# eladhoffer/convNet.pytorch

Measured on NVIDIA H100. Metric: ResNet-50 images/sec (training step, synthetic 224x224), higher is better.
Workload: dtype bf16

## Files before the change

### convnet/pytorch_b200/csrc/bn_common.cuh

```cuda
#pragma once
#include "common.cuh"
#include "host.h"

namespace b200 {

constexpr int kBnThreads = 256;
constexpr int kBnMaxC = 2048;
constexpr int kBnMaxBlocks = 1184;
constexpr int kAccumFloats = kReplicas * 2 * kBnMaxC * 2 + 64;
constexpr int kMaxPartialBlocks = 6 * 148;
constexpr int kWsFloats = kAccumFloats + kMaxPartialBlocks * 2 * kBnMaxC;

struct RowMap {
  int cv, rows_per_iter;
};
static inline RowMap make_rowmap(int C) {
  RowMap m;
  m.cv = C / 8;
  m.rows_per_iter = kBnThreads / m.cv;
  return m;
}
static inline int partial_blocks(long long M, const RowMap& rm, int resident_per_sm) {
  long long iters = (M + rm.rows_per_iter - 1) / rm.rows_per_iter;
  long long want = (iters + 3) / 4;
  long long cap = (long long)resident_per_sm * sm_count();
  if (cap > kMaxPartialBlocks) cap = kMaxPartialBlocks;
  if (want > cap) want = cap;
  if (want < 1) want = 1;
  return (int)want;
}
static inline int stream_blocks(long long M, const RowMap& rm) {
  long long iters = (M + rm.rows_per_iter - 1) / rm.rows_per_iter;
  long long blocks = (iters + 15) / 16;
  if (blocks < 1) blocks = 1;
  if (blocks > 4 * kBnMaxBlocks) blocks = 4 * kBnMaxBlocks;
  return (int)blocks;
}

__device__ __forceinline__ void load8(const __nv_bfloat16* p, float (&f)[8]) {
  const uint4 u = *reinterpret_cast<const uint4*>(p);
  float2 a = unpack_bf16x2(u.x), b = unpack_bf16x2(u.y), c = unpack_bf16x2(u.z), d = unpack_bf16x2(u.w);
  f[0] = a.x; f[1] = a.y; f[2] = b.x; f[3] = b.y; f[4] = c.x; f[5] = c.y; f[6] = d.x; f[7] = d.y;
}
__device__ __forceinline__ uint4 ld_stream(const __nv_bfloat16* p) {
  uint4 u;
  asm volatile("ld.global.nc.L1::no_allocate.v4.u32 {%0,%1,%2,%3}, [%4];"
               : "=r"(u.x), "=r"(u.y), "=r"(u.z), "=r"(u.w) : "l"(p));
  return u;
}
__device__ __forceinline__ void unpack8(const uint4& u, float (&f)[8]) {
  float2 a = unpack_bf16x2(u.x), b = unpack_bf16x2(u.y), c = unpack_bf16x2(u.z), d = unpack_bf16x2(u.w);
  f[0] = a.x; f[1] = a.y; f[2] = b.x; f[3] = b.y; f[4] = c.x; f[5] = c.y; f[6] = d.x; f[7] = d.y;
}
__device__ __forceinline__ void store8(__nv_bfloat16* p, const float (&f)[8]) {
  uint4 u;
  u.x = pack_bf16x2(f[0], f[1]); u.y = pack_bf16x2(f[2], f[3]);
  u.z = pack_bf16x2(f[4], f[5]); u.w = pack_bf16x2(f[6], f[7]);
  *reinterpret_cast<uint4*>(p) = u;
}
__device__ __forceinline__ void loadf8(const float* p, float (&f)[8]) {
  const float4 a = __ldg(reinterpret_cast<const float4*>(p));
  const float4 b = __ldg(reinterpret_cast<const float4*>(p) + 1);
  f[0] = a.x; f[1] = a.y; f[2] = a.z; f[3] = a.w; f[4] = b.x; f[5] = b.y; f[6] = b.z; f[7] = b.w;
}
__device__ __forceinline__ int act_mask_value(float pre, int act) {
  if (act == B200_ACT_RELU) return pre > 0.f ? 1 : 0;
  if (act == B200_ACT_RELU6) return (pre > 0.f && pre < 6.f) ? 1 : 0;
  return 1;
}
__device__ __forceinline__ float act_mask(float v, int act) {
  if (act == B200_ACT_RELU) return v > 0.f ? 1.f : 0.f;
  if (act == B200_ACT_RELU6) return (v > 0.f && v < 6.f) ? 1.f : 0.f;
  return 1.f;
}

__device__ __forceinline__ long long mask_byte_index(long long row, int cv8, int v8) {
  return (((row >> 2) * cv8 + v8) << 2) + (row & 3);
}
template <int ROWS>
__device__ __forceinline__ unsigned long long mask_rows(const uint8_t* __restrict__ amask, long long row0, int cv8,
                                                        int v8) {
  const uint8_t* p = amask + mask_byte_index(row0, cv8, v8);
  if (ROWS == 2) return __ldg(reinterpret_cast<const unsigned short*>(p));
  if (ROWS == 4) return __ldg(reinterpret_cast<const unsigned int*>(p));
  const unsigned long long lo = __ldg(reinterpret_cast<const unsigned int*>(p));
  const unsigned long long hi = __ldg(reinterpret_cast<const unsigned int*>(p + 4LL * cv8));
  return lo | (hi << 32);
}

template <int VEC> struct RawVec;
template <> struct RawVec<4> { uint2 u; };
template <> struct RawVec<8> { uint4 u; };
__device__ __forceinline__ RawVec<4> ldv(const __nv_bfloat16* p, RawVec<4>*) {
  RawVec<4> r;
  asm volatile("ld.global.nc.L1::no_allocate.v2.u32 {%0,%1}, [%2];" : "=r"(r.u.x), "=r"(r.u.y) : "l"(p));
  return r;
}
__device__ __forceinline__ RawVec<8> ldv(const __nv_bfloat16* p, RawVec<8>*) {
  RawVec<8> r;
  r.u = ld_stream(p);
  return r;
}
__device__ __forceinline__ void unpackv(const RawVec<4>& r, float (&f)[4]) {
  const float2 a = unpack_bf16x2(r.u.x), b = unpack_bf16x2(r.u.y);
  f[0] = a.x; f[1] = a.y; f[2] = b.x; f[3] = b.y;
}
__device__ __forceinline__ void unpackv(const RawVec<8>& r, float (&f)[8]) { unpack8(r.u, f); }
__device__ __forceinline__ void storev(__nv_bfloat16* p, const float (&f)[4]) {
  uint2 u;
  u.x = pack_bf16x2(f[0], f[1]); u.y = pack_bf16x2(f[2], f[3]);
  *reinterpret_cast<uint2*>(p) = u;
}
__device__ __forceinline__ void storev(__nv_bfloat16* p, const float (&f)[8]) { store8(p, f); }
template <int VEC>
__device__ __forceinline__ void loadfv(const float* p, float (&f)[VEC]) {
#pragma unroll
  for (int i = 0; i < VEC; i += 4) {
    const float4 a = __ldg(reinterpret_cast<const float4*>(p + i));
    f[i] = a.x; f[i + 1] = a.y; f[i + 2] = a.z; f[i + 3] = a.w;
  }
}

template <int VEC>
static inline RowMap make_rowmap_v(int C) {
  RowMap m;
  m.cv = C / VEC;
  m.rows_per_iter = kBnThreads / m.cv;
  return m;
}

static int check_c(int C, const char* who) {
  B200_REQUIRE(C > 0 && C % 8 == 0 && C <= kBnMaxC, B200_ERR_UNSUPPORTED,
               "%s: C=%d must be a multiple of 8 and <= %d", who, C, kBnMaxC);
  return B200_OK;
}


template <int VEC, int ROWS, int SRC>
__device__ __forceinline__ void bn_bwd_reduce_body(
    const __nv_bfloat16* __restrict__ dy, const __nv_bfloat16* __restrict__ y, const uint8_t* __restrict__ amask,
    const __nv_bfloat16* __restrict__ z, long long M, int C, int cv, int rows_per_iter, int act,
    const float* __restrict__ mean, const float* __restrict__ invstd, const float* __restrict__ gamma,
    const float* __restrict__ beta, float* __restrict__ partial, float dscale) {
  constexpr bool kBits = SRC >= 2;
  const int t = threadIdx.x;
  const bool active = t < rows_per_iter * cv;
  const int r0 = t / cv, v = t - r0 * cv;
  const long long rows_per_block = kBits ? (((M + gridDim.x - 1) / gridDim.x + 7) & ~7LL) : (M + gridDim.x - 1) / gridDim.x;
  const long long row_begin = blockIdx.x * rows_per_block;
  const long long row_end = min(M, row_begin + rows_per_block);
  constexpr long long kRowStep = kBits ? 1 : 0;
  float acc[2 * VEC];
#pragma unroll
  for (int i = 0; i < 2 * VEC; ++i) acc[i] = 0.f;
  if (active) {
    float mu[VEC], sc[VEC], sh[VEC];
    loadfv<VEC>(mean + v * VEC, mu);
    if (SRC == 0 && act != B200_ACT_NONE) {
      float is[VEC];
      loadfv<VEC>(invstd + v * VEC, is);
      if (gamma) loadfv<VEC>(gamma + v * VEC, sc);
      if (beta) loadfv<VEC>(beta + v * VEC, sh);
#pragma unroll
      for (int i = 0; i < VEC; ++i) {
        sc[i] = (gamma ? sc[i] : 1.f) * is[i];
        sh[i] = (beta ? sh[i] : 0.f) - mu[i] * sc[i];
      }
    }
    const long long col = (long long)v * VEC;
    const long long rstep = kRowStep ? 1 : rows_per_iter;
    for (long long r = row_begin + (kRowStep ? (long long)r0 * ROWS : r0); r < row_end;
         r += (long long)ROWS * rows_per_iter) {
      RawVec<VEC> rd[ROWS], rz[ROWS], ry[ROWS];
      unsigned long long rm = 0;
      bool ok[ROWS];
      if (kBits) rm = mask_rows<ROWS>(amask, r, C >> 3, (int)(col >> 3)) >> (col & 7 & ~(VEC - 1));
#pragma unroll
      for (int u = 0; u < ROWS; ++u) {
        const long long rr = r + (long long)u * rstep;
        ok[u] = rr < row_end;
        if (ok[u]) {
          rd[u] = ldv(dy + rr * C + col, (RawVec<VEC>*)nullptr);
          rz[u] = ldv(z + rr * C + col, (RawVec<VEC>*)nullptr);
          if (SRC == 1) ry[u] = ldv(y + rr * C + col, (RawVec<VEC>*)nullptr);
        }
      }
#pragma unroll
      for (int u = 0; u < ROWS; ++u) {
        if (!ok[u]) continue;
        float da[VEC], za[VEC], ya[VEC];
        unpackv(rd[u], da);
        unpackv(rz[u], za);
        if (SRC == 1) unpackv(ry[u], ya);
#pragma unroll
        for (int i = 0; i < VEC; ++i) {
          float g = da[i];
          if (kBits) g = ((rm >> (8 * u + i)) & 1ull) ? (SRC == 3 ? g * dscale : g) : 0.f;
          else if (act != B200_ACT_NONE && act_mask(SRC == 1 ? ya[i] : fmaf(za[i], sc[i], sh[i]), act) == 0.f) g = 0.f;
          acc[i] = fmaf(g, za[i] - mu[i], acc[i]);
          acc[VEC + i] += g;
        }
      }
    }
    float is[VEC];
    loadfv<VEC>(invstd + v * VEC, is);
#pragma unroll
    for (int i = 0; i < VEC; ++i) acc[i] *= is[i];
  }
  __shared__ float red[kBnThreads][2 * VEC + 1];
#pragma unroll
  for (int i = 0; i < 2 * VEC; ++i) red[t][i] = acc[i];
  __syncthreads();
  float* dst = partial + (size_t)blockIdx.x * 2 * C;
  for (int o = t; o < 2 * C; o += kBnThreads) {
    const int stat = o / C;
    const int c = o - stat * C;
    const int vv = c / VEC, e = c - vv * VEC;
    float sacc = 0.f;
    for (int r = 0; r < rows_per_iter; ++r) sacc += red[r * cv + vv][stat * VEC + e];
    dst[o] = sacc;
  }
}

template <int VEC, int ROWS, int SRC>
__device__ __forceinline__ void bn_bwd_dx_body(
    const __nv_bfloat16* __restrict__ dy, const __nv_bfloat16* __restrict__ y, const uint8_t* __restrict__ amask,
    const __nv_bfloat16* __restrict__ z, long long M, int C, int cv, int rows_per_iter, int act,
    const float* __restrict__ mean, const float* __restrict__ invstd, const float* __restrict__ gamma,
    const float* __restrict__ beta, const float* __restrict__ sums, __nv_bfloat16* __restrict__ dz,
    __nv_bfloat16* __restrict__ g_out, float dscale) {
  constexpr bool kBits = SRC >= 2;
  const int t = threadIdx.x;
  if (t >= rows_per_iter * cv) return;
  const int r0 = t / cv, v = t - r0 * cv;
  const long long rows_per_block = kBits ? (((M + gridDim.x - 1) / gridDim.x + 7) & ~7LL) : (M + gridDim.x - 1) / gridDim.x;
  const long long row_begin = blockIdx.x * rows_per_block;
  const long long row_end = min(M, row_begin + rows_per_block);
  constexpr long long kRowStep = kBits ? 1 : 0;
  float A[VEC], B[VEC], Cc[VEC], sh[VEC];
  {
    float mu[VEC], is[VEC], dg[VEC], dbt[VEC];
    loadfv<VEC>(mean + v * VEC, mu);
    loadfv<VEC>(invstd + v * VEC, is);
    if (gamma) loadfv<VEC>(gamma + v * VEC, A);
    if (beta) loadfv<VEC>(beta + v * VEC, sh);
    loadfv<VEC>(sums + v * VEC, dg);
    loadfv<VEC>(sums + C + v * VEC, dbt);
    const float invM = 1.f / (float)M;
#pragma unroll
    for (int i = 0; i < VEC; ++i) {
      const float gm = gamma ? A[i] : 1.f;
      A[i] = gm * is[i];
      B[i] = -gm * is[i] * is[i] * dg[i] * invM;
      Cc[i] = -A[i] * dbt[i] * invM - B[i] * mu[i];
      sh[i] = (beta ? sh[i] : 0.f) - mu[i] * A[i];
    }
  }
  const long long col = (long long)v * VEC;
  const long long rstep = kRowStep ? 1 : rows_per_iter;
  for (long long r = row_begin + (kRowStep ? (long long)r0 * ROWS : r0); r < row_end;
       r += (long long)ROWS * rows_per_iter) {
    RawVec<VEC> rd[ROWS], rz[ROWS], ry[ROWS];
    unsigned long long rm = 0;
    bool ok[ROWS];
    if (kBits) rm = mask_rows<ROWS>(amask, r, C >> 3, (int)(col >> 3)) >> (col & 7 & ~(VEC - 1));
#pragma unroll
    for (int u = 0; u < ROWS; ++u) {
      const long long rr = r + (long long)u * rstep;
      ok[u] = rr < row_end;
      if (ok[u]) {
        rd[u] = ldv(dy + rr * C + col, (RawVec<VEC>*)nullptr);
        rz[u] = ldv(z + rr * C + col, (RawVec<VEC>*)nullptr);
        if (SRC == 1) ry[u] = ldv(y + rr * C + col, (RawVec<VEC>*)nullptr);
      }
    }
#pragma unroll
    for (int u = 0; u < ROWS; ++u) {
      if (!ok[u]) continue;
      const long long rr = r + (long long)u * rstep;
      float da[VEC], za[VEC], ya[VEC];
      unpackv(rd[u], da);
      unpackv(rz[u], za);
      if (SRC == 1) unpackv(ry[u], ya);
#pragma unroll
      for (int i = 0; i < VEC; ++i) {
        float g = da[i];
        if (kBits) g = ((rm >> (8 * u + i)) & 1ull) ? (SRC == 3 ? g * dscale : g) : 0.f;
        else if (act != B200_ACT_NONE && act_mask(SRC == 1 ? ya[i] : fmaf(za[i], A[i], sh[i]), act) == 0.f) g = 0.f;
        da[i] = g;
        za[i] = A[i] * g + B[i] * za[i] + Cc[i];
      }
      storev(dz + rr * C + col, za);
      if (g_out) storev(g_out + rr * C + col, da);
    }
  }
}

void launch_bwd_reduce_final(const float* partial, int nblocks, int C, float* sums, float* dgamma_acc,
                             float* dbeta_acc, cudaStream_t stream);

}
```

### convnet/pytorch_b200/csrc/conv.cu

```cuda
#include "common.cuh"
#include "host.h"
#include <stdlib.h>
#include <utility>

namespace b200 {

constexpr int kMaxStages = 8;
constexpr int kMaxTaps = 32;
constexpr int kConsumers = 256;
constexpr int kProducerWarp = 8;

struct TapEntry {
  uint16_t off_w, off_h;
  uint16_t b_tap;
  uint16_t pad_;
};

struct IgemmParams {
  int M_total;
  int I, J;
  int trav;
  int lower_w, lower_h;
  int N_total;
  int block_n, n_tiles, m_tiles;
  int ck, c_chunks;
  int ntaps;
  int num_stages;
  uint32_t a_bytes, b_bytes, tx_bytes;
  int OH, OW, os, oh0, ow0;
  int ldo;
  int act, out_fp32;
  int tma_store;
  int plain_a;
  int b_stationary;
  int own_ntile;
  int window;
  uint32_t epi_bytes;
  double* stats;
  void* out;
  const void* res;
  const float* bias;
  TapEntry taps[kMaxTaps];
};

__device__ __forceinline__ void store_pair(const IgemmParams& p, float v0, float v1, long long off, int n) {
  if (n >= p.N_total) return;
  const bool two = n + 1 < p.N_total;
  const bool vec = two && (p.ldo & 1) == 0;
  if (p.bias != nullptr) {
    v0 += __ldg(p.bias + n);
    if (two) v1 += __ldg(p.bias + n + 1);
  }
  if (p.res != nullptr) {
    const __nv_bfloat16* r = reinterpret_cast<const __nv_bfloat16*>(p.res) + off + n;
    if (vec) {
      const float2 t = unpack_bf16x2(*reinterpret_cast<const uint32_t*>(r));
      v0 += t.x;
      v1 += t.y;
    } else {
      v0 += __bfloat162float(r[0]);
      if (two) v1 += __bfloat162float(r[1]);
    }
  }
  v0 = apply_act(v0, p.act);
  v1 = apply_act(v1, p.act);
  if (p.out_fp32) {
    float* o = reinterpret_cast<float*>(p.out) + off + n;
    if (vec) {
      *reinterpret_cast<float2*>(o) = make_float2(v0, v1);
    } else {
      o[0] = v0;
      if (two) o[1] = v1;
    }
  } else {
    __nv_bfloat16* o = reinterpret_cast<__nv_bfloat16*>(p.out) + off + n;
    if (vec) {
      *reinterpret_cast<uint32_t*>(o) = pack_bf16x2(v0, v1);
    } else {
      o[0] = __float2bfloat16(v0);
      if (two) o[1] = __float2bfloat16(v1);
    }
  }
}

template <int KS, int SZ>
__device__ __forceinline__ void igemm_stage_mma(float (&acc)[2][SZ], uint64_t da, uint64_t db, uint32_t a_half,
                                                uint32_t scale0) {
  wgmma_fence();
#pragma unroll
  for (int k = 0; k < KS; ++k) {
    wgmma_bf16<0, 0>(acc[0], da + 2 * k, db + 2 * k, k != 0 ? 1u : scale0);
    wgmma_bf16<0, 0>(acc[1], da + a_half + 2 * k, db + 2 * k, k != 0 ? 1u : scale0);
  }
  wgmma_commit();
}

template <int BN>
__global__ void __launch_bounds__(kThreads, 1)
conv_igemm_kernel(const __grid_constant__ CUtensorMap tmA, const __grid_constant__ CUtensorMap tmB,
                  const __grid_constant__ CUtensorMap tmC, const __grid_constant__ CUtensorMap tmR,
                  const __grid_constant__ IgemmParams p) {
  extern __shared__ uint8_t smem_raw[];
  __shared__ __align__(8) uint64_t full_bar[kMaxStages];
  __shared__ __align__(8) uint64_t empty_bar[kMaxStages];
  __shared__ __align__(8) uint64_t turn_bar[2], res_bar[2], bstat_bar;

  const int warp = threadIdx.x >> 5;
  const int lane = threadIdx.x & 31;
  const uint32_t raw_addr = smem_u32(smem_raw);
  uint8_t* smem = smem_raw + (((raw_addr + 1023u) & ~1023u) - raw_addr);
  const uint32_t stage_bytes = p.b_stationary ? p.a_bytes : p.a_bytes + p.b_bytes;
  uint8_t* sBstat = smem + p.num_stages * stage_bytes;
  uint8_t* epi = sBstat + (p.b_stationary ? static_cast<uint32_t>(p.ntaps * p.c_chunks) * p.b_bytes : 0u);

  if (threadIdx.x == 0) {
    for (int s = 0; s < p.num_stages; ++s) {
      mbar_init(&full_bar[s], 1);
      mbar_init(&empty_bar[s], 4);
    }
    mbar_init(&bstat_bar, 1);
    for (int i = 0; i < 2; ++i) {
      mbar_init(&res_bar[i], 1);
      mbar_init(&turn_bar[i], 4);
    }
    fence_mbar_init();
    prefetch_tmap(&tmA);
    prefetch_tmap(&tmB);
    if (p.tma_store) {
      prefetch_tmap(&tmC);
      if (p.res != nullptr) prefetch_tmap(&tmR);
    }
  }
  __syncthreads();

  const int k_iters = p.ntaps * p.c_chunks;
  const int walk_first = p.own_ntile ? static_cast<int>(blockIdx.x) / p.n_tiles : static_cast<int>(blockIdx.x);
  const int walk_step = p.own_ntile ? static_cast<int>(gridDim.x) / p.n_tiles : static_cast<int>(gridDim.x);
  const int walk_end = p.own_ntile ? p.m_tiles : p.m_tiles * p.n_tiles;
  const int own_n = static_cast<int>(blockIdx.x) % p.n_tiles;

  if (warp >= kProducerWarp) {
    producer_setmaxnreg();
    if (warp == kProducerWarp && lane == 0) {
      int stage = 0;
      uint32_t phase = 0;
      const int IJ = p.I * p.J;
      if (p.b_stationary && walk_first < walk_end) {
        mbar_arrive_expect_tx(&bstat_bar, static_cast<uint32_t>(k_iters) * (p.tx_bytes - p.a_bytes));
        for (int t = 0; t < p.ntaps; ++t)
          for (int cc = 0; cc < p.c_chunks; ++cc)
            tma_load_3d(&tmB, &bstat_bar, sBstat + (t * p.c_chunks + cc) * p.b_bytes, cc * p.ck, p.taps[t].b_tap,
                        p.own_ntile ? own_n * BN : 0);
      }
      for (int tile = walk_first; tile < walk_end; tile += walk_step) {
        const int m_tile = p.own_ntile ? tile : tile / p.n_tiles;
        const int n_tile = p.own_ntile ? own_n : tile - m_tile * p.n_tiles;
        const int m0 = m_tile * kTileM;
        const int img = m0 / IJ;
        const int rem = m0 - img * IJ;
        const int bi = rem / p.J;
        const int bj = rem - bi * p.J;
        const int base_w = bj * p.trav + p.lower_w;
        const int base_h = bi * p.trav + p.lower_h;
        const int a_c0 = p.window ? (n_tile * BN / p.window) * p.window : 0;
        for (int t = 0; t < p.ntaps; ++t) {
          const TapEntry te = p.taps[t];
          for (int cc = 0; cc < p.c_chunks; ++cc) {
            mbar_wait(&empty_bar[stage], phase ^ 1u);
            uint8_t* sa = smem + stage * stage_bytes;
            uint8_t* sb = sa + p.a_bytes;
            mbar_arrive_expect_tx(&full_bar[stage], p.b_stationary ? p.a_bytes : p.tx_bytes);
            const int a_c = a_c0 + cc * p.ck;
            if (p.plain_a)
              tma_load_2d(&tmA, &full_bar[stage], sa, a_c, m0);
            else
              tma_load_im2col_4d(&tmA, &full_bar[stage], sa, a_c, base_w, base_h, img, te.off_w, te.off_h);
            if (!p.b_stationary) tma_load_3d(&tmB, &full_bar[stage], sb, cc * p.ck, te.b_tap, n_tile * BN);
            if (++stage == p.num_stages) { stage = 0; phase ^= 1u; }
          }
        }
      }
    }
    return;
  }
  consumer_setmaxnreg();

  const int wg = warp >> 2;
  const int wt = threadIdx.x & 127;
  const int r_lo = (warp & 3) * 16 + (lane >> 2);
  const int c_lo = 2 * (lane & 3);
  const bool leader = wt == 0;
  const uint32_t row_bytes = p.ck * 2;
  const uint64_t proto = make_smem_desc(0, 16, 8 * row_bytes, layout_type_for_row_bytes(row_bytes));
  const uint32_t a_half = (64u * row_bytes) >> 4;
  const int ksteps = p.ck / 16;
  const uint32_t bstat_addr = smem_u32(sBstat);
  constexpr int nbox = BN / 64;
  uint8_t* epi_w = epi + wg * p.epi_bytes;
  const int st_col = wt % BN;
  constexpr int st_rows = BN;
  const int st_row0 = (wt / BN) * st_rows;
  int st_ntile = -1;
  float st_s1 = 0.f, st_s2 = 0.f;
  const int IJ = p.I * p.J;
  if (p.b_stationary && walk_first < walk_end) mbar_wait(&bstat_bar, 0);

  float acc[2][BN / 2];
  int local = 0;
  for (int tile = walk_first; tile < walk_end; tile += walk_step, ++local) {
    if ((local & 1) != wg) continue;
    const int m_tile = p.own_ntile ? tile : tile / p.n_tiles;
    const int n_tile = p.own_ntile ? own_n : tile - m_tile * p.n_tiles;
    const int nbase = n_tile * BN;
    const int mine = local >> 1;
    if (p.tma_store) {
      if (leader && mine > 0) bulk_wait_group_read0();
      named_bar_sync(1 + wg, 128);
      if (leader && p.res != nullptr) {
        fence_proxy_async();
        mbar_arrive_expect_tx(&res_bar[wg], static_cast<uint32_t>(nbox) * kTileM * 128u);
        for (int b = 0; b < nbox; ++b)
          tma_load_2d(&tmR, &res_bar[wg], epi_w + b * (kTileM * 128), nbase + b * 64, m_tile * kTileM);
      }
    }

    const int pos = local * k_iters;
    int stage = pos % p.num_stages;
    uint32_t phase = static_cast<uint32_t>(pos / p.num_stages) & 1u;
    if (local > 0) mbar_wait(&turn_bar[wg], static_cast<uint32_t>((local - 1) >> 1) & 1u);
    wgmma_fence_acc(acc[0]);
    wgmma_fence_acc(acc[1]);
    int prev = 0;
    for (int it = 0; it < k_iters; ++it) {
      mbar_wait(&full_bar[stage], phase);
      const uint32_t a_addr = smem_u32(smem + stage * stage_bytes);
      const uint64_t da = proto + (a_addr >> 4);
      const uint64_t db = proto + ((p.b_stationary ? bstat_addr + it * p.b_bytes : a_addr + p.a_bytes) >> 4);
      const uint32_t scale0 = it != 0 ? 1u : 0u;
      if (ksteps == 4) igemm_stage_mma<4>(acc, da, db, a_half, scale0);
      else if (ksteps == 2) igemm_stage_mma<2>(acc, da, db, a_half, scale0);
      else igemm_stage_mma<1>(acc, da, db, a_half, scale0);
      wgmma_wait<1>();
      if (it > 0) release_stage(&empty_bar[prev], lane);
      prev = stage;
      if (++stage == p.num_stages) { stage = 0; phase ^= 1u; }
    }
    __syncwarp();
    if (lane == 0) mbar_arrive(&turn_bar[wg ^ 1]);
    wgmma_wait<0>();
    wgmma_fence_acc(acc[0]);
    wgmma_fence_acc(acc[1]);
    release_stage(&empty_bar[prev], lane);

    if (p.tma_store) {
      if constexpr (BN % 64 == 0) {
        if (p.res != nullptr) mbar_wait(&res_bar[wg], static_cast<uint32_t>(mine & 1));
#pragma unroll
        for (int j = 0; j < BN / 2; j += 4) {
          const int c = 2 * j + c_lo;
          float bias0 = 0.f, bias1 = 0.f;
          if (p.bias != nullptr) { bias0 = __ldg(p.bias + nbase + c); bias1 = __ldg(p.bias + nbase + c + 1); }
#pragma unroll
          for (int mh = 0; mh < 2; ++mh)
#pragma unroll
            for (int h = 0; h < 2; ++h) {
              const int row = mh * 64 + r_lo + 8 * h;
              uint32_t* dst = reinterpret_cast<uint32_t*>(epi_w + staged_offset(row, c, kTileM * 128));
              float v0 = acc[mh][j + 2 * h] + bias0, v1 = acc[mh][j + 2 * h + 1] + bias1;
              if (p.res != nullptr) {
                const float2 t = unpack_bf16x2(*dst);
                v0 += t.x;
                v1 += t.y;
              }
              *dst = pack_bf16x2(apply_act(v0, p.act), apply_act(v1, p.act));
            }
        }
        fence_proxy_async();
        named_bar_sync(1 + wg, 128);
        if (leader) {
          for (int b = 0; b < nbox; ++b)
            tma_store_2d(&tmC, epi_w + b * (kTileM * 128), nbase + b * 64, m_tile * kTileM);
          bulk_commit_group();
        }
        if constexpr (BN == 64 || BN == 128) {
          if (p.stats != nullptr) {
            if (st_ntile != n_tile) {
              if (st_ntile >= 0) {
                flush_bn_stats(p.stats, p.N_total, st_ntile * BN, st_col, st_s1, st_s2);
                st_s1 = 0.f; st_s2 = 0.f;
              }
              st_ntile = n_tile;
            }
            float s1 = 0.f, s2 = 0.f;
#pragma unroll 8
            for (int r = st_row0; r < st_row0 + st_rows; ++r) {
              const float vv = __bfloat162float(*reinterpret_cast<const __nv_bfloat16*>(epi_w + staged_offset(r, st_col, kTileM * 128)));
              s1 += vv;
              s2 = fmaf(vv, vv, s2);
            }
            st_s1 += s1;
            st_s2 += s2;
          }
        }
      }
      continue;
    }
#pragma unroll
    for (int mh = 0; mh < 2; ++mh)
#pragma unroll
      for (int h = 0; h < 2; ++h) {
        const int m = m_tile * kTileM + mh * 64 + r_lo + 8 * h;
        if (m >= p.M_total) continue;
        const int img = m / IJ;
        const int rem = m - img * IJ;
        const int bi = rem / p.J;
        const int bj = rem - bi * p.J;
        const long long off = ((static_cast<long long>(img) * p.OH + (bi * p.os + p.oh0)) * p.OW + (bj * p.os + p.ow0)) *
                              static_cast<long long>(p.ldo);
#pragma unroll
        for (int j = 0; j < BN / 2; j += 4) store_pair(p, acc[mh][j + 2 * h], acc[mh][j + 2 * h + 1], off, nbase + 2 * j + c_lo);
      }
  }
  if constexpr (BN == 64 || BN == 128)
    if (p.stats != nullptr && st_ntile >= 0) flush_bn_stats(p.stats, p.N_total, st_ntile * BN, st_col, st_s1, st_s2);
  if (p.tma_store && leader) bulk_wait_group0();
}

constexpr int kBk = 64;
struct WgradParams {
  int M_total;
  int P, Q;
  int trav;
  int lower_w, lower_h;
  int K_out, C, taps_total;
  int ckA, ckB;
  int bk;
  int c_chunks;
  int total_boxes;
  int boxes_per_cta;
  int k_tiles, col_groups, splits;
  int blocks_per_split, total_blocks;
  int num_stages;
  uint32_t boxA_bytes, boxB_bytes, stage_bytes;
  float* dw;
  int plain_x;
  float* partial;
  int pitch;
  int window;
  int S_filter;
};

__device__ __forceinline__ void red_add_v2(float* addr, float a, float b) {
  asm volatile("red.global.add.v2.f32 [%0], {%1, %2};" ::"l"(addr), "f"(a), "f"(b) : "memory");
}

template <int NC>
__global__ void __launch_bounds__(kThreads, 1)
conv_wgrad_kernel(const __grid_constant__ CUtensorMap tmDy, const __grid_constant__ CUtensorMap tmX,
                  const __grid_constant__ WgradParams p) {
  extern __shared__ uint8_t smem_raw[];
  __shared__ __align__(8) uint64_t full_bar[kMaxStages];
  __shared__ __align__(8) uint64_t empty_bar[kMaxStages];

  const int warp = threadIdx.x >> 5;
  const int lane = threadIdx.x & 31;
  const uint32_t raw_addr = smem_u32(smem_raw);
  uint8_t* smem = smem_raw + (((raw_addr + 1023u) & ~1023u) - raw_addr);

  if (threadIdx.x == 0) {
    for (int s = 0; s < p.num_stages; ++s) {
      mbar_init(&full_bar[s], 1);
      mbar_init(&empty_bar[s], kConsumers / 32);
    }
    fence_mbar_init();
    prefetch_tmap(&tmDy);
    prefetch_tmap(&tmX);
  }
  __syncthreads();

  const int tiles = p.k_tiles * p.col_groups;
  const int split = blockIdx.x / tiles;
  const int tile = blockIdx.x - split * tiles;
  const int k_tile = tile % p.k_tiles;
  const int cgroup = tile / p.k_tiles;
  const int k0 = k_tile * kTileM;
  const int box0 = cgroup * p.boxes_per_cta;
  const int nboxes = min(p.boxes_per_cta, p.total_boxes - box0);
  const int blk_begin = split * p.blocks_per_split;
  const int blk_end = min(p.total_blocks, blk_begin + p.blocks_per_split);
  const int nblk = blk_end - blk_begin;
  const uint32_t a_tile = (kTileM / p.ckA) * p.boxA_bytes;
  if (nblk <= 0) return;

  if (warp >= kProducerWarp) {
    producer_setmaxnreg();
    if (warp == kProducerWarp && lane == 0) {
      int stage = 0;
      uint32_t phase = 0;
      const int PQ = p.P * p.Q;
      const int nA = min(kTileM / p.ckA, (p.K_out - k0 + p.ckA - 1) / p.ckA);
      int box_c[8];
      uint16_t box_w[8], box_h[8];
      for (int x = 0; x < 8; ++x) {
        const int id = box0 + min(x, nboxes - 1);
        const int t = id / p.c_chunks;
        const int th = t / p.S_filter;
        box_c[x] = (id - t * p.c_chunks) * p.ckB + (p.window ? k0 : 0);
        box_w[x] = static_cast<uint16_t>(t - th * p.S_filter);
        box_h[x] = static_cast<uint16_t>(th);
      }
      const uint32_t tx = nA * p.boxA_bytes + nboxes * p.boxB_bytes;
      for (int b = blk_begin; b < blk_end; ++b) {
        const int pix0 = b * p.bk;
        mbar_wait(&empty_bar[stage], phase ^ 1u);
        uint8_t* sa = smem + stage * p.stage_bytes;
        uint8_t* sb = sa + a_tile;
        mbar_arrive_expect_tx(&full_bar[stage], tx);
        for (int a = 0; a < nA; ++a)
          tma_load_2d(&tmDy, &full_bar[stage], sa + a * p.boxA_bytes, k0 + a * p.ckA, pix0);
        if (p.plain_x) {
#pragma unroll
          for (int x = 0; x < 8; ++x)
            if (x < nboxes) tma_load_2d(&tmX, &full_bar[stage], sb + x * p.boxB_bytes, box_c[x], pix0);
        } else {
          const int img = pix0 / PQ;
          const int rem = pix0 - img * PQ;
          const int pi = rem / p.Q;
          const int pj = rem - pi * p.Q;
          const int base_w = pj * p.trav + p.lower_w;
          const int base_h = pi * p.trav + p.lower_h;
#pragma unroll
          for (int x = 0; x < 8; ++x)
            if (x < nboxes)
              tma_load_im2col_4d(&tmX, &full_bar[stage], sb + x * p.boxB_bytes, box_c[x], base_w, base_h, img, box_w[x],
                                 box_h[x]);
        }
        if (++stage == p.num_stages) { stage = 0; phase ^= 1u; }
      }
    }
    return;
  }

  consumer_setmaxnreg();

  const int wg = warp >> 2;
  const bool wg_on = k0 + wg * 64 < p.K_out;
  const int ncols = nboxes * p.ckB;
  const uint64_t protoA = make_smem_desc(0, p.boxA_bytes, 8 * p.ckA * 2, layout_type_for_row_bytes(p.ckA * 2));
  const uint64_t protoB = make_smem_desc(0, p.boxB_bytes, 8 * p.ckB * 2, layout_type_for_row_bytes(p.ckB * 2));
  const uint32_t a_wg = (wg * (64 / p.ckA) * p.boxA_bytes) >> 4;
  const uint32_t kincA = (16u * p.ckA * 2) >> 4, kincB = (16u * p.ckB * 2) >> 4;
  float acc[NC / 2];
  wgmma_fence_acc(acc);
  int stage = 0, prev = 0;
  uint32_t phase = 0;
  for (int b = 0; b < nblk; ++b) {
    mbar_wait(&full_bar[stage], phase);
    const uint32_t a_addr = smem_u32(smem + stage * p.stage_bytes);
    if (wg_on) {
      const uint64_t da = protoA + (a_addr >> 4) + a_wg, db = protoB + ((a_addr + a_tile) >> 4);
      wgmma_fence();
#pragma unroll
      for (int k = 0; k < kBk / 16; ++k)
        wgmma_bf16<1, 1>(acc, da + k * kincA, db + k * kincB, (b | k) != 0 ? 1u : 0u);
      wgmma_commit();
      wgmma_wait<1>();
    }
    if (b > 0) release_stage(&empty_bar[prev], lane);
    prev = stage;
    if (++stage == p.num_stages) { stage = 0; phase ^= 1u; }
  }
  wgmma_wait<0>();
  wgmma_fence_acc(acc);
  release_stage(&empty_bar[prev], lane);
  if (!wg_on) return;

  const int r_lo = wg * 64 + (warp & 3) * 16 + (lane >> 2);
  const int c_lo = 2 * (lane & 3);
#pragma unroll
  for (int h = 0; h < 2; ++h) {
    const int k = k0 + r_lo + 8 * h;
    if (k >= p.K_out) continue;
    if (p.partial != nullptr) {
      float* dst = p.partial + ((static_cast<long long>(tile) * p.splits + split) * kTileM + (r_lo + 8 * h)) * p.pitch;
#pragma unroll
      for (int j = 0; j < NC / 2; j += 4)
        if (2 * j < ncols)
          *reinterpret_cast<float2*>(dst + 2 * j + c_lo) = make_float2(acc[j + 2 * h], acc[j + 2 * h + 1]);
    } else {
#pragma unroll
      for (int j = 0; j < NC / 2; j += 4) {
        const int col = 2 * j + c_lo;
        if (col < ncols) {
          const int x = col / p.ckB;
          const int id = box0 + x;
          const int tap = id / p.c_chunks;
          const int c = (id - tap * p.c_chunks) * p.ckB + (col - x * p.ckB);
          if (c < p.C) red_add_v2(p.dw + (static_cast<long long>(k) * p.taps_total + tap) * p.C + c, acc[j + 2 * h],
                                  acc[j + 2 * h + 1]);
        }
      }
    }
  }
}

__global__ void __launch_bounds__(256) conv_wgrad_reduce_kernel(const float* __restrict__ partial, float* __restrict__ dw,
                                                                int K_out, int taps, int C, int ck, int tap_stride,
                                                                int cc_stride, int bpc, int k_tiles, int splits,
                                                                int pitch) {
  __shared__ float4 red[8][32];
  const int c4n = C >> 2;
  const long long total = static_cast<long long>(K_out) * taps * c4n;
  const int lane = threadIdx.x & 31, w = threadIdx.x >> 5, nw = blockDim.x >> 5;
  for (long long base = static_cast<long long>(blockIdx.x) * 32; base < total; base += static_cast<long long>(gridDim.x) * 32) {
    const long long idx = base + lane;
    float4 acc = make_float4(0.f, 0.f, 0.f, 0.f);
    int c = 0, tap = 0, k = 0;
    if (idx < total) {
      c = static_cast<int>(idx % c4n) * 4;
      tap = static_cast<int>((idx / c4n) % taps);
      k = static_cast<int>(idx / (static_cast<long long>(c4n) * taps));
      const int k_tile = k / kTileM, row = k - k_tile * kTileM;
      const int cc = c / ck;
      const int id = tap * tap_stride + cc * cc_stride;
      const int cgroup = id / bpc, x = id - cgroup * bpc;
      const int unit = cgroup * k_tiles + k_tile;
      const float* src = partial + ((static_cast<long long>(unit) * splits) * kTileM + row) * pitch + x * ck + (c - cc * ck);
      for (int s2 = w; s2 < splits; s2 += nw) {
        const float4 v = __ldcg(reinterpret_cast<const float4*>(src + static_cast<long long>(s2) * kTileM * pitch));
        acc.x += v.x; acc.y += v.y; acc.z += v.z; acc.w += v.w;
      }
    }
    red[w][lane] = acc;
    __syncthreads();
    if (w == 0 && idx < total) {
      for (int j = 1; j < nw; ++j) {
        const float4 v = red[j][lane];
        acc.x += v.x; acc.y += v.y; acc.z += v.z; acc.w += v.w;
      }
      float4* o = reinterpret_cast<float4*>(dw + (static_cast<long long>(k) * taps + tap) * C + c);
      float4 cur = *o;
      cur.x += acc.x; cur.y += acc.y; cur.z += acc.z; cur.w += acc.w;
      *o = cur;
    }
    __syncthreads();
  }
}

static int pick_ck(int channels) { return channels <= 16 ? 16 : (channels <= 32 ? 32 : 64); }

static int encode_im2col(CUtensorMap* tm, const void* base, int Nimg, int H, int W, int C, int ck, int pixels,
                         int lower_w, int lower_h, int upper_w, int upper_h, int trav, long long pix_stride = 0,
                         long long row_stride = 0, long long img_stride = 0) {
  EncodeIm2colFn fn = encode_im2col_fn();
  B200_REQUIRE(fn != nullptr, B200_ERR_CUDA, "cuTensorMapEncodeIm2col entry point unavailable");
  cuuint64_t dims[4] = {(cuuint64_t)C, (cuuint64_t)W, (cuuint64_t)H, (cuuint64_t)Nimg};
  cuuint64_t strides[3] = {(cuuint64_t)C * 2, (cuuint64_t)W * C * 2, (cuuint64_t)H * W * C * 2};
  if (pix_stride > 0) {
    strides[0] = (cuuint64_t)pix_stride * 2;
    strides[1] = (cuuint64_t)row_stride * 2;
    strides[2] = (cuuint64_t)img_stride * 2;
  }
  int lower[2] = {lower_w, lower_h};
  int upper[2] = {upper_w, upper_h};
  cuuint32_t estr[4] = {1, (cuuint32_t)trav, (cuuint32_t)trav, 1};
  B200_REQUIRE(lower_w >= -128 && lower_w <= 127 && lower_h >= -128 && lower_h <= 127 && upper_w >= -128 &&
                   upper_w <= 127 && upper_h >= -128 && upper_h <= 127,
               B200_ERR_UNSUPPORTED, "im2col corner offsets out of the TMA range");
  CUresult r = fn(tm, CU_TENSOR_MAP_DATA_TYPE_BFLOAT16, 4, const_cast<void*>(base), dims, strides, lower, upper,
                  (cuuint32_t)ck, (cuuint32_t)pixels, estr, CU_TENSOR_MAP_INTERLEAVE_NONE,
                  swizzle_for_row_bytes(ck * 2), CU_TENSOR_MAP_L2_PROMOTION_L2_128B,
                  CU_TENSOR_MAP_FLOAT_OOB_FILL_NONE);
  B200_REQUIRE(r == CUDA_SUCCESS, B200_ERR_CUDA,
               "cuTensorMapEncodeIm2col failed (%d) N=%d H=%d W=%d C=%d ck=%d pix=%d lower=(%d,%d) upper=(%d,%d) trav=%d",
               (int)r, Nimg, H, W, C, ck, pixels, lower_w, lower_h, upper_w, upper_h, trav);
  int drv = 0;
  cudaDriverGetVersion(&drv);
  if (drv <= 13010 && (size_t)Nimg * H * W * C * 2 < 131072) {
    reinterpret_cast<uint64_t*>(tm)[1] &= ~(1ull << 21);
  }
  return B200_OK;
}

static const int kSmemBudget = 200 * 1024;
static const int kSmemBudgetMax = 224 * 1024;

int launch_wgrad_reduce(const float* partial, float* dw, int K_out, int taps, int C, int ck, int tap_stride,
                        int cc_stride, int bpc, int k_tiles, int splits, int pitch, cudaStream_t stream) {
  const long long total = static_cast<long long>(K_out) * taps * (C / 4);
  long long blocks = (total + 31) / 32;
  if (blocks > 16LL * sm_count()) blocks = 16LL * sm_count();
  int warps = 8;
  while (warps > 1 && warps > splits) warps >>= 1;
  b200::launch(conv_wgrad_reduce_kernel, static_cast<int>(blocks), 32 * warps, 0, stream, partial, dw, K_out, taps, C, ck,
               tap_stride, cc_stride, bpc, k_tiles, splits, pitch);
  B200_CHECK_LAUNCH("conv_wgrad_reduce_kernel");
  return B200_OK;
}

struct IgemmLaunch {
  const void* src; int Nimg, SH, SW, SC;
  long long s_pix, s_row, s_img;
  const void* wmat; int Nout, wtaps;
  int I, J, trav, lower_w, lower_h;
  int ntaps; TapEntry taps[kMaxTaps];
  void* out; int OH, OW, os, oh0, ow0, ldo;
  const void* res; const float* bias; int act, out_fp32;
  double* stats;
  int window;
};

template <int... Is>
static auto igemm_kernel_for(int block_n, std::integer_sequence<int, Is...>) {
  static constexpr decltype(&conv_igemm_kernel<16>) table[] = {&conv_igemm_kernel<16 * (Is + 1)>...};
  return table[block_n / 16 - 1];
}
static auto wgrad_kernel_for(int ncols) {
  static constexpr decltype(&conv_wgrad_kernel<16>) table[] = {
      &conv_wgrad_kernel<16>,  &conv_wgrad_kernel<32>,  &conv_wgrad_kernel<48>,  &conv_wgrad_kernel<64>,
      &conv_wgrad_kernel<80>,  &conv_wgrad_kernel<96>,  &conv_wgrad_kernel<112>, &conv_wgrad_kernel<128>,
      nullptr,                 &conv_wgrad_kernel<160>, nullptr,                 &conv_wgrad_kernel<192>,
      nullptr,                 &conv_wgrad_kernel<224>, nullptr,                 &conv_wgrad_kernel<256>};
  return table[ncols / 16 - 1];
}

static int launch_igemm(const IgemmLaunch& L, cudaStream_t stream) {
  B200_REQUIRE(L.SC % 8 == 0, B200_ERR_UNSUPPORTED, "igemm: source channels (%d) must be a multiple of 8", L.SC);
  B200_REQUIRE(L.ntaps >= 1 && L.ntaps <= kMaxTaps, B200_ERR_UNSUPPORTED, "igemm: %d taps unsupported", L.ntaps);
  IgemmParams p;
  memset(&p, 0, sizeof(p));
  p.M_total = L.Nimg * L.I * L.J;
  B200_REQUIRE(p.M_total > 0, B200_ERR_INVALID, "igemm: empty problem");
  p.I = L.I; p.J = L.J; p.trav = L.trav; p.lower_w = L.lower_w; p.lower_h = L.lower_h;
  p.N_total = L.Nout;
  p.block_n = L.Nout % 128 == 0 ? 128 : (L.Nout % 64 == 0 ? 64 : 0);
  if (p.block_n == 0) {
    const int nt = (L.Nout + 127) / 128;
    p.block_n = (((L.Nout + nt - 1) / nt) + 15) / 16 * 16;
  }
  p.n_tiles = (L.Nout + p.block_n - 1) / p.block_n;
  p.m_tiles = (p.M_total + kTileM - 1) / kTileM;
  p.ck = pick_ck(L.SC);
  p.c_chunks = (L.SC + p.ck - 1) / p.ck;
  p.window = L.window;
  if (L.window) {
    B200_REQUIRE(L.window % 64 == 0 && L.window <= 256 && L.SC == L.Nout && L.Nout % L.window == 0, B200_ERR_UNSUPPORTED,
                 "igemm: window %d needs C == K (C=%d K=%d), K %% window == 0", L.window, L.SC, L.Nout);
    p.block_n = L.window <= 128 ? L.window : L.window / 2;
    p.n_tiles = L.Nout / p.block_n;
    p.ck = 64;
    p.c_chunks = L.window / 64;
  }
  p.ntaps = L.ntaps;
  p.a_bytes = kTileM * p.ck * 2;
  p.b_bytes = p.block_n * p.ck * 2;
  p.tx_bytes = p.a_bytes + p.b_bytes;
  uint32_t stage = p.a_bytes + p.b_bytes;
  if (stage % 1024) { p.b_bytes += 1024 - stage % 1024; stage = p.a_bytes + p.b_bytes; }
  p.tma_store = (L.os == 1 && !L.out_fp32 && (p.block_n % 64) == 0 && (L.Nout % p.block_n) == 0 && L.ldo == L.Nout &&
                 L.OH == L.I && L.OW == L.J && L.oh0 == 0 && L.ow0 == 0) ? 1 : 0;
  const int epi_bytes = p.tma_store ? kTileM * p.block_n * 2 : 0;
  const int epi_total = 2 * epi_bytes;
  const int b_all = L.ntaps * p.c_chunks * (int)p.b_bytes;
  int bstat_bytes = 0;
  if (p.n_tiles == 1 && !L.window && (p.a_bytes % 1024) == 0 && (p.b_bytes % 1024) == 0 && b_all <= 64 * 1024) {
    p.b_stationary = 1;
    bstat_bytes = b_all;
    stage = p.a_bytes;
  }
  int grid_own = 0;
  if (!p.b_stationary && p.n_tiles > 1 && p.n_tiles <= 8 && !L.window &&
      (p.a_bytes % 1024) == 0 && (p.b_bytes % 1024) == 0 && (L.Nout % p.block_n) == 0) {
    const int ctas = sm_count() / p.n_tiles;
    const long long a_all = (long long)p.M_total * L.SC * 2 * L.ntaps;
    const long long w_all = (long long)b_all * p.n_tiles;
    const long long rr_bytes = a_all * p.n_tiles + w_all * p.m_tiles;
    const long long own_bytes = a_all * p.n_tiles + (long long)b_all * ctas * p.n_tiles;
    const int stages_left = (kSmemBudgetMax - epi_total - b_all) / (int)p.a_bytes;
    if (ctas >= 1 && p.m_tiles >= 4 * ctas && stages_left >= 3 && own_bytes * 4 <= rr_bytes * 3) {
      p.b_stationary = 1;
      p.own_ntile = 1;
      bstat_bytes = b_all;
      stage = p.a_bytes;
      grid_own = ctas * p.n_tiles;
    }
  }
  p.epi_bytes = (uint32_t)epi_bytes;
  p.num_stages = (kSmemBudgetMax - epi_total - bstat_bytes) / (int)stage;
  if (p.num_stages > kMaxStages) p.num_stages = kMaxStages;
  if (p.num_stages < 2) p.num_stages = 2;
  p.OH = L.OH; p.OW = L.OW; p.os = L.os; p.oh0 = L.oh0; p.ow0 = L.ow0; p.ldo = L.ldo;
  p.act = L.act; p.out_fp32 = L.out_fp32; p.out = L.out; p.res = L.res; p.bias = L.bias;
  p.stats = L.stats;
  if (L.stats != nullptr)
    B200_REQUIRE(p.tma_store && (128 % p.block_n) == 0 && L.res == nullptr && L.bias == nullptr && L.act == 0,
                 B200_ERR_UNSUPPORTED, "conv_fprop: fused BN statistics need a dense bf16 output with K %% 64 == 0 "
                 "(block_n=%d) and no bias/residual/activation", p.block_n);
  for (int t = 0; t < L.ntaps; ++t) p.taps[t] = L.taps[t];

  const int upper_w = L.lower_w + (L.J - 1) * L.trav + 1 - L.SW;
  const int upper_h = L.lower_h + (L.I - 1) * L.trav + 1 - L.SH;
  CUtensorMap tmA, tmB;
  int rc;
  p.plain_a = (L.ntaps == 1 && L.trav == 1 && L.lower_w == 0 && L.lower_h == 0 && L.taps[0].off_w == 0 &&
               L.taps[0].off_h == 0 && L.I == L.SH && L.J == L.SW && L.s_pix == 0) ? 1 : 0;
  if (p.plain_a)
    rc = encode_tiled(&tmA, L.src, 2, {L.SC, p.M_total}, {p.ck, kTileM}, "igemm A");
  else
    rc = encode_im2col(&tmA, L.src, L.Nimg, L.SH, L.SW, L.SC, p.ck, kTileM, L.lower_w, L.lower_h, upper_w, upper_h,
                       L.trav, L.s_pix, L.s_row, L.s_img);
  if (rc) return rc;
  rc = encode_tiled(&tmB, L.wmat, 3, {L.window ? L.window : L.SC, L.wtaps, L.Nout}, {p.ck, 1, p.block_n}, "igemm B");
  if (rc) return rc;

  CUtensorMap tmC, tmR;
  memset(&tmC, 0, sizeof(tmC));
  memset(&tmR, 0, sizeof(tmR));
  if (p.tma_store) {
    rc = encode_tiled(&tmC, L.out, 2, {L.ldo, p.M_total}, {64, kTileM}, "igemm output");
    if (rc) return rc;
    if (L.res != nullptr) {
      rc = encode_tiled(&tmR, L.res, 2, {L.ldo, p.M_total}, {64, kTileM}, "igemm residual");
      if (rc) return rc;
    }
  }
  const int smem_bytes = p.num_stages * (int)stage + bstat_bytes + epi_total + 1024;
  const auto kfn = igemm_kernel_for(p.block_n, std::make_integer_sequence<int, 8>{});
  rc = set_smem_attr((const void*)kfn, smem_bytes);
  if (rc) return rc;
  const int total_tiles = p.m_tiles * p.n_tiles;
  const int grid = grid_own ? grid_own : (total_tiles < sm_count() ? total_tiles : sm_count());
  if (getenv("B200_IGEMM_DEBUG")) {
    const int max_tiles = p.own_ntile ? (p.m_tiles + grid / p.n_tiles - 1) / (grid / p.n_tiles)
                                      : (total_tiles + grid - 1) / grid;
    fprintf(stderr, "[igemm] M=%d C=%d N=%d taps=%d os=%d block_n=%d n_tiles=%d m_tiles=%d ck=%d k_iters=%d stages=%d "
            "tma_store=%d plain_a=%d bstat=%d own=%d out_fp32=%d bias=%d res=%d act=%d stats=%d grid=%d max_tiles=%d "
            "smem=%d\n",
            p.M_total, L.SC, L.Nout, L.ntaps, L.os, p.block_n, p.n_tiles, p.m_tiles, p.ck, L.ntaps * p.c_chunks,
            p.num_stages, p.tma_store, p.plain_a, p.b_stationary, p.own_ntile, p.out_fp32, L.bias != nullptr,
            L.res != nullptr, p.act, L.stats != nullptr, grid, max_tiles, smem_bytes);
  }
  b200::launch(kfn, grid, kThreads, smem_bytes, stream, tmA, tmB, tmC, tmR, p);
  B200_CHECK_LAUNCH("conv_igemm_kernel");
  return B200_OK;
}

static int check_desc(const b200_conv_desc* d) {
  B200_REQUIRE(d != nullptr, B200_ERR_INVALID, "conv: null descriptor");
  B200_REQUIRE(d->N > 0 && d->H > 0 && d->W > 0 && d->C > 0 && d->K > 0 && d->R > 0 && d->S > 0 && d->P > 0 &&
                   d->Q > 0 && d->stride >= 1 && d->stride <= 8,
               B200_ERR_INVALID, "conv: bad descriptor N=%d H=%d W=%d C=%d K=%d R=%d S=%d P=%d Q=%d stride=%d", d->N,
               d->H, d->W, d->C, d->K, d->R, d->S, d->P, d->Q, d->stride);
  B200_REQUIRE(d->R * d->S <= kMaxTaps, B200_ERR_UNSUPPORTED, "conv: %dx%d filter exceeds %d taps", d->R, d->S,
               kMaxTaps);
  B200_REQUIRE((d->x_pixel_stride == 0 && d->x_row_stride == 0 && d->x_image_stride == 0) ||
                   (d->x_pixel_stride > 0 && d->x_pixel_stride % 8 == 0 && d->x_row_stride % 8 == 0 &&
                    d->x_image_stride % 8 == 0 && d->x_row_stride > 0 && d->x_image_stride > 0),
               B200_ERR_INVALID, "conv: x strides must all be 0 (dense) or positive multiples of 8 elements");
  B200_REQUIRE(d->window == 0 || (d->window % 64 == 0 && d->C == d->K && d->C % d->window == 0 && d->x_pixel_stride == 0),
               B200_ERR_UNSUPPORTED, "conv: window %d needs C == K, C %% window == 0 (C=%d K=%d)", d->window, d->C, d->K);
  return B200_OK;
}

}

using namespace b200;

extern "C" int b200_conv_fprop(const b200_conv_desc* d, const void* x, const void* w, void* y,
                               const b200_epilogue* ep, b200_stream_t stream) {
  int rc = check_desc(d);
  if (rc) return rc;
  B200_REQUIRE(x && w && y, B200_ERR_INVALID, "conv_fprop: null pointer");
  B200_REQUIRE(d->C % 8 == 0, B200_ERR_UNSUPPORTED, "conv_fprop: C=%d must be a multiple of 8 (pad the input)", d->C);
  if (d->stride == 1 && d->pad_h == d->pad_w && d->P == d->H + 2 * d->pad_h - d->R + 1 &&
      d->Q == d->W + 2 * d->pad_w - d->S + 1 && d->x_pixel_stride == 0 && (!ep || !ep->out_fp32) &&
      !(ep && ep->bias && ep->bn_stats_workspace) && (d->window == 0 || d->window == 64) &&
      halo_eligible(d->P, d->Q, d->C, d->K, d->R, d->S, d->pad_h)) {
    return launch_halo(x, w, y, ep ? ep->residual : nullptr, ep ? ep->bias : nullptr, d->N, d->P, d->Q, d->C, d->K,
                       d->R, d->S, d->pad_h, 0, ep ? ep->act : 0,
                       (ep && ep->bn_stats_workspace) ? reinterpret_cast<double*>(ep->bn_stats_workspace) : nullptr,
                       (cudaStream_t)stream, d->window);
  }
  IgemmLaunch L;
  memset(&L, 0, sizeof(L));
  L.src = x; L.Nimg = d->N; L.SH = d->H; L.SW = d->W; L.SC = d->C;
  L.s_pix = d->x_pixel_stride; L.s_row = d->x_row_stride; L.s_img = d->x_image_stride;
  L.wmat = w; L.Nout = d->K; L.wtaps = d->R * d->S;
  L.I = d->P; L.J = d->Q; L.trav = d->stride; L.lower_w = -d->pad_w; L.lower_h = -d->pad_h;
  L.ntaps = d->R * d->S;
  for (int r = 0; r < d->R; ++r)
    for (int s = 0; s < d->S; ++s) {
      TapEntry& t = L.taps[r * d->S + s];
      t.off_w = (uint16_t)s; t.off_h = (uint16_t)r; t.b_tap = (uint16_t)(r * d->S + s); t.pad_ = 0;
    }
  L.out = y; L.OH = d->P; L.OW = d->Q; L.os = 1; L.oh0 = 0; L.ow0 = 0; L.ldo = d->K;
  L.res = ep ? ep->residual : nullptr;
  L.bias = ep ? ep->bias : nullptr;
  L.act = ep ? ep->act : 0;
  L.out_fp32 = ep ? ep->out_fp32 : 0;
  L.stats = (ep && ep->bn_stats_workspace) ? reinterpret_cast<double*>(ep->bn_stats_workspace) : nullptr;
  L.window = d->window;
  return launch_igemm(L, (cudaStream_t)stream);
}

extern "C" int b200_conv_dgrad(const b200_conv_desc* d, const void* dy, const void* wt, void* dx,
                               const void* residual, b200_stream_t stream_) {
  int rc = check_desc(d);
  if (rc) return rc;
  cudaStream_t stream = (cudaStream_t)stream_;
  B200_REQUIRE(dy && wt && dx, B200_ERR_INVALID, "conv_dgrad: null pointer");
  B200_REQUIRE(d->K % 8 == 0, B200_ERR_UNSUPPORTED, "conv_dgrad: K=%d must be a multiple of 8", d->K);
  const int st = d->stride;
  B200_REQUIRE(st == 1 || st == 2, B200_ERR_UNSUPPORTED, "conv_dgrad: stride %d unsupported", st);
  if (d->R == 3 && d->S == 3 && st == 1 && d->pad_h == 1 && d->pad_w == 1 && d->P == d->H && d->Q == d->W &&
      (d->window == 0 || d->window == 64) && halo_eligible(d->H, d->W, d->K, d->C, 3, 3, 1)) {
    return launch_halo(dy, wt, dx, residual, nullptr, d->N, d->H, d->W, d->K, d->C, 3, 3, 1, 1, 0, nullptr, stream,
                       d->window);
  }
  bool any_empty = false;
  for (int ph = 0; ph < st; ++ph)
    for (int pw = 0; pw < st; ++pw) {
      int nr = 0, ns = 0;
      for (int r = 0; r < d->R; ++r) if (((ph + d->pad_h - r) % st + st) % st == 0) ++nr;
      for (int s = 0; s < d->S; ++s) if (((pw + d->pad_w - s) % st + st) % st == 0) ++ns;
      if (nr * ns == 0 && (d->H - ph + st - 1) / st > 0 && (d->W - pw + st - 1) / st > 0) any_empty = true;
    }
  if (any_empty) {
    B200_REQUIRE(residual == nullptr, B200_ERR_UNSUPPORTED,
                 "conv_dgrad: residual add with an empty stride class is unsupported");
    cudaError_t e = cudaMemsetAsync(dx, 0, (size_t)d->N * d->H * d->W * d->C * 2, stream);
    B200_REQUIRE(e == cudaSuccess, B200_ERR_CUDA, "conv_dgrad: memset failed: %s", cudaGetErrorString(e));
    count_launch();
  }
  for (int ph = 0; ph < st; ++ph)
    for (int pw = 0; pw < st; ++pw) {
      const int I = (d->H - ph + st - 1) / st;
      const int J = (d->W - pw + st - 1) / st;
      if (I <= 0 || J <= 0) continue;
      IgemmLaunch L;
      memset(&L, 0, sizeof(L));
      int dh[kMaxTaps], dwv[kMaxTaps], rr[kMaxTaps], ss[kMaxTaps];
      int nr = 0, ns = 0;
      for (int r = 0; r < d->R; ++r) {
        const int v = ph + d->pad_h - r;
        if (((v % st) + st) % st == 0) { dh[nr] = (v - (((v % st) + st) % st)) / st; rr[nr] = r; ++nr; }
      }
      for (int s = 0; s < d->S; ++s) {
        const int v = pw + d->pad_w - s;
        if (((v % st) + st) % st == 0) { dwv[ns] = (v - (((v % st) + st) % st)) / st; ss[ns] = s; ++ns; }
      }
      if (nr * ns == 0) continue;
      int lo_h = dh[0], lo_w = dwv[0];
      for (int i = 1; i < nr; ++i) lo_h = dh[i] < lo_h ? dh[i] : lo_h;
      for (int i = 1; i < ns; ++i) lo_w = dwv[i] < lo_w ? dwv[i] : lo_w;
      L.ntaps = nr * ns;
      for (int a = 0; a < nr; ++a)
        for (int b = 0; b < ns; ++b) {
          TapEntry& t = L.taps[a * ns + b];
          t.off_h = (uint16_t)(dh[a] - lo_h);
          t.off_w = (uint16_t)(dwv[b] - lo_w);
          t.b_tap = (uint16_t)(rr[a] * d->S + ss[b]);
          t.pad_ = 0;
        }
      L.src = dy; L.Nimg = d->N; L.SH = d->P; L.SW = d->Q; L.SC = d->K;
      L.wmat = wt; L.Nout = d->C; L.wtaps = d->R * d->S;
      L.I = I; L.J = J; L.trav = 1; L.lower_w = lo_w; L.lower_h = lo_h;
      L.out = dx; L.OH = d->H; L.OW = d->W; L.os = st; L.oh0 = ph; L.ow0 = pw; L.ldo = d->C;
      L.res = residual; L.bias = nullptr; L.act = 0; L.out_fp32 = 0;
      L.window = d->window;
      rc = launch_igemm(L, stream);
      if (rc) return rc;
    }
  return B200_OK;
}

extern "C" size_t b200_conv_wgrad_workspace_bytes(void) {
  return static_cast<size_t>(sm_count() + 8) * kTileM * 512 * sizeof(float);
}

extern "C" int b200_conv_wgrad(const b200_conv_desc* d, const void* x, const void* dy, float* dw, void* workspace,
                               size_t workspace_bytes, b200_stream_t stream_) {
  int rc = check_desc(d);
  if (rc) return rc;
  cudaStream_t stream = (cudaStream_t)stream_;
  B200_REQUIRE(x && dy && dw, B200_ERR_INVALID, "conv_wgrad: null pointer");
  B200_REQUIRE(d->C % 8 == 0 && d->K % 8 == 0, B200_ERR_UNSUPPORTED,
               "conv_wgrad: C=%d and K=%d must be multiples of 8", d->C, d->K);
  if (d->stride == 1 && d->pad_h == d->pad_w && d->P == d->H + 2 * d->pad_h - d->R + 1 &&
      d->Q == d->W + 2 * d->pad_w - d->S + 1 && d->x_pixel_stride == 0 &&
      (d->window == 0 || d->window == 128) &&
      halo_wgrad_eligible(d->P, d->Q, d->C, d->K, d->R, d->S, d->pad_h, d->window))
    return launch_halo_wgrad(x, dy, dw, workspace, workspace_bytes, d->N, d->P, d->Q, d->C, d->K, d->R, d->S, d->pad_h,
                             stream, d->window);
  B200_REQUIRE(d->window == 0 || d->window == 128, B200_ERR_UNSUPPORTED, "conv_wgrad: window must be 0 or 128");
  const int Cw = d->window ? d->window : d->C;
  WgradParams p;
  memset(&p, 0, sizeof(p));
  p.M_total = d->N * d->P * d->Q;
  p.P = d->P; p.Q = d->Q; p.trav = d->stride; p.lower_w = -d->pad_w; p.lower_h = -d->pad_h;
  p.K_out = d->K; p.C = Cw; p.taps_total = d->R * d->S;
  p.window = d->window;
  p.ckA = pick_ck(d->K);
  p.ckB = pick_ck(Cw);
  p.bk = kBk;
  p.c_chunks = (Cw + p.ckB - 1) / p.ckB;
  p.total_boxes = p.taps_total * p.c_chunks;
  p.k_tiles = (d->K + kTileM - 1) / kTileM;
  p.boxA_bytes = p.bk * p.ckA * 2;
  p.boxB_bytes = p.bk * p.ckB * 2;
  p.boxes_per_cta = 256 / p.ckB;
  if (p.boxes_per_cta > 8) p.boxes_per_cta = 8;
  if (p.boxes_per_cta > p.total_boxes) p.boxes_per_cta = p.total_boxes;
  p.col_groups = (p.total_boxes + p.boxes_per_cta - 1) / p.boxes_per_cta;
  p.total_blocks = (p.M_total + p.bk - 1) / p.bk;
  const int tiles = p.k_tiles * p.col_groups;
  int splits = sm_count() / tiles;
  if (splits > p.total_blocks) splits = p.total_blocks;
  if (splits < 1) splits = 1;
  p.blocks_per_split = (p.total_blocks + splits - 1) / splits;
  p.splits = (p.total_blocks + p.blocks_per_split - 1) / p.blocks_per_split;
  p.stage_bytes = (kTileM / p.ckA) * p.boxA_bytes + p.boxes_per_cta * p.boxB_bytes;
  p.stage_bytes = (p.stage_bytes + 1023u) & ~1023u;
  p.num_stages = kSmemBudget / (int)p.stage_bytes;
  if (p.num_stages > kMaxStages) p.num_stages = kMaxStages;
  if (p.num_stages < 2) p.num_stages = 2;
  p.dw = dw;
  p.pitch = p.boxes_per_cta * p.ckB;
  p.partial = nullptr;
  if (p.splits > 1) {
    const size_t need = static_cast<size_t>(tiles) * p.splits * kTileM * p.pitch * sizeof(float);
    B200_REQUIRE(workspace != nullptr && workspace_bytes >= need, B200_ERR_INVALID,
                 "conv_wgrad: workspace too small (%zu < %zu); see b200_conv_wgrad_workspace_bytes()", workspace_bytes,
                 need);
    B200_REQUIRE((Cw & 3) == 0, B200_ERR_UNSUPPORTED, "conv_wgrad: C must be a multiple of 4");
    p.partial = static_cast<float*>(workspace);
  }
  p.S_filter = d->S;
  CUtensorMap tmDy, tmX;
  rc = encode_tiled(&tmDy, dy, 2, {d->K, p.M_total}, {p.ckA, p.bk}, "wgrad dy");
  if (rc) return rc;
  const int upper_w = p.lower_w + (d->Q - 1) * d->stride + 1 - d->W;
  const int upper_h = p.lower_h + (d->P - 1) * d->stride + 1 - d->H;
  p.plain_x = (d->R == 1 && d->S == 1 && d->stride == 1 && d->pad_h == 0 && d->pad_w == 0 && d->P == d->H &&
               d->Q == d->W && d->x_pixel_stride == 0) ? 1 : 0;
  if (getenv("B200_WGRAD_DEBUG"))
    fprintf(stderr, "[wgrad] K=%d C=%d taps=%d stride=%d ckA=%d ckB=%d kt=%d bpc=%d k_groups=%d col_groups=%d splits=%d "
            "bps=%d stages=%d stage=%u nc=%d nboxes_last=%d plain_x=%d partial=%d\n", d->K, d->C, p.taps_total,
            d->stride, p.ckA, p.ckB, 1, p.boxes_per_cta, p.k_tiles, p.col_groups, p.splits, p.blocks_per_split,
            p.num_stages, p.stage_bytes, p.pitch, p.total_boxes - (p.col_groups - 1) * p.boxes_per_cta, p.plain_x,
            p.partial != nullptr);
  if (p.plain_x)
    rc = encode_tiled(&tmX, x, 2, {d->C, p.M_total}, {p.ckB, p.bk}, "wgrad x");
  else
    rc = encode_im2col(&tmX, x, d->N, d->H, d->W, d->C, p.ckB, p.bk, p.lower_w, p.lower_h, upper_w, upper_h,
                       d->stride, d->x_pixel_stride, d->x_row_stride, d->x_image_stride);
  if (rc) return rc;
  const int smem_bytes = p.num_stages * (int)p.stage_bytes + 1024;
  const auto kfn = wgrad_kernel_for(p.pitch);
  rc = set_smem_attr((const void*)kfn, smem_bytes);
  if (rc) return rc;
  const int grid = tiles * p.splits;
  b200::launch(kfn, grid, kThreads, smem_bytes, stream, tmDy, tmX, p);
  B200_CHECK_LAUNCH("conv_wgrad_kernel");
  if (p.partial == nullptr) return B200_OK;
  return launch_wgrad_reduce(p.partial, dw, d->K, p.taps_total, Cw, p.ckB, p.c_chunks, 1, p.boxes_per_cta, p.k_tiles,
                             p.splits, p.pitch, stream);
}
```

### convnet/pytorch_b200/csrc/host.cu

```cuda
#include "host.h"
#include <atomic>
#include <mutex>
#include <string.h>

namespace b200 {

static thread_local char g_err[512] = "";
static std::atomic<long long> g_launches{0};

void set_error(const char* fmt, ...) {
  va_list ap;
  va_start(ap, fmt);
  vsnprintf(g_err, sizeof(g_err), fmt, ap);
  va_end(ap);
}
void count_launch(int n) { g_launches.fetch_add(n, std::memory_order_relaxed); }

int sm_count() {
  static int cached[64] = {0};
  int dev = 0;
  cudaGetDevice(&dev);
  if (dev < 0 || dev >= 64) dev = 0;
  if (cached[dev] == 0) {
    int n = 0;
    cudaDeviceGetAttribute(&n, cudaDevAttrMultiProcessorCount, dev);
    cached[dev] = n > 0 ? n : 148;
  }
  return cached[dev];
}

static void* driver_entry(const char* name) {
  void* fn = nullptr;
  cudaDriverEntryPointQueryResult q;
  if (cudaGetDriverEntryPoint(name, &fn, cudaEnableDefault, &q) != cudaSuccess ||
      q != cudaDriverEntryPointSuccess) {
    return nullptr;
  }
  return fn;
}
EncodeIm2colFn encode_im2col_fn() {
  static EncodeIm2colFn fn = (EncodeIm2colFn)driver_entry("cuTensorMapEncodeIm2col");
  return fn;
}

typedef CUresult (*EncodeTiledFn)(CUtensorMap*, CUtensorMapDataType, cuuint32_t, void*, const cuuint64_t*,
                                  const cuuint64_t*, const cuuint32_t*, const cuuint32_t*, CUtensorMapInterleave,
                                  CUtensorMapSwizzle, CUtensorMapL2promotion, CUtensorMapFloatOOBfill);

int encode_tiled(CUtensorMap* tm, const void* base, int rank, const long long (&dims)[4], const int (&box)[4],
                 const char* what) {
  static EncodeTiledFn fn = (EncodeTiledFn)driver_entry("cuTensorMapEncodeTiled");
  B200_REQUIRE(fn != nullptr, B200_ERR_CUDA, "cuTensorMapEncodeTiled entry point unavailable");
  cuuint64_t gdims[4], strides[3];
  cuuint32_t gbox[4], estr[4] = {1, 1, 1, 1};
  for (int i = 0; i < rank; ++i) {
    gdims[i] = (cuuint64_t)dims[i];
    gbox[i] = (cuuint32_t)box[i];
    if (i + 1 < rank) strides[i] = (i == 0 ? 2 : strides[i - 1]) * gdims[i];
  }
  CUresult r = fn(tm, CU_TENSOR_MAP_DATA_TYPE_BFLOAT16, rank, const_cast<void*>(base), gdims, strides, gbox, estr,
                  CU_TENSOR_MAP_INTERLEAVE_NONE, swizzle_for_row_bytes(box[0] * 2), CU_TENSOR_MAP_L2_PROMOTION_L2_128B,
                  CU_TENSOR_MAP_FLOAT_OOB_FILL_NONE);
  if (r != CUDA_SUCCESS) {
    char d[96] = "", b[64] = "";
    for (int i = 0, nd = 0, nb = 0; i < rank; ++i) {
      nd += snprintf(d + nd, sizeof(d) - nd, i ? ",%lld" : "%lld", dims[i]);
      nb += snprintf(b + nb, sizeof(b) - nb, i ? ",%d" : "%d", box[i]);
    }
    set_error("%s: cuTensorMapEncodeTiled(%dd) failed (%d) dims=(%s) box=(%s)", what, rank, (int)r, d, b);
    return B200_ERR_CUDA;
  }
  return B200_OK;
}

int set_smem_attr(const void* fn, int bytes) {
  cudaError_t e = cudaFuncSetAttribute(fn, cudaFuncAttributeMaxDynamicSharedMemorySize, bytes);
  B200_REQUIRE(e == cudaSuccess, B200_ERR_CUDA, "cudaFuncSetAttribute(smem=%d): %s", bytes, cudaGetErrorString(e));
  return B200_OK;
}

}

extern "C" {
const char* b200_last_error(void) { return b200::g_err; }
int b200_version(void) { return 100; }
long long b200_launch_count(void) { return b200::g_launches.load(); }
}
```

### convnet/pytorch_b200/csrc/host.h

```cpp
#pragma once
#include <cuda.h>
#include <cuda_runtime.h>
#include <stdarg.h>
#include <stdio.h>
#include "../../../include/b200conv.h"

namespace b200 {

void set_error(const char* fmt, ...);
void count_launch(int n = 1);
int sm_count();

typedef CUresult (*EncodeIm2colFn)(CUtensorMap*, CUtensorMapDataType, cuuint32_t, void*, const cuuint64_t*,
                                   const cuuint64_t*, const int*, const int*, cuuint32_t, cuuint32_t,
                                   const cuuint32_t*, CUtensorMapInterleave, CUtensorMapSwizzle,
                                   CUtensorMapL2promotion, CUtensorMapFloatOOBfill);
EncodeIm2colFn encode_im2col_fn();

int encode_tiled(CUtensorMap* tm, const void* base, int rank, const long long (&dims)[4], const int (&box)[4],
                 const char* what);
int set_smem_attr(const void* fn, int bytes);

int launch_wgrad_reduce(const float* partial, float* dw, int K_out, int taps, int C, int ck, int tap_stride,
                        int cc_stride, int bpc, int k_tiles, int splits, int pitch, cudaStream_t stream);

bool halo_geometry_ok(int H, int W, int Cs, int R, int S, int pad);
bool halo_eligible(int H, int W, int Cs, int Nout, int R, int S, int pad);
int launch_halo(const void* src, const void* wmat, void* out, const void* res, const float* bias, int N, int H, int W,
                int Cs, int Nout, int R, int S, int pad, int dir, int act, double* stats, cudaStream_t stream,
                int window = 0);

bool halo_wgrad_eligible(int H, int W, int C, int K_out, int R, int S, int pad, int window);
int launch_halo_wgrad(const void* x, const void* dy, float* dw, void* workspace, size_t workspace_bytes, int N, int H,
                      int W, int C, int K_out, int R, int S, int pad, cudaStream_t stream, int window = 0);

template <typename... KArgs, typename... Args>
inline void launch(void (*kernel)(KArgs...), dim3 grid, dim3 block, size_t smem, cudaStream_t stream, Args&&... args) {
  kernel<<<grid, block, smem, stream>>>(static_cast<KArgs>(args)...);
}

inline CUtensorMapSwizzle swizzle_for_row_bytes(int row_bytes) {
  return row_bytes == 128 ? CU_TENSOR_MAP_SWIZZLE_128B
                          : (row_bytes == 64 ? CU_TENSOR_MAP_SWIZZLE_64B : CU_TENSOR_MAP_SWIZZLE_32B);
}

#define B200_CHECK_LAUNCH(name)                                                   \
  do {                                                                            \
    cudaError_t e__ = cudaGetLastError();                                         \
    if (e__ != cudaSuccess) {                                                     \
      b200::set_error("%s: launch failed: %s", name, cudaGetErrorString(e__));    \
      return B200_ERR_CUDA;                                                       \
    }                                                                             \
    b200::count_launch();                                                         \
  } while (0)

#define B200_REQUIRE(cond, code, ...)   \
  do {                                  \
    if (!(cond)) {                      \
      b200::set_error(__VA_ARGS__);     \
      return code;                      \
    }                                   \
  } while (0)

}
```

### convnet/pytorch_b200/engine.py

```python
import torch
import torch.nn as nn

from . import ops
from .lib import B200Error, ACT_NONE, ACT_RELU, ACT_RELU6

_ALIGN = 64
FOLD_BN_EVAL = True


def _round_up(n, m):
    return (n + m - 1) // m * m


class _Slot(object):
    __slots__ = ('name', 'param', 'kind', 'offset', 'numel', 'alloc', 'shape', 'group', 'module')


class Arena(object):

    def __init__(self, model, device):
        self.device = device
        self.convs = []
        self.version = 0
        self.grads_zero = False
        slots = []
        seen = set()
        for mod_name, mod in model.named_modules():
            for p_name, p in mod.named_parameters(recurse=False):
                if id(p) in seen:
                    continue
                seen.add(id(p))
                s = _Slot()
                s.name = (mod_name + '.' if mod_name else '') + p_name
                s.param, s.module, s.shape = p, mod, tuple(p.shape)
                s.numel = p.numel()
                s.alloc = s.numel
                if isinstance(mod, nn.Conv2d) and p_name == 'weight':
                    depthwise = mod.groups > 1 and mod.groups == mod.in_channels and mod.in_channels == mod.out_channels
                    if mod.groups > 1 and not depthwise and (mod.in_channels % mod.groups or mod.out_channels % mod.groups):
                        raise B200Error('grouped convolution %s: channels not divisible by groups' % s.name)
                    s.kind = 'dw' if depthwise else 'conv'
                    s.group = 1 if depthwise else 0
                elif isinstance(mod, nn.Linear) and p_name == 'weight':
                    s.kind, s.group = 'fc', 0
                    s.alloc = _round_up(p.shape[0], 8) * p.shape[1]
                elif isinstance(mod, nn.Linear) and p_name == 'bias':
                    s.kind, s.group = 'vec', 2
                    s.alloc = _round_up(p.shape[0], 8)
                else:
                    s.kind, s.group = 'vec', 2
                slots.append(s)
        slots.sort(key=lambda s: s.group)
        off = 0
        self.group_end = [0, 0, 0]
        for s in slots:
            s.offset = off
            off += _round_up(s.alloc, _ALIGN)
            self.group_end[s.group] = off
        self.group_end[1] = max(self.group_end[1], self.group_end[0])
        self.group_end[2] = off
        self.total = off
        self.slots = slots
        self.by_param = {id(s.param): s for s in slots}
        self.p32 = torch.zeros(off, device=device, dtype=torch.float32)
        self.g32 = torch.zeros(off, device=device, dtype=torch.float32)
        self.p16 = torch.zeros(off, device=device, dtype=torch.bfloat16)
        with torch.no_grad():
            for s in slots:
                src = s.param.detach().to(device=device, dtype=torch.float32)
                view = self.logical_view(self.p32, s)
                view.copy_(src)
                s.param.data = view
                s.param.grad = self.logical_view(self.g32, s)
        self.sync_shadow()

    def logical_view(self, flat, s):
        seg = flat[s.offset:s.offset + s.numel]
        if s.kind == 'conv':
            K, C, R, S = s.shape
            return seg.view(K, R, S, C).permute(0, 3, 1, 2)
        if s.kind == 'dw':
            C, _, R, S = s.shape
            return seg.view(R, S, C).permute(2, 0, 1).unsqueeze(1)
        return seg.view(s.shape)

    def kernel_view(self, flat, s):
        if s.kind == 'conv':
            K, C, R, S = s.shape
            return flat[s.offset:s.offset + s.numel].view(K, R * S, C)
        if s.kind == 'dw':
            C, _, R, S = s.shape
            return flat[s.offset:s.offset + s.numel].view(R * S, C)
        if s.kind == 'fc':
            K, C = s.shape
            return flat[s.offset:s.offset + s.alloc].view(_round_up(K, 8), 1, C)
        return flat[s.offset:s.offset + s.alloc]

    def slot(self, param):
        return self.by_param[id(param)]

    def sync_shadow(self):
        ops.cast_bf16(self.p32, self.p16)
        self.version += 1

    def zero_grad(self):
        if not self.grads_zero:
            self.g32.zero_()
            self.grads_zero = True

    def zero_grad_force(self):
        self.grads_zero = False
        self.zero_grad()

    def rebind_grads(self):
        for s in self.slots:
            if s.param.grad is None or s.param.grad.data_ptr() != self.g32.data_ptr() + 4 * s.offset:
                s.param.grad = self.logical_view(self.g32, s)


class _Conv(object):
    def __init__(self, arena, mod):
        s = arena.slot(mod.weight)
        self.kind = s.kind
        self.K, self.C = mod.out_channels, mod.in_channels
        self.R, self.S = mod.kernel_size
        self.stride = mod.stride[0]
        self.pad = mod.padding[0]
        if mod.stride[0] != mod.stride[1] or mod.padding[0] != mod.padding[1] or mod.dilation != (1, 1):
            raise B200Error('conv %s: only square stride/padding and dilation 1 are supported' % s.name)
        self.bias32 = None
        if mod.bias is not None:
            if s.kind != 'dw':
                raise B200Error('conv %s: bias is only supported on depthwise convolutions followed by BatchNorm' % s.name)
            self.bias32 = arena.kernel_view(arena.p32, arena.slot(mod.bias))
        self.groups = mod.groups if s.kind == 'conv' else 1
        cg = self.C // max(self.groups, 1)
        self.window = 64 if (self.groups > 1 and self.C == self.K and self.C % 128 == 0 and 64 % cg == 0) else 0
        self.slot = s
        self.wt = None
        arena.convs.append(self)
        self.w16 = arena.kernel_view(arena.p16, s)
        self.w32 = arena.kernel_view(arena.p32, s)
        self.g32 = arena.kernel_view(arena.g32, s)

    def desc(self, N, H, W, wgrad=False):
        return ops.make_desc(N, H, W, self.C, self.K, self.R, self.S, self.stride, self.pad,
                             algo_macs=self.K * self.R * self.S * self.C // self.groups,
                             window=(128 if wgrad else 64) if self.window else 0)

    def kernel_weights(self, w32=None):
        if self.groups == 1:
            return self.w16
        return ops.group_weight_pack(self.w32 if w32 is None else w32, self.K, self.R * self.S, self.C, self.groups,
                                     self.window or self.C)

    def dgrad_weights(self):
        return ops.group_weight_pack(self.w32, self.K, self.R * self.S, self.C, self.groups, self.window or self.C,
                                     transpose=True)


class _BN(object):

    def __init__(self, arena, mod):
        from .models.modules.lp_norm import L1BatchNorm2d
        if not mod.affine or not mod.track_running_stats:
            raise B200Error('BatchNorm2d without affine/running stats is not supported')
        self.mod = mod
        self.l1 = isinstance(mod, L1BatchNorm2d)
        self.C = mod.num_features
        sw, sb = arena.slot(mod.weight), arena.slot(mod.bias)
        self.gamma = arena.kernel_view(arena.p32, sw)
        self.beta = arena.kernel_view(arena.p32, sb)
        self.dgamma = arena.kernel_view(arena.g32, sw)
        self.dbeta = arena.kernel_view(arena.g32, sb)


class _SE(object):

    def __init__(self, arena, mod):
        from .models.modules.se import SEBlock
        if not isinstance(mod, SEBlock):
            raise B200Error('residual_block of type %s is outside the B200 hot path' % type(mod).__name__)
        l1, l2 = mod.transform[0], mod.transform[2]
        self.C, self.hidden = l1.in_features, l1.out_features
        if self.C % 8 or self.hidden % 8 or l2.out_features != self.C:
            raise B200Error('SE gate: channel counts must be multiples of 8 (got %d -> %d)' % (self.C, self.hidden))
        sw1, sb1, sw2, sb2 = (arena.slot(p) for p in (l1.weight, l1.bias, l2.weight, l2.bias))
        self.w1, self.gw1 = arena.kernel_view(arena.p16, sw1), arena.kernel_view(arena.g32, sw1)
        self.b1, self.gb1 = arena.kernel_view(arena.p32, sb1), arena.kernel_view(arena.g32, sb1)
        self.w2, self.gw2 = arena.kernel_view(arena.p16, sw2), arena.kernel_view(arena.g32, sw2)
        self.b2, self.gb2 = arena.kernel_view(arena.p32, sb2), arena.kernel_view(arena.g32, sb2)

    def fwd(self, r):
        N = r.shape[0]
        mean = ops.se_pool(r)
        d1 = ops.make_desc(N, 1, 1, self.C, self.hidden, 1, 1, 1, 0)
        d2 = ops.make_desc(N, 1, 1, self.hidden, self.C, 1, 1, 1, 0)
        h = ops.conv_fprop(mean, self.w1, d1, bias=self.b1, act=ACT_RELU)
        logit = ops.conv_fprop(h, self.w2, d2, bias=self.b2, out_fp32=True).view(N, self.C)
        return ops.se_scale_fwd(r, logit), (r, mean, h, logit, d1, d2)

    def bwd(self, rt, tape, g):
        r, mean, h, logit, d1, d2 = tape
        N = r.shape[0]
        dlogit = ops.se_bwd_reduce(g, r, logit)
        ops.colsum_bf16(dlogit.view(N, self.C), self.gb2)
        rt._wgrad_async(lambda: ops.conv_wgrad(h, dlogit, d2, self.gw2), h, dlogit)
        dh = ops.conv_dgrad(dlogit, ops.weight_transpose(self.w2), d2)
        dh = ops.act_bwd(dh, h, ACT_RELU)
        ops.colsum_bf16(dh.view(N, self.hidden), self.gb1)
        rt._wgrad_async(lambda: ops.conv_wgrad(mean, dh, d1, self.gw1), mean, dh)
        dmean = ops.conv_dgrad(dh, ops.weight_transpose(self.w1), d1)
        return ops.se_bwd_dx(g, logit, dmean)


class _Unit(object):
    __slots__ = ('x', 'z', 'y', 'w', 'desc', 'mean', 'invstd', 'scale', 'shift', 'sums', 'conv', 'bn', 'act', 'mask',
                 'sign_sum', 'drop')


class Runtime(object):

    def __init__(self, model, device):
        self.model = model
        self.device = device
        self.arena = Arena(model, device)
        for name, buf in model.named_buffers():
            buf.data = buf.data.to(device)
        self._anchor = self.arena.slots[0].param
        from .models.modules.lp_norm import L1BatchNorm2d
        self._max_c = max([m.num_features for m in model.modules() if isinstance(m, (nn.BatchNorm2d, L1BatchNorm2d))]
                          + [8])
        self._ws = torch.zeros(ops.bn_workspace_floats(self._max_c), device=device, dtype=torch.float32)
        self._wg_stream = torch.cuda.Stream(device=device)
        self._wg_keep = []
        self._fold_cache = {}
        self._want_tape = True
        self.loss_scale_inv = 1.0
        self.grad_bucket_hook = None
        self._bucket_hi = None
        self._bucket_min = 1 << 20
        self.sync_bn_group = None
        self.sync_bn_world = 1
        self._fused_dl = None
        self._ce_dummy = torch.zeros((), device=device, dtype=torch.float32)
        self._build()
        self._setup_transposes()

    def _setup_transposes(self):
        self._p16t, self._wt_jobs, self._wt_tiles = None, None, 0
        convs = [c for c in self.arena.convs if c.kind == 'conv' and c.groups == 1]
        if not convs:
            return
        self._p16t = torch.empty_like(self.arena.p16)
        spec = []
        for c in convs:
            off, n = c.slot.offset, c.slot.numel
            spec.append((off, off, c.K, c.R * c.S, c.C))
            c.wt = self._p16t[off:off + n].view(c.C, c.R * c.S, c.K)
        self._wt_jobs, self._wt_tiles = ops.transpose_jobs(spec, self.device)

    def _transpose_weights(self):
        if self._wt_jobs is not None:
            ops.weight_transpose_batched(self.arena.p16, self._p16t, self._wt_jobs, self._wt_tiles)

    def _build(self):
        raise NotImplementedError

    def _coeffs(self, n):
        return torch.empty(n, device=self.device, dtype=torch.float32)

    input_mean = (0.485, 0.456, 0.406)
    input_std = (0.229, 0.224, 0.225)

    def _input(self, x, mix=None, aug=None):
        if isinstance(aug, ops.Rrc):
            if mix is not None:
                raise B200Error('the resized crop on the device is not combined with MixUp / CutMix')
            if x.dtype != torch.uint8 or x.dim() != 1:
                raise B200Error('the resized crop on the device needs the flat uint8 region buffer; got %s %s'
                                % (x.dtype, tuple(x.shape)))
            OH, OW = aug.size
            return x, (lambda t, cpad, **kw: ops.input_prep_u8_rrc(t, cpad, aug, **kw)), \
                (aug.draws.shape[0], aug.lut.shape[0], OH, OW)
        if x.dtype == torch.uint8:
            if x.dim() != 4 or x.shape[-1] > 4:
                raise B200Error('uint8 network inputs must be NHWC [N, H, W, C<=4]; got %s' % (tuple(x.shape),))
            N, H, W, C = x.shape
            if aug is not None:
                if mix is not None:
                    raise B200Error('batch augmentation on the device is not combined with MixUp / CutMix')

                def prep_aug(t, cpad, s2d=False, border=False, **kw):
                    if s2d:
                        raise B200Error('batch augmentation on the device needs the CIFAR-style 3x3 stem '
                                        '(the space-to-depth stem layouts are not supported)')
                    return ops.input_prep_u8_aug(t, cpad, aug, **kw)
                OH, OW = aug.out_hw or (H, W)
                return x.contiguous(), prep_aug, (N * aug.duplicates, C, OH, OW)
            mean = getattr(self.model, 'input_mean', self.input_mean)
            std = getattr(self.model, 'input_std', self.input_std)
            return x.contiguous(), (lambda t, cpad, **kw: ops.input_prep_u8(t, cpad, mean[:C], std[:C], mix=mix, **kw)), \
                (N, C, H, W)
        if aug is not None:
            raise B200Error('batch augmentation on the device needs the uint8 NHWC images; got %s' % (x.dtype,))
        N, C, H, W = x.shape
        return x.float().contiguous(), (lambda t, cpad, **kw: ops.input_prep(t, cpad, mix=mix, **kw)), (N, C, H, W)

    def _folded(self, conv, bn):
        key = (id(conv), id(bn))
        hit = self._fold_cache.get(key)
        if hit is not None and hit[0] == self.arena.version:
            return hit[1], hit[2]
        m = bn.mod
        coef = self._coeffs(2 * bn.C)
        scale, shift = coef[:bn.C], coef[bn.C:]
        self._eval_coeffs(bn, scale, shift)
        w32 = conv.w32 * scale.view(-1, 1, 1)
        if conv.groups == 1:
            wf = w32.to(torch.bfloat16).contiguous()
        else:
            wf = conv.kernel_weights(w32.contiguous())
        self._fold_cache[key] = (self.arena.version, wf, shift)
        return wf, shift

    def _unit_fwd_folded(self, x, conv, bn, act, residual=None, other=None):
        N, H, W, _ = x.shape
        u = _Unit()
        u.conv, u.bn, u.act, u.x = conv, bn, act, x
        u.desc = conv.desc(N, H, W)
        wf, bf = self._folded(conv, bn)
        if other is not None:
            residual = other.y
        u.z, u.mask = None, None
        u.y = ops.conv_fprop(x, wf, u.desc, bias=bf, residual=residual, act=act)
        return u

    def _unit_fwd(self, x, conv, bn, act, training, tape, residual=None, other=None, drop=None):
        if not training and FOLD_BN_EVAL and not self._want_tape:
            return self._unit_fwd_folded(x, conv, bn, act, residual=residual, other=other)
        N, H, W, _ = x.shape
        u = _Unit()
        u.conv, u.bn, u.act, u.x = conv, bn, act, x
        u.desc = conv.desc(N, H, W)
        u.w = conv.kernel_weights()
        self._conv_and_coeffs(u, x, u.w, training)
        u.drop = drop if training else None
        if u.drop is not None:
            u.mask = torch.empty(ops.bn_act_mask_bytes(u.z.numel() // u.z.shape[-1], u.z.shape[-1]), device=self.device,
                                 dtype=torch.uint8)
            u.y = ops.bn_apply_dropout(u.z, u.scale, u.shift, self.dropout_key, drop[0], drop[1], u.mask)
            return u
        u.mask = None
        if tape and training and act != ACT_NONE and (other is not None or residual is not None):
            u.mask = torch.empty(ops.bn_act_mask_bytes(u.z.numel() // u.z.shape[-1], u.z.shape[-1]), device=self.device,
                                 dtype=torch.uint8)
        if other is not None:
            u.y = ops.bn_apply(u.z, u.scale, u.shift, act, z2=other.z, scale2=other.scale, shift2=other.shift,
                               act_mask=u.mask)
        else:
            u.y = ops.bn_apply(u.z, u.scale, u.shift, act, residual=residual, act_mask=u.mask)
        return u

    def _conv_and_coeffs(self, u, x, w16, training):
        if training and not u.bn.l1 and ops.can_fuse_bn_stats(u.desc.K):
            u.z = ops.conv_fprop(x, w16, u.desc, bn_stats_ws=self._ws)
            self._bn_coeffs(u, training, fused=True)
        else:
            u.z = ops.conv_fprop(x, w16, u.desc)
            self._bn_coeffs(u, training)

    def _eval_coeffs(self, bn, scale, shift):
        m = bn.mod
        if bn.l1:
            ops.bn_l1_eval_coeffs(bn.gamma, bn.beta, m.running_mean, m.running_var, scale, shift)
        else:
            ops.bn_eval_coeffs(bn.gamma, bn.beta, m.running_mean, m.running_var, m.eps, scale, shift)

    def _bn_coeffs(self, u, training, fused=False):
        bn = u.bn
        C = bn.C
        buf = self._coeffs((7 if bn.l1 else 6) * C)
        u.mean, u.invstd, u.scale, u.shift, u.sums = buf[0:C], buf[C:2 * C], buf[2 * C:3 * C], buf[3 * C:4 * C], \
            buf[4 * C:6 * C]
        u.sign_sum = buf[6 * C:7 * C] if bn.l1 else None
        m = bn.mod
        if training and self.sync_bn_world > 1 and bn.l1:
            raise B200Error('SyncBatchNorm is not implemented for L1 BatchNorm')
        if training and self.sync_bn_world > 1 and not fused:
            raise B200Error('SyncBatchNorm on the B200 path needs the conv-epilogue statistics (output channels % 64 == 0)')
        if training and bn.l1:
            ops.bn_l1_stats(u.z, bn.gamma, bn.beta, m.eps, m.momentum, m.running_mean, m.running_var, u.mean,
                            u.invstd, u.sign_sum, u.scale, u.shift, self._ws)
        elif training and fused:
            M = u.z.numel() // C
            if self.sync_bn_world > 1:
                import torch.distributed as dist
                dist.all_reduce(self._ws.view(torch.float64)[:16 * 2 * C], group=self.sync_bn_group)
                M *= self.sync_bn_world
            ops.bn_finalize(M, C, bn.gamma, bn.beta, m.eps, m.momentum, m.running_mean, m.running_var,
                            m.num_batches_tracked, u.mean, u.invstd, u.scale, u.shift, self._ws)
        elif training:
            ops.bn_stats(u.z, bn.gamma, bn.beta, m.eps, m.momentum, m.running_mean, m.running_var,
                         m.num_batches_tracked, u.mean, u.invstd, u.scale, u.shift, self._ws)
        else:
            self._eval_coeffs(bn, u.scale, u.shift)
        bias = getattr(u.conv, 'bias32', None) if u.conv is not None else None
        if bias is not None:
            if training:
                if m.momentum is None:
                    m.running_mean.add_(bias / m.num_batches_tracked.to(torch.float32))
                else:
                    m.running_mean.add_(bias, alpha=float(m.momentum))
            else:
                u.shift.add_(u.scale * bias)

    def _stats_only(self, x, conv, bn, training):
        if not training and FOLD_BN_EVAL and not self._want_tape:
            return self._unit_fwd_folded(x, conv, bn, ACT_NONE)
        N, H, W, _ = x.shape
        u = _Unit()
        u.conv, u.bn, u.act, u.x = conv, bn, ACT_NONE, x
        u.desc = conv.desc(N, H, W)
        u.w = conv.kernel_weights()
        self._conv_and_coeffs(u, x, u.w, training)
        u.y = None
        return u

    def _sync_bn_sums(self, sums):
        import torch.distributed as dist
        dist.all_reduce(sums, group=self.sync_bn_group)
        sums.mul_(1.0 / self.sync_bn_world)

    def _bn_bwd(self, u, dy, y_mask, act, want_g=False):
        bn = u.bn
        drop = getattr(u, 'drop', None)
        if drop is not None:
            ops.bn_bwd_reduce_dropout(dy, u.z, u.mask, drop[1], u.mean, u.invstd, u.sums, bn.dgamma, bn.dbeta, self._ws)
            if self.sync_bn_world > 1:
                self._sync_bn_sums(u.sums)
            return ops.bn_bwd_dx_dropout(dy, u.z, u.mask, drop[1], u.mean, u.invstd, bn.gamma, u.sums), None
        mask = getattr(u, 'mask', None) if y_mask is not None else None
        ops.bn_bwd_reduce(dy, y_mask, u.z, act, u.mean, u.invstd, bn.gamma, bn.beta, u.sums, bn.dgamma, bn.dbeta,
                          self._ws, act_mask=mask)
        if self.sync_bn_world > 1:
            self._sync_bn_sums(u.sums)
        g = torch.empty_like(dy) if want_g else None
        if bn.l1:
            dz = ops.bn_l1_bwd_dx(dy, y_mask, u.z, act, u.mean, u.invstd, u.sign_sum, bn.gamma, bn.beta, u.sums,
                                  g_out=g, act_mask=mask)
        else:
            dz = ops.bn_bwd_dx(dy, y_mask, u.z, act, u.mean, u.invstd, bn.gamma, bn.beta, u.sums, g_out=g,
                               act_mask=mask)
        return dz, g

    def _wgrad_async(self, fn, *operands):
        if self._wg_stream is None:
            fn()
            return
        ev = torch.cuda.Event()
        ev.record()
        self._wg_stream.wait_event(ev)
        with torch.cuda.stream(self._wg_stream):
            fn()
        self._wg_keep.append(operands)

    def _wgrad_join(self):
        if self._wg_stream is not None and self._wg_keep:
            torch.cuda.current_stream().wait_stream(self._wg_stream)
            self._wg_keep = []

    def _buckets_begin(self):
        self._bucket_hi = self.arena.group_end[0] if self.grad_bucket_hook is not None else None

    def _bucket_point(self, lo, force=False):
        if self._bucket_hi is None:
            return
        if lo < self._bucket_hi and (force or self._bucket_hi - lo >= self._bucket_min):
            self.grad_bucket_hook.bucket(lo, self._bucket_hi, self._wg_stream)
            self._bucket_hi = lo

    def _buckets_end(self):
        if self._bucket_hi is None:
            return
        self._bucket_point(0, force=True)
        a = self.arena
        if a.total > a.group_end[0]:
            self.grad_bucket_hook.bucket(a.group_end[0], a.total, None)
        self.grad_bucket_hook.finish()
        self._bucket_hi = None

    @staticmethod
    def _spec_lo(convs):
        return min(c.slot.offset for c in convs)

    def _conv_bwd(self, u, dz, need_dx=True, residual=None):
        conv = u.conv
        if conv.groups == 1:
            self._wgrad_async(lambda: ops.conv_wgrad(u.x, dz, u.desc, conv.g32), u.x, dz)
        else:
            def grouped():
                T = conv.R * conv.S
                N, H, W, _ = u.x.shape
                win = 128 if conv.window else conv.C
                scratch = torch.zeros((conv.K, T, win), device=self.device, dtype=torch.float32)
                ops.conv_wgrad(u.x, dz, conv.desc(N, H, W, wgrad=True), scratch)
                ops.group_wgrad_unpack(scratch, conv.K, T, conv.C, conv.groups, win, conv.g32)
            self._wgrad_async(grouped, u.x, dz)
        if not need_dx:
            return None
        if conv.groups > 1:
            wt = conv.dgrad_weights()
        else:
            wt = conv.wt
        return ops.conv_dgrad(dz, wt, u.desc, residual=residual)

    def _head_build(self, fc, dropout_p=0.0):
        a = self.arena
        sw, sb = a.slot(fc.weight), a.slot(fc.bias)
        self.classes = fc.out_features
        self.classes_pad = _round_up(self.classes, 8)
        self.fc_in = fc.in_features
        self.fc_w16 = a.kernel_view(a.p16, sw)
        self.fc_gw = a.kernel_view(a.g32, sw)
        self.fc_b = a.kernel_view(a.p32, sb)
        self.fc_gb = a.kernel_view(a.g32, sb)
        self.dropout_p = float(dropout_p)

    def _head_fwd(self, h, training, want_tape):
        N = h.shape[0]
        feat = ops.avgpool_fwd(h)
        mask = None
        if training and self.dropout_p > 0:
            keep = 1.0 - self.dropout_p
            mask = (torch.rand(feat.shape, device=self.device) < keep).to(torch.bfloat16) / keep
            feat = feat * mask
        desc = ops.make_desc(N, 1, 1, self.fc_in, self.classes_pad, 1, 1, 1, 0, algo_macs=self.fc_in * self.classes)
        logits = ops.conv_fprop(feat, self.fc_w16, desc, bias=self.fc_b, out_fp32=True).view(N, self.classes_pad)
        out = logits if self.classes_pad == self.classes else logits[:, :self.classes]
        tape = {'feat': feat, 'mask': mask, 'last_shape': tuple(h.shape), 'fc_desc': desc,
                'logits_pad': logits} if want_tape else None
        return out, tape

    def _head_bwd(self, tape, dlogits, dl_bf16=None):
        N = dlogits.shape[0]
        if dl_bf16 is not None:
            dl = dl_bf16
        elif self.classes_pad == self.classes:
            dl = torch.empty((N, self.classes_pad), device=self.device, dtype=torch.bfloat16)
            ops.cast_bf16(dlogits.contiguous().float(), dl)
        else:
            dl = torch.zeros((N, self.classes_pad), device=self.device, dtype=torch.bfloat16)
            dl[:, :self.classes].copy_(dlogits)
        desc = tape['fc_desc']
        dl4 = dl.view(N, 1, 1, self.classes_pad)
        ops.colsum_bf16(dl, self.fc_gb)
        feat = tape['feat']
        self._wgrad_async(lambda: ops.conv_wgrad(feat, dl4, desc, self.fc_gw), feat, dl4)
        wt = ops.weight_transpose(self.fc_w16)
        dfeat = ops.conv_dgrad(dl4, wt, desc)
        if tape['mask'] is not None:
            dfeat = dfeat * tape['mask']
        return ops.avgpool_bwd(dfeat, tape['last_shape'])

    def forward(self, x):
        if x.device.type != 'cuda':
            raise B200Error('B200 runtime needs CUDA inputs (no CPU fallback); got %s' % x.device)
        training = self.model.training
        if torch.is_grad_enabled() and training:
            out = _NetFn.apply(x, self._anchor, self, training)
            out._b200_head = _HeadHandle(self, self._last_logits_pad)
            return out
        logits, _ = self.run_forward(x, training, False)
        return logits

    def run_forward(self, x, training, want_tape, mix=None, aug=None):
        raise NotImplementedError

    def run_backward(self, tape, dlogits, dl_bf16=None):
        raise NotImplementedError

    def train_step(self, x, target, smooth_eps=0.0, upstream=None, mix=None, aug=None):
        if x.device.type != 'cuda':
            raise B200Error('B200 runtime needs CUDA inputs (no CPU fallback); got %s' % x.device)
        n_rows = aug.draws.shape[0] if isinstance(aug, ops.Rrc) else \
            x.shape[0] * (aug.duplicates if aug is not None else 1)
        if target.dtype != torch.int64 or target.dim() != 1 or target.shape[0] != n_rows or not target.is_cuda:
            raise B200Error('train_step: target must be a CUDA int64 vector with one class index per sample')
        logits, tape = self.run_forward(x, True, True, mix=mix, aug=aug)
        pad = tape['head']['logits_pad']
        dev = pad.device
        stats = torch.empty(3, device=dev, dtype=torch.float32)
        rows = torch.empty(2 * pad.shape[0], device=dev, dtype=torch.float32)
        dl = torch.empty(pad.shape, device=dev, dtype=torch.bfloat16)
        up = None
        if upstream is not None:
            up = upstream.reshape(1)
        if mix is not None:
            ops.softmax_ce_mix(pad, target.contiguous(), mix, self.classes, loss=stats, row_loss=rows, dlogits=dl,
                               grad_scale_dev=up)
        else:
            ops.softmax_ce(pad, target.contiguous(), self.classes, smooth_eps, loss=stats, row_loss=rows, dlogits=dl,
                           grad_scale_dev=up)
        self.arena.rebind_grads()
        self.arena.grads_zero = False
        self.run_backward(tape, logits, dl_bf16=dl)
        return logits, stats


class _HeadHandle(object):
    __slots__ = ('rt', 'logits_pad', 'stats')

    def __init__(self, rt, logits_pad):
        self.rt, self.logits_pad, self.stats = rt, logits_pad, None

    def loss(self, logits, target, smooth_eps=0.0):
        return _FusedCE.apply(logits, target, float(smooth_eps or 0.0), self)


class _FusedCE(torch.autograd.Function):

    @staticmethod
    def forward(ctx, logits, target, eps, head):
        pad, rt = head.logits_pad, head.rt
        if logits.data_ptr() != pad.data_ptr() or logits.shape != (pad.shape[0], rt.classes) or \
                target.shape != (pad.shape[0],) or target.dtype != torch.int64 or not target.is_cuda:
            raise B200Error('fused cross-entropy: logits/target do not belong to this forward pass')
        target = target.contiguous()
        stats = torch.empty(3, device=pad.device, dtype=torch.float32)
        rows = torch.empty(2 * pad.shape[0], device=pad.device, dtype=torch.float32)
        ops.softmax_ce(pad, target, rt.classes, eps, loss=stats, row_loss=rows)
        ctx.head, ctx.eps = head, eps
        ctx.save_for_backward(target)
        head.stats = stats
        return stats[0]

    @staticmethod
    def backward(ctx, gout):
        head, (target,) = ctx.head, ctx.saved_tensors
        pad, rt = head.logits_pad, head.rt
        up = gout.reshape(1)
        if up.dtype != torch.float32 or not up.is_contiguous():
            up = up.float().contiguous()
        dl = torch.empty(pad.shape, device=pad.device, dtype=torch.bfloat16)
        ops.softmax_ce(pad, target, rt.classes, ctx.eps, dlogits=dl, grad_scale_dev=up)
        rt._fused_dl = dl
        return rt._ce_dummy.expand(pad.shape[0], rt.classes), None, None, None


class _NetFn(torch.autograd.Function):

    @staticmethod
    def forward(ctx, x, anchor, rt, training):
        logits, tape = rt.run_forward(x.detach(), training, True)
        ctx.rt, ctx.tape = rt, tape
        rt._last_logits_pad = tape['head']['logits_pad']
        return logits

    @staticmethod
    def backward(ctx, dlogits):
        rt, tape = ctx.rt, ctx.tape
        ctx.tape = None
        rt.arena.rebind_grads()
        rt.arena.grads_zero = False
        side, rt._fused_dl = rt._fused_dl, None
        if side is not None and (side.shape[0] != dlogits.shape[0] or side.device != dlogits.device):
            side = None
        if side is not None and not (dlogits.data_ptr() == rt._ce_dummy.data_ptr() and dlogits.stride() == (0, 0)):
            dlogits = dlogits + side[:, :rt.classes].float()
            side = None
        rt.run_backward(tape, dlogits, dl_bf16=side)
        return None, None, None, None


class ResNetRuntime(Runtime):

    def _build(self):
        from .models.resnet import BasicBlock, Bottleneck
        from .models.modules.lp_norm import L1BatchNorm2d
        m, a = self.model, self.arena
        self.imagenet_stem = m.conv1.kernel_size == (7, 7)
        if self.imagenet_stem:
            if m.conv1.stride != (2, 2) or m.conv1.padding != (3, 3) or m.conv1.in_channels != 3:
                raise B200Error('unsupported 7x7 stem geometry')
        elif m.conv1.kernel_size != (3, 3) or m.conv1.stride != (1, 1) or m.conv1.in_channels > 16:
            raise B200Error('unsupported stem geometry')
        self.stem_conv = m.conv1
        s = a.slot(m.conv1.weight)
        self.stem_w32 = a.p32[s.offset:s.offset + s.numel]
        self.stem_g32 = a.g32[s.offset:s.offset + s.numel]
        self.stem_bn = _BN(a, m.bn1)
        self.has_maxpool = isinstance(m.maxpool, nn.MaxPool2d)
        self.blocks = []
        n_drop = 0
        for lname in ('layer1', 'layer2', 'layer3', 'layer4'):
            layer = getattr(m, lname)
            if isinstance(layer, nn.Identity):
                continue
            for blk in layer:
                p = float(blk.dropout.p) if isinstance(blk.dropout, nn.Dropout) else 0.0
                if p != 0 and not isinstance(blk, BasicBlock):
                    raise B200Error('dropout inside residual blocks is not supported on the B200 path')
                spec = {'kind': 'bottleneck' if isinstance(blk, Bottleneck) else 'basic'}
                if not isinstance(blk, (BasicBlock, Bottleneck)):
                    raise B200Error('unknown block type %s' % type(blk).__name__)
                spec['drop'] = None
                if p != 0:
                    if not 0.0 < p < 1.0:
                        raise B200Error('dropout rate %r inside residual blocks: the B200 path needs 0 < p < 1' % p)
                    if isinstance(blk.bn1, L1BatchNorm2d):
                        raise B200Error('dropout with L1 BatchNorm is not supported on the B200 path')
                    spec['drop'] = (n_drop, p)
                    n_drop += 1
                names = ('conv1', 'conv2', 'conv3') if spec['kind'] == 'bottleneck' else ('conv1', 'conv2')
                spec['convs'] = [_Conv(a, getattr(blk, n)) for n in names]
                spec['bns'] = [_BN(a, getattr(blk, n.replace('conv', 'bn'))) for n in names]
                spec['down'] = None
                if blk.downsample is not None:
                    spec['down'] = (_Conv(a, blk.downsample[0]), _BN(a, blk.downsample[1]))
                spec['se'] = _SE(a, blk.residual_block) if blk.residual_block is not None else None
                self.blocks.append(spec)
        self._head_build(m.fc)
        self.dropout_key = torch.zeros(1, device=self.device, dtype=torch.int64) if n_drop else None

    def _stem_fwd(self, x, training, mix=None, aug=None):
        x, prep, (N, Cin, H, W) = self._input(x, mix, aug)
        K = self.stem_conv.out_channels
        st = {}
        if self.imagenet_stem:
            ws = torch.empty((K, 16, 16), device=self.device, dtype=torch.bfloat16)
            ops.stem_weight_to_s2d(self.stem_w32, K, Cin, 16, ws)
            Hs, Ws = H // 2, W // 2
            xs = prep(x, 16, s2d=True, border=True)
            desc = ops.make_desc(N, Hs + 3, Ws, 64, K, 4, 1, 1, 0, P=Hs, Q=Ws,
                                 x_strides=(16, (Ws + 3) * 16, (Hs + 3) * (Ws + 3) * 16), algo_macs=K * 49 * Cin)
            if Ws + 3 <= 128:
                desc = ops.make_desc(N, Hs + 3, Ws + 3, 16, K, 4, 4, 1, 0, P=Hs, Q=Ws, algo_macs=K * 49 * Cin)
        else:
            xs = prep(x, 16, s2d=False)
            ws = torch.zeros((K, 9, 16), device=self.device, dtype=torch.bfloat16)
            ws[:, :, :Cin].copy_(self.stem_w32.view(K, 9, Cin))
            desc = ops.make_desc(N, H, W, 16, K, 3, 3, 1, 1, algo_macs=K * 9 * Cin)
        u = _Unit()
        u.conv, u.bn, u.act, u.x, u.desc = None, self.stem_bn, ACT_RELU, xs, desc
        self._conv_and_coeffs(u, xs, ws, training)
        st['unit'] = u
        if self.has_maxpool:
            u.y = None
            out, st['argmax'] = ops.bn_apply_maxpool(u.z, u.scale, u.shift, ACT_RELU)
        else:
            u.y = ops.bn_apply(u.z, u.scale, u.shift, ACT_RELU)
            out = u.y
        st['cin'] = Cin
        return out, st

    def _stem_bwd(self, st, dy):
        u = st['unit']
        if self.has_maxpool:
            dy = ops.maxpool_bwd(dy, st['argmax'], tuple(u.z.shape))
        dz, _ = self._bn_bwd(u, dy, None, ACT_RELU)
        K, Cin = self.stem_conv.out_channels, st['cin']
        def stem_wgrad():
            if self.imagenet_stem:
                dws = torch.zeros((K, 16, 16), device=self.device, dtype=torch.float32)
                ops.conv_wgrad(u.x, dz, u.desc, dws)
                ops.stem_wgrad_from_s2d(dws, K, Cin, 16, self.stem_g32)
            else:
                dws = torch.zeros((K, 9, 16), device=self.device, dtype=torch.float32)
                ops.conv_wgrad(u.x, dz, u.desc, dws)
                self.stem_g32.view(K, 9, Cin).add_(dws[:, :, :Cin])
        self._wgrad_async(stem_wgrad, u.x, dz)

    def _block_fwd(self, spec, x, training):
        convs, bns = spec['convs'], spec['bns']
        units = []
        h = x
        for i in range(len(convs) - 1):
            u = self._unit_fwd(h, convs[i], bns[i], ACT_RELU, training, True, drop=spec['drop'] if i == 0 else None)
            units.append(u)
            h = u.y
        down, se_tape = None, None
        if spec.get('se') is not None:
            r = x
            if spec['down'] is not None:
                down = self._unit_fwd(x, spec['down'][0], spec['down'][1], ACT_NONE, training, True)
                r = down.y
            r, se_tape = spec['se'].fwd(r)
            last = self._unit_fwd(h, convs[-1], bns[-1], ACT_RELU, training, True, residual=r)
        elif spec['down'] is not None:
            down = self._stats_only(x, spec['down'][0], spec['down'][1], training)
            last = self._unit_fwd(h, convs[-1], bns[-1], ACT_RELU, training, True, other=down)
        else:
            last = self._unit_fwd(h, convs[-1], bns[-1], ACT_RELU, training, True, residual=x)
        units.append(last)
        return last.y, {'units': units, 'down': down, 'se': se_tape}

    def _block_bwd(self, spec, saved, dy):
        units, down = saved['units'], saved['down']
        last = units[-1]
        dz, g = self._bn_bwd(last, dy, last.y, ACT_RELU, want_g=True)
        if saved.get('se') is not None:
            g = spec['se'].bwd(self, saved['se'], g)
        if down is not None:
            dzd, _ = self._bn_bwd(down, g, None, ACT_NONE)
            skip = self._conv_bwd(down, dzd)
        else:
            skip = g
        d = self._conv_bwd(last, dz)
        for u in reversed(units[1:-1]):
            dz, _ = self._bn_bwd(u, d, None, ACT_RELU)
            d = self._conv_bwd(u, dz)
        u = units[0]
        dz, _ = self._bn_bwd(u, d, None, ACT_RELU)
        return self._conv_bwd(u, dz, residual=skip)

    def run_forward(self, x, training, want_tape, mix=None, aug=None):
        self._want_tape = want_tape
        if training:
            self.arena.version += 1
            if self.dropout_key is not None:
                self.dropout_key.random_(-2 ** 63, None)
        h, stem = self._stem_fwd(x, training, mix, aug)
        saved = []
        for spec in self.blocks:
            h, s = self._block_fwd(spec, h, training)
            saved.append(s if want_tape else None)
        out, head = self._head_fwd(h, training, want_tape)
        tape = {'stem': stem, 'blocks': saved, 'head': head} if want_tape else None
        return out, tape

    def run_backward(self, tape, dlogits, dl_bf16=None):
        self._transpose_weights()
        self._buckets_begin()
        d = self._head_bwd(tape['head'], dlogits, dl_bf16)
        for spec, saved in zip(reversed(self.blocks), reversed(tape['blocks'])):
            d = self._block_bwd(spec, saved, d)
            convs = spec['convs'] + ([spec['down'][0]] if spec['down'] is not None else [])
            self._bucket_point(self._spec_lo(convs))
        self._stem_bwd(tape['stem'], d)
        self._wgrad_join()
        self._buckets_end()


class MobileNetRuntime(Runtime):

    def _build(self):
        m, a = self.model, self.arena
        f = m.features
        conv0 = f.conv0[0]
        if conv0.kernel_size != (3, 3) or conv0.in_channels > 16 or conv0.groups != 1:
            raise B200Error('unsupported MobileNet stem')
        self.stem_conv = conv0
        s = a.slot(conv0.weight)
        self.stem_w32 = a.p32[s.offset:s.offset + s.numel]
        self.stem_g32 = a.g32[s.offset:s.offset + s.numel]
        self.stem_bn = _BN(a, f.conv0[1])
        self.blocks = []
        for name, mod in f.named_children():
            if not name.startswith('bottleneck'):
                continue
            if mod.residual_block is not None:
                raise B200Error('residual_block is outside the B200 hot path')
            self.blocks.append({'add_res': mod.add_res, 'units': self._parse_units(list(mod.block))})
        self.blocks.append({'add_res': False, 'units': self._parse_units(list(f.conv1))})
        drop, fc = m.classifier[0], m.classifier[1]
        self._head_build(fc, dropout_p=drop.p if isinstance(drop, nn.Dropout) else 0.0)
        max_c = max(u[1].C for b in self.blocks for u in b['units'] if u[0] == 'dw')
        self._dw_ws = torch.empty(592 * 9 * max_c, device=self.device, dtype=torch.float32)

    def _parse_units(self, layers):
        units, i = [], 0
        while i < len(layers):
            conv, bn = layers[i], layers[i + 1]
            has_act = i + 2 < len(layers) and isinstance(layers[i + 2], (nn.ReLU6, nn.ReLU))
            act = ACT_NONE
            if has_act:
                act = ACT_RELU6 if isinstance(layers[i + 2], nn.ReLU6) else ACT_RELU
            kind = 'dw' if conv.groups > 1 else 'dense'
            units.append((kind, _Conv(self.arena, conv), _BN(self.arena, bn), act))
            i += 3 if has_act else 2
        return units

    def _mb_unit_fwd(self, x, kind, conv, bn, act, training, residual=None):
        N, H, W, _ = x.shape
        u = _Unit()
        u.conv, u.bn, u.act, u.x = conv, bn, act, x
        u.desc = conv.desc(N, H, W)
        if kind == 'dw':
            u.w = None
            u.z = ops.dwconv_fprop(x, conv.w16, u.desc)
            self._bn_coeffs(u, training)
        else:
            u.w = conv.kernel_weights()
            self._conv_and_coeffs(u, x, u.w, training)
        u.y = ops.bn_apply(u.z, u.scale, u.shift, act, residual=residual)
        return u

    def _mb_conv_bwd(self, kind, u, dz, need_dx=True, residual=None):
        if kind == 'dw':
            self._wgrad_async(lambda: ops.dwconv_wgrad(u.x, dz, u.desc, u.conv.g32, self._dw_ws), u.x, dz)
            return ops.dwconv_dgrad(dz, u.conv.w16, u.desc) if need_dx else None
        return self._conv_bwd(u, dz, need_dx=need_dx, residual=residual)

    def _stem_fwd(self, x, training, mix=None, aug=None):
        x, prep, (N, Cin, H, W) = self._input(x, mix, aug)
        K = self.stem_conv.out_channels
        xs = prep(x, 16, s2d=False)
        ws = torch.zeros((K, 9, 16), device=self.device, dtype=torch.bfloat16)
        ws[:, :, :Cin].copy_(self.stem_w32.view(K, 9, Cin))
        st, pad = self.stem_conv.stride[0], self.stem_conv.padding[0]
        act = getattr(self, 'stem_act', ACT_RELU6)
        u = _Unit()
        u.conv, u.bn, u.act, u.x = None, self.stem_bn, act, xs
        u.desc = ops.make_desc(N, H, W, 16, K, 3, 3, st, pad, algo_macs=K * 9 * Cin)
        u.z = ops.conv_fprop(xs, ws, u.desc)
        self._bn_coeffs(u, training)
        u.y = ops.bn_apply(u.z, u.scale, u.shift, act)
        return u.y, {'unit': u, 'cin': Cin}

    def _stem_bwd(self, st, dy):
        u = st['unit']
        dz, _ = self._bn_bwd(u, dy, None, u.act)
        K, Cin = self.stem_conv.out_channels, st['cin']
        def stem_wgrad():
            dws = torch.zeros((K, 9, 16), device=self.device, dtype=torch.float32)
            ops.conv_wgrad(u.x, dz, u.desc, dws)
            self.stem_g32.view(K, 9, Cin).add_(dws[:, :, :Cin])
        self._wgrad_async(stem_wgrad, u.x, dz)

    def run_forward(self, x, training, want_tape, mix=None, aug=None):
        self._want_tape = want_tape
        if training:
            self.arena.version += 1
        h, stem = self._stem_fwd(x, training, mix, aug)
        saved = []
        for spec in self.blocks:
            xin, units = h, []
            for j, (kind, conv, bn, act) in enumerate(spec['units']):
                last = j == len(spec['units']) - 1
                u = self._mb_unit_fwd(h, kind, conv, bn, act, training,
                                      residual=xin if (last and spec['add_res']) else None)
                units.append(u)
                h = u.y
            saved.append(units if want_tape else None)
        out, head = self._head_fwd(h, training, want_tape)
        tape = {'stem': stem, 'blocks': saved, 'head': head} if want_tape else None
        return out, tape

    def run_backward(self, tape, dlogits, dl_bf16=None):
        self._transpose_weights()
        self._buckets_begin()
        d = self._head_bwd(tape['head'], dlogits, dl_bf16)
        for spec, units in zip(reversed(self.blocks), reversed(tape['blocks'])):
            skip = d if spec['add_res'] else None
            for j in range(len(units) - 1, -1, -1):
                kind, _, _, act = spec['units'][j]
                u = units[j]
                dz, _ = self._bn_bwd(u, d, None, act)
                d = self._mb_conv_bwd(kind, u, dz, residual=skip if j == 0 else None)
            dense = [c for k, c, _, _ in spec['units'] if k != 'dw']
            if dense:
                self._bucket_point(self._spec_lo(dense))
        self._stem_bwd(tape['stem'], d)
        self._wgrad_join()
        self._buckets_end()


class MobileNetV1Runtime(MobileNetRuntime):

    def _build(self):
        m, a = self.model, self.arena
        layers = list(m.features)
        conv0, bn0 = layers[0], layers[1]
        if conv0.kernel_size != (3, 3) or conv0.in_channels > 16 or conv0.groups != 1 or conv0.bias is not None:
            raise B200Error('unsupported MobileNet stem')
        self.stem_conv = conv0
        s = a.slot(conv0.weight)
        self.stem_w32 = a.p32[s.offset:s.offset + s.numel]
        self.stem_g32 = a.g32[s.offset:s.offset + s.numel]
        self.stem_bn = _BN(a, bn0)
        self.stem_act = ACT_RELU6 if isinstance(layers[2], nn.ReLU6) else ACT_RELU
        self.blocks = []
        for mod in layers[3:]:
            self.blocks.append({'add_res': False, 'units': self._parse_units(list(mod.components))})
        self._head_build(m.fc, dropout_p=0.0)
        max_c = max(u[1].C for b in self.blocks for u in b['units'] if u[0] == 'dw')
        self._dw_ws = torch.empty(592 * 9 * max_c, device=self.device, dtype=torch.float32)


def enable_sync_batchnorm(model, process_group=None):
    import torch.distributed as dist
    rt = getattr(model, '_b200', None)
    if rt is None:
        raise B200Error('enable_sync_batchnorm needs a model converted by convert_b200')
    if not (dist.is_available() and dist.is_initialized()):
        raise B200Error('enable_sync_batchnorm needs an initialised process group')
    from .models.modules.lp_norm import L1BatchNorm2d
    if any(isinstance(m, L1BatchNorm2d) for m in model.modules()):
        raise NotImplementedError('SyncBatchNorm is not implemented for L1 BatchNorm (bn_norm=\'L1\')')
    rt.sync_bn_group = process_group
    rt.sync_bn_world = dist.get_world_size(process_group)
    return model


def convert_b200(model, device=None):
    from .models.resnet import ResNet
    from .models.mobilenet_v2 import MobileNet_v2
    from .models.mobilenet import MobileNet
    from . import lib
    lib.load()
    if not torch.cuda.is_available():
        raise B200Error('convert_b200 needs a CUDA device: the B200 path has no CPU fallback')
    device = torch.device(device if device is not None else 'cuda:%d' % torch.cuda.current_device())
    if getattr(model, '_b200', None) is not None:
        return model
    if isinstance(model, ResNet):
        rt = ResNetRuntime(model, device)
    elif isinstance(model, MobileNet_v2):
        rt = MobileNetRuntime(model, device)
    elif isinstance(model, MobileNet):
        rt = MobileNetV1Runtime(model, device)
    else:
        raise B200Error('no B200 runtime for model type %s yet' % type(model).__name__)
    object.__setattr__(model, '_b200', rt)
    model.register_load_state_dict_post_hook(lambda module, incompatible: rt.arena.sync_shadow())
    return model
```

### convnet/pytorch_b200/lib.py

```python
import ctypes
import os
import threading

_HERE = os.path.dirname(os.path.abspath(__file__))
LIB_PATH = os.environ.get("B200_LIB_PATH") or os.path.join(_HERE, "libb200conv.so")

ACT_NONE, ACT_RELU, ACT_RELU6 = 0, 1, 2
MIX_NONE, MIX_MIXUP, MIX_CUTMIX = 0, 1, 2


class B200Error(RuntimeError):
    pass


class ConvDesc(ctypes.Structure):
    _fields_ = [(n, ctypes.c_int) for n in
                ("N", "H", "W", "C", "K", "R", "S", "stride", "pad_h", "pad_w", "P", "Q",
                 "x_pixel_stride", "x_row_stride", "x_image_stride", "window")]


class Epilogue(ctypes.Structure):
    _fields_ = [("bias", ctypes.c_void_p), ("residual", ctypes.c_void_p),
                ("act", ctypes.c_int), ("out_fp32", ctypes.c_int), ("bn_stats_workspace", ctypes.c_void_p)]


_vp, _i, _ll, _f, _sz = ctypes.c_void_p, ctypes.c_int, ctypes.c_longlong, ctypes.c_float, ctypes.c_size_t
_dp = ctypes.POINTER(ConvDesc)
_ep = ctypes.POINTER(Epilogue)

SIGNATURES = {
    "b200_conv_fprop": [_dp, _vp, _vp, _vp, _ep, _vp],
    "b200_conv_dgrad": [_dp, _vp, _vp, _vp, _vp, _vp],
    "b200_conv_wgrad": [_dp, _vp, _vp, _vp, _vp, _sz, _vp],
    "b200_conv_wgrad_workspace_bytes": [],
    "b200_dwconv_fprop": [_dp, _vp, _vp, _vp, _vp],
    "b200_dwconv_dgrad": [_dp, _vp, _vp, _vp, _vp],
    "b200_dwconv_wgrad": [_dp, _vp, _vp, _vp, _vp, _sz, _vp],
    "b200_bn_workspace_floats": [_i],
    "b200_bn_act_mask_bytes": [_ll, _i],
    "b200_bn_stats": [_vp, _ll, _i, _vp, _vp, _f, _f, _vp, _vp, _vp, _vp, _vp, _vp, _vp, _vp, _vp],
    "b200_bn_finalize": [_ll, _i, _vp, _vp, _f, _f, _vp, _vp, _vp, _vp, _vp, _vp, _vp, _vp, _vp],
    "b200_bn_eval_coeffs": [_i, _vp, _vp, _vp, _vp, _f, _vp, _vp, _vp],
    "b200_bn_apply": [_vp, _ll, _i, _vp, _vp, _vp, _vp, _vp, _vp, _i, _vp, _vp, _vp],
    "b200_bn_bwd_reduce": [_vp, _vp, _vp, _vp, _ll, _i, _i, _vp, _vp, _vp, _vp, _vp, _vp, _vp, _vp, _vp],
    "b200_bn_bwd_dx": [_vp, _vp, _vp, _vp, _ll, _i, _i, _vp, _vp, _vp, _vp, _vp, _vp, _vp, _vp],
    "b200_bn_l1_stats": [_vp, _ll, _i, _vp, _vp, _f, _f, _vp, _vp, _vp, _vp, _vp, _vp, _vp, _vp, _vp],
    "b200_bn_l1_eval_coeffs": [_i, _vp, _vp, _vp, _vp, _vp, _vp, _vp],
    "b200_bn_l1_bwd_dx": [_vp, _vp, _vp, _vp, _ll, _i, _i, _vp, _vp, _vp, _vp, _vp, _vp, _vp, _vp, _vp],
    "b200_bn_apply_dropout": [_vp, _ll, _i, _vp, _vp, _vp, _i, ctypes.c_uint, _f, _vp, _vp, _vp],
    "b200_bn_bwd_reduce_dropout": [_vp, _vp, _vp, _ll, _i, _f, _vp, _vp, _vp, _vp, _vp, _vp, _vp],
    "b200_bn_bwd_dx_dropout": [_vp, _vp, _vp, _ll, _i, _f, _vp, _vp, _vp, _vp, _vp, _vp],
    "b200_maxpool3x3s2_fwd": [_vp, _i, _i, _i, _i, _vp, _vp, _vp],
    "b200_maxpool3x3s2_bwd": [_vp, _vp, _i, _i, _i, _i, _vp, _vp],
    "b200_bn_apply_maxpool3x3s2": [_vp, _i, _i, _i, _i, _vp, _vp, _i, _vp, _vp, _vp],
    "b200_avgpool_fwd": [_vp, _i, _i, _i, _vp, _vp],
    "b200_avgpool_bwd": [_vp, _i, _i, _i, _vp, _vp],
    "b200_input_prep": [_vp, _i, _i, _i, _i, _i, _i, _vp, _vp],
    "b200_input_prep_u8": [_vp, _i, _i, _i, _i, _i, _i, ctypes.POINTER(ctypes.c_float), ctypes.POINTER(ctypes.c_float),
                           _vp, _vp],
    "b200_input_prep_mix": [_vp, _i, _i, _i, _i, _i, _i, _vp, _vp, _i, _vp, _vp],
    "b200_input_prep_u8_mix": [_vp, _i, _i, _i, _i, _i, _i, ctypes.POINTER(ctypes.c_float),
                               ctypes.POINTER(ctypes.c_float), _vp, _vp, _i, _vp, _vp],
    "b200_input_prep_u8_aug": [_vp, _i, _i, _i, _i, _i, _i, _i, _vp, _vp, _i, _vp, _vp],
    "b200_input_prep_u8_aug_resize": [_vp, _i, _i, _i, _i, _i, _i, _i, _i, _i, _vp, _vp, _i, _vp, _vp],
    "b200_input_prep_u8_rrc": [_vp, _ll, _vp, _vp, _i, _i, _i, _i, _i, _i, _i, _vp, _vp, _vp],
    "b200_weight_transpose": [_vp, _vp, _i, _i, _i, _vp],
    "b200_weight_transpose_batched": [_vp, _vp, _vp, _i, _i, _vp],
    "b200_stem_weight_to_s2d": [_vp, _i, _i, _i, _vp, _vp],
    "b200_stem_wgrad_from_s2d": [_vp, _i, _i, _i, _vp, _vp],
    "b200_cast_f32_to_bf16": [_vp, _vp, _ll, _vp],
    "b200_group_weight_pack": [_vp, _i, _i, _i, _i, _i, _i, _vp, _vp],
    "b200_group_wgrad_unpack": [_vp, _i, _i, _i, _i, _i, _vp, _vp],
    "b200_se_pool": [_vp, _i, _i, _i, _vp, _vp],
    "b200_se_scale_fwd": [_vp, _vp, _i, _i, _i, _vp, _vp],
    "b200_se_bwd_reduce": [_vp, _vp, _vp, _i, _i, _i, _vp, _vp],
    "b200_se_bwd_dx": [_vp, _vp, _vp, _i, _i, _i, _vp, _vp],
    "b200_act_bwd": [_vp, _vp, _ll, _i, _vp, _vp],
    "b200_softmax_ce": [_vp, _vp, _i, _i, _i, _f, _f, _vp, _vp, _vp, _vp, _vp],
    "b200_softmax_ce_mix": [_vp, _vp, _vp, _vp, _i, _i, _i, _f, _vp, _vp, _vp, _vp, _vp],
    "b200_colsum_bf16": [_vp, _i, _i, _vp, _vp],
    "b200_fused_sgd": [_vp, _vp, _vp, _vp, _ll, _ll, _f, _f, _f, _f, _f, _vp, _i, _i, _vp],
    "b200_sumsq": [_vp, _ll, _vp, _vp, _vp],
    "b200_grad_coef": [_vp, _f, _i, _f, _f, _vp, _vp, _vp, _vp],
    "b200_last_error": [],
    "b200_version": [],
    "b200_launch_count": [],
}
_RESTYPES = {"b200_last_error": ctypes.c_char_p, "b200_launch_count": ctypes.c_longlong,
             "b200_conv_wgrad_workspace_bytes": ctypes.c_size_t,
             "b200_bn_workspace_floats": ctypes.c_size_t, "b200_bn_act_mask_bytes": ctypes.c_size_t}

_lib = None
_lock = threading.Lock()


def available():
    return os.path.exists(LIB_PATH)


def load():
    global _lib
    if _lib is not None:
        return _lib
    with _lock:
        if _lib is not None:
            return _lib
        if not os.path.exists(LIB_PATH):
            raise B200Error(
                "libb200conv.so not found at %s -- build it with `python -c 'import __graft_entry__ as g; "
                "g.build()'` or `make -C convnet/pytorch_b200/csrc`. There is no CPU/cuDNN fallback." % LIB_PATH)
        lib = ctypes.CDLL(LIB_PATH)
        for name, argtypes in SIGNATURES.items():
            fn = getattr(lib, name)
            fn.argtypes = argtypes
            fn.restype = _RESTYPES.get(name, ctypes.c_int)
        _lib = lib
    return _lib


def check(rc, what):
    if rc != 0:
        msg = load().b200_last_error()
        raise B200Error("%s failed (rc=%d): %s" % (what, rc, msg.decode() if msg else "?"))


def launch_count():
    return int(load().b200_launch_count())


def ptr(t):
    return None if t is None else t.data_ptr()
```

### convnet/pytorch_b200/ops.py

```python
import ctypes

import torch

from . import lib as _l
from .lib import ACT_NONE, ACT_RELU, ACT_RELU6, ConvDesc, Epilogue

bf16 = torch.bfloat16


def _stream():
    return torch.cuda.current_stream().cuda_stream


_TIMING = None


class _T(object):
    __slots__ = ('name', 'flops', 'nbytes', 'e0')

    def __init__(self, name, flops=0, nbytes=0):
        self.name, self.flops, self.nbytes = name, flops, nbytes

    def __enter__(self):
        if _TIMING is not None:
            self.e0 = torch.cuda.Event(enable_timing=True)
            self.e0.record()
        return self

    def __exit__(self, *exc):
        if _TIMING is not None:
            e1 = torch.cuda.Event(enable_timing=True)
            e1.record()
            _TIMING.append((self.name, self.flops, self.nbytes, self.e0, e1))
        return False


def start_timing():
    global _TIMING
    _TIMING = []


def stop_timing():
    global _TIMING
    rec, _TIMING = _TIMING, None
    torch.cuda.synchronize()
    out = {}
    for name, flops, nbytes, e0, e1 in rec or []:
        c = out.setdefault(name, {'ms': 0.0, 'calls': 0, 'flops': 0, 'bytes': 0})
        c['ms'] += e0.elapsed_time(e1)
        c['calls'] += 1
        c['flops'] += flops
        c['bytes'] += nbytes
    return out


def _conv_flops(d):
    macs = getattr(d, 'algo_macs', None)
    if macs is None:
        macs = d.K * d.R * d.S * d.C
    return 2 * d.N * d.P * d.Q * macs


def _conv_bytes(x, w, out, residual=None):
    n = x.numel() * x.element_size() + w.numel() * w.element_size() + out.numel() * out.element_size()
    if residual is not None:
        n += residual.numel() * residual.element_size()
    return n


def _chk(t, dtype, name):
    if t is None:
        return
    if not t.is_cuda:
        raise _l.B200Error("%s must be a CUDA tensor (no CPU fallback exists)" % name)
    if t.dtype != dtype:
        raise _l.B200Error("%s must be %s, got %s" % (name, dtype, t.dtype))
    if not t.is_contiguous():
        raise _l.B200Error("%s must be contiguous" % name)


def out_size(h, r, stride, pad_lo, pad_hi=None):
    pad_hi = pad_lo if pad_hi is None else pad_hi
    return (h + pad_lo + pad_hi - r) // stride + 1


def make_desc(N, H, W, C, K, R, S, stride, pad, P=None, Q=None, x_strides=(0, 0, 0), algo_macs=None, window=0):
    pad_h, pad_w = (pad, pad) if isinstance(pad, int) else pad
    P = out_size(H, R, stride, pad_h) if P is None else P
    Q = out_size(W, S, stride, pad_w) if Q is None else Q
    d = ConvDesc(N, H, W, C, K, R, S, stride, pad_h, pad_w, P, Q, *x_strides, int(window))
    if algo_macs is not None:
        d.algo_macs = int(algo_macs)
    return d


def can_fuse_bn_stats(K):
    n_tiles = (K + 255) // 256
    block_n = ((K + n_tiles - 1) // n_tiles + 15) // 16 * 16
    return K % 64 == 0 and K % block_n == 0 and 256 % block_n == 0


def conv_fprop(x, w, desc, out=None, bias=None, residual=None, act=ACT_NONE, out_fp32=False, bn_stats_ws=None):
    _chk(x, bf16, "x"); _chk(w, bf16, "w"); _chk(bias, torch.float32, "bias"); _chk(residual, bf16, "residual")
    if out is None:
        out = torch.empty((desc.N, desc.P, desc.Q, desc.K), device=x.device,
                          dtype=torch.float32 if out_fp32 else bf16)
    ep = Epilogue(_l.ptr(bias), _l.ptr(residual), int(act), int(bool(out_fp32)), _l.ptr(bn_stats_ws))
    with _T('conv_fprop', _conv_flops(desc), _conv_bytes(x, w, out, residual)):
        _l.check(_l.load().b200_conv_fprop(ctypes.byref(desc), x.data_ptr(), w.data_ptr(), out.data_ptr(),
                                           ctypes.byref(ep), _stream()), "b200_conv_fprop")
    return out


def conv_dgrad(dy, wt, desc, out=None, residual=None):
    _chk(dy, bf16, "dy"); _chk(wt, bf16, "wt"); _chk(residual, bf16, "residual")
    if out is None:
        out = torch.empty((desc.N, desc.H, desc.W, desc.C), device=dy.device, dtype=bf16)
    with _T('conv_dgrad', _conv_flops(desc), _conv_bytes(dy, wt, out, residual)):
        _l.check(_l.load().b200_conv_dgrad(ctypes.byref(desc), dy.data_ptr(), wt.data_ptr(), out.data_ptr(),
                                           _l.ptr(residual), _stream()), "b200_conv_dgrad")
    return out


_WGRAD_WS = {}


def _wgrad_workspace(device):
    ws = _WGRAD_WS.get(device)
    if ws is None:
        ws = torch.empty(int(_l.load().b200_conv_wgrad_workspace_bytes()), device=device, dtype=torch.uint8)
        _WGRAD_WS[device] = ws
    return ws


def conv_wgrad(x, dy, desc, dw):
    _chk(x, bf16, "x"); _chk(dy, bf16, "dy"); _chk(dw, torch.float32, "dw")
    ws = _wgrad_workspace(x.device)
    with _T('conv_wgrad', _conv_flops(desc), _conv_bytes(x, dy, dw)):
        _l.check(_l.load().b200_conv_wgrad(ctypes.byref(desc), x.data_ptr(), dy.data_ptr(), dw.data_ptr(),
                                           ws.data_ptr(), ws.numel(), _stream()), "b200_conv_wgrad")
    return dw


def dwconv_fprop(x, w, desc, out=None):
    _chk(x, bf16, "x"); _chk(w, bf16, "w")
    if out is None:
        out = torch.empty((desc.N, desc.P, desc.Q, desc.K), device=x.device, dtype=bf16)
    with _T('dw_fprop', 0, _conv_bytes(x, w, out)):
        _l.check(_l.load().b200_dwconv_fprop(ctypes.byref(desc), x.data_ptr(), w.data_ptr(), out.data_ptr(), _stream()),
                 "b200_dwconv_fprop")
    return out


def dwconv_dgrad(dy, w, desc, out=None):
    _chk(dy, bf16, "dy"); _chk(w, bf16, "w")
    if out is None:
        out = torch.empty((desc.N, desc.H, desc.W, desc.C), device=dy.device, dtype=bf16)
    with _T('dw_dgrad', 0, _conv_bytes(dy, w, out)):
        _l.check(_l.load().b200_dwconv_dgrad(ctypes.byref(desc), dy.data_ptr(), w.data_ptr(), out.data_ptr(), _stream()),
                 "b200_dwconv_dgrad")
    return out


def dwconv_wgrad(x, dy, desc, dw, workspace):
    _chk(x, bf16, "x"); _chk(dy, bf16, "dy"); _chk(dw, torch.float32, "dw"); _chk(workspace, torch.float32, "ws")
    with _T('dw_wgrad', 0, _conv_bytes(x, dy, dw)):
        _l.check(_l.load().b200_dwconv_wgrad(ctypes.byref(desc), x.data_ptr(), dy.data_ptr(), dw.data_ptr(),
                                             workspace.data_ptr(), workspace.numel() * 4, _stream()), "b200_dwconv_wgrad")
    return dw


def bn_workspace_floats(C):
    return int(_l.load().b200_bn_workspace_floats(int(C)))


def bn_act_mask_bytes(M, C):
    return (int(M) + 7) // 8 * 8 * (int(C) // 8)


def bn_stats(z, gamma, beta, eps, momentum, running_mean, running_var, nbt, mean, invstd, scale, shift, workspace):
    C = z.shape[-1]
    M = z.numel() // C
    _chk(z, bf16, "z")
    mom = -1.0 if momentum is None else float(momentum)
    with _T('bn_stats', 0, 2 * z.numel()):
        _l.check(_l.load().b200_bn_stats(z.data_ptr(), M, C, _l.ptr(gamma), _l.ptr(beta), float(eps), mom,
                                         _l.ptr(running_mean), _l.ptr(running_var), _l.ptr(nbt), mean.data_ptr(),
                                         invstd.data_ptr(), scale.data_ptr(), shift.data_ptr(), workspace.data_ptr(),
                                         _stream()), "b200_bn_stats")


def bn_finalize(M, C, gamma, beta, eps, momentum, running_mean, running_var, nbt, mean, invstd, scale, shift, workspace):
    mom = -1.0 if momentum is None else float(momentum)
    with _T('bn_stats', 0, 0):
        _l.check(_l.load().b200_bn_finalize(int(M), int(C), _l.ptr(gamma), _l.ptr(beta), float(eps), mom,
                                            _l.ptr(running_mean), _l.ptr(running_var), _l.ptr(nbt), mean.data_ptr(),
                                            invstd.data_ptr(), scale.data_ptr(), shift.data_ptr(),
                                            workspace.data_ptr(), _stream()), "b200_bn_finalize")


def bn_eval_coeffs(gamma, beta, running_mean, running_var, eps, scale, shift):
    C = running_mean.numel()
    _l.check(_l.load().b200_bn_eval_coeffs(C, _l.ptr(gamma), _l.ptr(beta), running_mean.data_ptr(),
                                           running_var.data_ptr(), float(eps), scale.data_ptr(), shift.data_ptr(),
                                           _stream()), "b200_bn_eval_coeffs")


def bn_apply(z, scale, shift, act=ACT_NONE, residual=None, z2=None, scale2=None, shift2=None, out=None, act_mask=None):
    C = z.shape[-1]
    M = z.numel() // C
    _chk(z, bf16, "z"); _chk(residual, bf16, "residual"); _chk(z2, bf16, "z2"); _chk(act_mask, torch.uint8, "act_mask")
    if act_mask is not None and act_mask.numel() != bn_act_mask_bytes(M, C):
        raise _l.B200Error("act_mask must hold bn_act_mask_bytes(M, C) bytes")
    if out is None:
        out = torch.empty_like(z)
    with _T('bn_apply', 0, 2 * z.numel() * (2 + (residual is not None) + (z2 is not None))):
        _l.check(_l.load().b200_bn_apply(z.data_ptr(), M, C, scale.data_ptr(), shift.data_ptr(), _l.ptr(residual),
                                         _l.ptr(z2), _l.ptr(scale2), _l.ptr(shift2), int(act), out.data_ptr(),
                                         _l.ptr(act_mask), _stream()),
                 "b200_bn_apply")
    return out


def bn_bwd_reduce(dy, y, z, act, mean, invstd, gamma, beta, sums, dgamma_acc, dbeta_acc, workspace, act_mask=None):
    C = z.shape[-1]
    M = z.numel() // C
    _chk(dy, bf16, "dy"); _chk(y, bf16, "y"); _chk(z, bf16, "z"); _chk(act_mask, torch.uint8, "act_mask")
    with _T('bn_bwd_reduce', 0, 2 * z.numel() * (2 + (y is not None and act_mask is None))):
        _l.check(_l.load().b200_bn_bwd_reduce(dy.data_ptr(), _l.ptr(y), _l.ptr(act_mask), z.data_ptr(), M, C, int(act),
                                              mean.data_ptr(),
                                              invstd.data_ptr(), _l.ptr(gamma), _l.ptr(beta), sums.data_ptr(),
                                              _l.ptr(dgamma_acc), _l.ptr(dbeta_acc), workspace.data_ptr(), _stream()),
                 "b200_bn_bwd_reduce")


def bn_bwd_dx(dy, y, z, act, mean, invstd, gamma, beta, sums, dz=None, g_out=None, act_mask=None):
    C = z.shape[-1]
    M = z.numel() // C
    if dz is None:
        dz = torch.empty_like(z)
    with _T('bn_bwd_dx', 0, 2 * z.numel() * (3 + (y is not None and act_mask is None) + (g_out is not None))):
        _l.check(_l.load().b200_bn_bwd_dx(dy.data_ptr(), _l.ptr(y), _l.ptr(act_mask), z.data_ptr(), M, C, int(act),
                                          mean.data_ptr(),
                                          invstd.data_ptr(), _l.ptr(gamma), _l.ptr(beta), sums.data_ptr(),
                                          dz.data_ptr(), _l.ptr(g_out), _stream()), "b200_bn_bwd_dx")
    return dz


def bn_l1_stats(z, gamma, beta, eps, momentum, running_mean, running_var, mean, invstd, sign_sum, scale, shift,
                workspace):
    C = z.shape[-1]
    M = z.numel() // C
    _chk(z, bf16, "z")
    with _T('bn_l1_stats', 0, 2 * 2 * z.numel()):
        _l.check(_l.load().b200_bn_l1_stats(z.data_ptr(), M, C, _l.ptr(gamma), _l.ptr(beta), float(eps),
                                            float(momentum), _l.ptr(running_mean), _l.ptr(running_var),
                                            mean.data_ptr(), invstd.data_ptr(), sign_sum.data_ptr(), scale.data_ptr(),
                                            shift.data_ptr(), workspace.data_ptr(), _stream()), "b200_bn_l1_stats")


def bn_l1_eval_coeffs(gamma, beta, running_mean, running_var, scale, shift):
    C = running_mean.numel()
    _l.check(_l.load().b200_bn_l1_eval_coeffs(C, _l.ptr(gamma), _l.ptr(beta), running_mean.data_ptr(),
                                              running_var.data_ptr(), scale.data_ptr(), shift.data_ptr(), _stream()),
             "b200_bn_l1_eval_coeffs")


def bn_l1_bwd_dx(dy, y, z, act, mean, invstd, sign_sum, gamma, beta, sums, dz=None, g_out=None, act_mask=None):
    C = z.shape[-1]
    M = z.numel() // C
    _chk(dy, bf16, "dy"); _chk(y, bf16, "y"); _chk(z, bf16, "z"); _chk(act_mask, torch.uint8, "act_mask")
    if dz is None:
        dz = torch.empty_like(z)
    with _T('bn_l1_bwd_dx', 0, 2 * z.numel() * (3 + (y is not None and act_mask is None) + (g_out is not None))):
        _l.check(_l.load().b200_bn_l1_bwd_dx(dy.data_ptr(), _l.ptr(y), _l.ptr(act_mask), z.data_ptr(), M, C, int(act),
                                             mean.data_ptr(), invstd.data_ptr(), sign_sum.data_ptr(), _l.ptr(gamma),
                                             _l.ptr(beta), sums.data_ptr(), dz.data_ptr(), _l.ptr(g_out), _stream()),
                 "b200_bn_l1_bwd_dx")
    return dz


def dropout_threshold(p):
    p = float(p)
    if not 0.0 <= p < 1.0:
        raise _l.B200Error('dropout rate must be in [0, 1), got %r' % p)
    return int(round((1.0 - p) * 65536.0)), float(ctypes.c_float(1.0 / (1.0 - p)).value)


def bn_apply_dropout(z, scale, shift, key, layer, p, act_mask, out=None):
    C = z.shape[-1]
    M = z.numel() // C
    _chk(z, bf16, "z"); _chk(key, torch.int64, "key"); _chk(act_mask, torch.uint8, "act_mask")
    if act_mask is None or act_mask.numel() != bn_act_mask_bytes(M, C):
        raise _l.B200Error("act_mask must hold bn_act_mask_bytes(M, C) bytes")
    T, c = dropout_threshold(p)
    if out is None:
        out = torch.empty_like(z)
    with _T('bn_apply_dropout', 0, 2 * 2 * z.numel() + act_mask.numel()):
        _l.check(_l.load().b200_bn_apply_dropout(z.data_ptr(), M, C, scale.data_ptr(), shift.data_ptr(), key.data_ptr(),
                                                 int(layer), T, c, out.data_ptr(), act_mask.data_ptr(), _stream()),
                 "b200_bn_apply_dropout")
    return out


def bn_bwd_reduce_dropout(dy, z, act_mask, p, mean, invstd, sums, dgamma_acc, dbeta_acc, workspace):
    C = z.shape[-1]
    M = z.numel() // C
    _chk(dy, bf16, "dy"); _chk(z, bf16, "z"); _chk(act_mask, torch.uint8, "act_mask")
    _, c = dropout_threshold(p)
    with _T('bn_bwd_reduce_dropout', 0, 2 * 2 * z.numel() + act_mask.numel()):
        _l.check(_l.load().b200_bn_bwd_reduce_dropout(dy.data_ptr(), act_mask.data_ptr(), z.data_ptr(), M, C, c,
                                                      mean.data_ptr(), invstd.data_ptr(), sums.data_ptr(),
                                                      _l.ptr(dgamma_acc), _l.ptr(dbeta_acc), workspace.data_ptr(),
                                                      _stream()), "b200_bn_bwd_reduce_dropout")


def bn_bwd_dx_dropout(dy, z, act_mask, p, mean, invstd, gamma, sums, dz=None):
    C = z.shape[-1]
    M = z.numel() // C
    _chk(dy, bf16, "dy"); _chk(z, bf16, "z"); _chk(act_mask, torch.uint8, "act_mask")
    _, c = dropout_threshold(p)
    if dz is None:
        dz = torch.empty_like(z)
    with _T('bn_bwd_dx_dropout', 0, 2 * 3 * z.numel() + act_mask.numel()):
        _l.check(_l.load().b200_bn_bwd_dx_dropout(dy.data_ptr(), act_mask.data_ptr(), z.data_ptr(), M, C, c,
                                                  mean.data_ptr(), invstd.data_ptr(), _l.ptr(gamma), sums.data_ptr(),
                                                  dz.data_ptr(), _stream()), "b200_bn_bwd_dx_dropout")
    return dz


def _out(out, shape, dtype, device, name):
    if out is None:
        return torch.empty(shape, device=device, dtype=dtype)
    _chk(out, dtype, name)
    if tuple(out.shape) != tuple(shape):
        raise _l.B200Error("%s has shape %s, expected %s" % (name, tuple(out.shape), tuple(shape)))
    return out


def maxpool_fwd(x, want_argmax=True, out=None, argmax_out=None):
    N, H, W, C = x.shape
    OH, OW = (H - 1) // 2 + 1, (W - 1) // 2 + 1
    y = _out(out, (N, OH, OW, C), bf16, x.device, "out")
    am = _out(argmax_out, (N, OH, OW, C), torch.uint8, x.device, "argmax_out") if want_argmax else None
    with _T('maxpool_fwd', 0, 2 * x.numel() + 3 * y.numel()):
        _l.check(_l.load().b200_maxpool3x3s2_fwd(x.data_ptr(), N, H, W, C, y.data_ptr(), _l.ptr(am), _stream()),
                 "b200_maxpool3x3s2_fwd")
    return y, am


def maxpool_bwd(dy, argmax, in_shape, out=None):
    N, H, W, C = in_shape
    dx = _out(out, in_shape, bf16, dy.device, "out")
    with _T('maxpool_bwd', 0, 2 * dx.numel() + 3 * dy.numel()):
        _l.check(_l.load().b200_maxpool3x3s2_bwd(dy.data_ptr(), argmax.data_ptr(), N, H, W, C, dx.data_ptr(), _stream()),
                 "b200_maxpool3x3s2_bwd")
    return dx


def bn_apply_maxpool(z, scale, shift, act=ACT_RELU, want_argmax=True, out=None, argmax_out=None):
    N, H, W, C = z.shape
    _chk(z, bf16, "z")
    OH, OW = (H - 1) // 2 + 1, (W - 1) // 2 + 1
    y = _out(out, (N, OH, OW, C), bf16, z.device, "out")
    am = _out(argmax_out, (N, OH, OW, C), torch.uint8, z.device, "argmax_out") if want_argmax else None
    with _T('bn_apply', 0, 2 * z.numel() + 3 * y.numel()):
        _l.check(_l.load().b200_bn_apply_maxpool3x3s2(z.data_ptr(), N, H, W, C, scale.data_ptr(), shift.data_ptr(),
                                                      int(act), y.data_ptr(), _l.ptr(am), _stream()),
                 "b200_bn_apply_maxpool3x3s2")
    return y, am


def avgpool_fwd(x, out=None):
    N, H, W, C = x.shape
    y = _out(out, (N, 1, 1, C), bf16, x.device, "out")
    with _T('avgpool', 0, 2 * x.numel()):
        _l.check(_l.load().b200_avgpool_fwd(x.data_ptr(), N, H * W, C, y.data_ptr(), _stream()), "b200_avgpool_fwd")
    return y


def avgpool_bwd(dy, in_shape, out=None):
    N, H, W, C = in_shape
    dx = _out(out, in_shape, bf16, dy.device, "out")
    with _T('avgpool', 0, 2 * dx.numel()):
        _l.check(_l.load().b200_avgpool_bwd(dy.data_ptr(), N, H * W, C, dx.data_ptr(), _stream()), "b200_avgpool_bwd")
    return dx


def se_pool(r, out=None):
    N, H, W, C = r.shape
    out = _out(out, (N, 1, 1, C), bf16, r.device, "out")
    with _T('se', 0, 2 * r.numel()):
        _l.check(_l.load().b200_se_pool(r.data_ptr(), N, H * W, C, out.data_ptr(), _stream()), "b200_se_pool")
    return out


def se_scale_fwd(r, logit, out=None):
    N, H, W, C = r.shape
    _chk(logit, torch.float32, "logit")
    out = _out(out, r.shape, bf16, r.device, "out")
    with _T('se', 0, 4 * r.numel()):
        _l.check(_l.load().b200_se_scale_fwd(r.data_ptr(), logit.data_ptr(), N, H * W, C, out.data_ptr(), _stream()),
                 "b200_se_scale_fwd")
    return out


def se_bwd_reduce(g, r, logit, out=None):
    N, H, W, C = r.shape
    out = _out(out, (N, 1, 1, C), bf16, r.device, "out")
    with _T('se', 0, 4 * r.numel()):
        _l.check(_l.load().b200_se_bwd_reduce(g.data_ptr(), r.data_ptr(), logit.data_ptr(), N, H * W, C, out.data_ptr(),
                                              _stream()), "b200_se_bwd_reduce")
    return out


def se_bwd_dx(g, logit, dmean, out=None):
    N, H, W, C = g.shape
    out = _out(out, g.shape, bf16, g.device, "out")
    with _T('se', 0, 4 * g.numel()):
        _l.check(_l.load().b200_se_bwd_dx(g.data_ptr(), logit.data_ptr(), dmean.data_ptr(), N, H * W, C, out.data_ptr(),
                                          _stream()), "b200_se_bwd_dx")
    return out


def act_bwd(dy, y, act, out=None):
    out = _out(out, dy.shape, bf16, dy.device, "out")
    _l.check(_l.load().b200_act_bwd(dy.data_ptr(), y.data_ptr(), dy.numel(), int(act), out.data_ptr(), _stream()),
             "b200_act_bwd")
    return out


class Mix(object):
    __slots__ = ('perm', 'params', 'kind')

    def __init__(self, perm, params, kind):
        self.perm, self.params, self.kind = perm, params, int(kind)

    @property
    def lam(self):
        return self.params[:1].view(torch.float32)


def _check_mix(mix, n):
    _chk(mix.perm, torch.int64, "perm"); _chk(mix.params, torch.int32, "mix params")
    if mix.perm.numel() != n or mix.params.numel() < 5 or mix.kind not in (_l.MIX_MIXUP, _l.MIX_CUTMIX):
        raise _l.B200Error("mix: perm must have one entry per sample, params 5 int32, kind MIXUP or CUTMIX")


def _prep_out(N, H, W, cpad, s2d, border, device, out):
    if s2d and border:
        shape = (N, H // 2 + 3, W // 2 + 3, cpad)
    else:
        shape = (N, H // 2, W // 2, cpad) if s2d else (N, H, W, cpad)
    if out is None:
        return torch.empty(shape, device=device, dtype=bf16)
    _chk(out, bf16, "out")
    if tuple(out.shape) != shape:
        raise _l.B200Error("input_prep: out has shape %s, expected %s" % (tuple(out.shape), shape))
    return out


def input_prep(x_nchw, cpad, s2d=False, border=False, mix=None, out=None):
    _chk(x_nchw, torch.float32, "x")
    N, C, H, W = x_nchw.shape
    out = _prep_out(N, H, W, cpad, s2d, border, x_nchw.device, out)
    mode = (2 if border else 1) if s2d else 0
    if mix is None:
        with _T('input_prep', 0, 4 * x_nchw.numel() + 2 * out.numel()):
            _l.check(_l.load().b200_input_prep(x_nchw.data_ptr(), N, C, H, W, cpad, mode, out.data_ptr(),
                                               _stream()), "b200_input_prep")
        return out
    _check_mix(mix, N)
    reads = 2 if mix.kind == _l.MIX_MIXUP else 1
    with _T('input_prep', 0, 4 * reads * x_nchw.numel() + 2 * out.numel()):
        _l.check(_l.load().b200_input_prep_mix(x_nchw.data_ptr(), N, C, H, W, cpad, mode, mix.perm.data_ptr(),
                                               mix.params.data_ptr(), mix.kind, out.data_ptr(), _stream()),
                 "b200_input_prep_mix")
    return out


def u8_norm_coeffs(mean, std):
    scale = [1.0 / (255.0 * float(s)) for s in std]
    bias = [-float(m) / float(s) for m, s in zip(mean, std)]
    return scale, bias


def input_prep_u8(x_nhwc_u8, cpad, mean, std, s2d=False, border=False, mix=None, out=None):
    _chk(x_nhwc_u8, torch.uint8, "x")
    N, H, W, C = x_nhwc_u8.shape
    out = _prep_out(N, H, W, cpad, s2d, border, x_nhwc_u8.device, out)
    sc, bi = u8_norm_coeffs(mean, std)
    scale = (ctypes.c_float * C)(*sc)
    bias = (ctypes.c_float * C)(*bi)
    mode = (2 if border else 1) if s2d else 0
    if mix is None:
        with _T('input_prep', 0, x_nhwc_u8.numel() + 2 * out.numel()):
            _l.check(_l.load().b200_input_prep_u8(x_nhwc_u8.data_ptr(), N, C, H, W, cpad, mode, scale, bias,
                                                  out.data_ptr(), _stream()), "b200_input_prep_u8")
        return out
    _check_mix(mix, N)
    reads = 2 if mix.kind == _l.MIX_MIXUP else 1
    with _T('input_prep', 0, reads * x_nhwc_u8.numel() + 2 * out.numel()):
        _l.check(_l.load().b200_input_prep_u8_mix(x_nhwc_u8.data_ptr(), N, C, H, W, cpad, mode, scale, bias,
                                                  mix.perm.data_ptr(), mix.params.data_ptr(), mix.kind, out.data_ptr(),
                                                  _stream()), "b200_input_prep_u8_mix")
    return out


class Aug(object):
    __slots__ = ('params', 'lut', 'duplicates', 'pad', 'out_hw')

    def __init__(self, params, lut, duplicates, pad, out_hw=None):
        self.params, self.lut, self.duplicates, self.pad = params, lut, int(duplicates), int(pad)
        self.out_hw = (int(out_hw[0]), int(out_hw[1])) if out_hw is not None else None

    @property
    def holes(self):
        return (self.params.shape[-1] - 3) // 4

    @property
    def key(self):
        return ('aug', tuple(self.params.shape), self.duplicates, self.pad, self.lut.data_ptr(), self.out_hw)

    @property
    def tables(self):
        return (self.params,)

    def with_tables(self, tables):
        return Aug(tables[0], self.lut, self.duplicates, self.pad, self.out_hw)


class Rrc(object):
    __slots__ = ('index', 'draws', 'lut', 'duplicates', 'size', 'host')

    def __init__(self, index, draws, lut, duplicates, size, host):
        self.index, self.draws, self.lut, self.duplicates = index, draws, lut, int(duplicates)
        self.size, self.host = (int(size[0]), int(size[1])), host

    @property
    def key(self):
        return ('rrc', tuple(self.index.shape), self.duplicates, self.size, self.lut.data_ptr())

    @property
    def tables(self):
        return (self.index, self.draws)

    def with_tables(self, tables):
        return Rrc(tables[0], tables[1], self.lut, self.duplicates, self.size, self.host)


def check_rrc_tables(index, draws, nbytes, C, D):
    if index.dim() != 2 or index.shape[1] != 3 or draws.dim() != 2 or draws.shape[1] != 5 \
            or draws.shape[0] != index.shape[0] * D:
        raise _l.B200Error("input_prep_u8_rrc: index must be [B, 3] and draws [B*D, 5]; got %s, %s (D=%d)"
                           % (tuple(index.shape), tuple(draws.shape), D))
    off, h, w = (index[:, k].long() for k in range(3))
    if bool(((off < 0) | (h < 1) | (w < 1) | (h > 65535) | (w > 65535) | (off + h * w * C > nbytes)).any()):
        raise _l.B200Error("input_prep_u8_rrc: a region lies outside the %d-byte buffer" % nbytes)
    d = draws.long()
    rh, rw = h.repeat_interleave(D), w.repeat_interleave(D)
    if bool(((d[:, 0] < 0) | (d[:, 1] < 0) | (d[:, 2] < 1) | (d[:, 3] < 1) | (d[:, 0] + d[:, 2] > rh)
             | (d[:, 1] + d[:, 3] > rw) | (d[:, 4] < 0) | (d[:, 4] > 1)).any()):
        raise _l.B200Error("input_prep_u8_rrc: a crop box lies outside its region")


def input_prep_u8_rrc(regions, cpad, rrc, s2d=False, border=False, out=None):
    _chk(regions, torch.uint8, "regions"); _chk(rrc.index, torch.int64, "index"); _chk(rrc.draws, torch.int32, "draws")
    _chk(rrc.lut, torch.float32, "lut")
    if s2d and not border:
        raise _l.B200Error("input_prep_u8_rrc: the space-to-depth layout needs the border (mode 2)")
    if regions.dim() != 1 or rrc.lut.dim() != 2 or rrc.lut.shape[1] != 256:
        raise _l.B200Error("input_prep_u8_rrc: regions must be a flat uint8 buffer and lut fp32 [C, 256]")
    C, D = rrc.lut.shape[0], rrc.duplicates
    (OH, OW), B = rrc.size, rrc.index.shape[0]
    h_index, h_draws, nbytes = rrc.host
    if nbytes > regions.numel() or tuple(h_index.shape) != tuple(rrc.index.shape) \
            or tuple(h_draws.shape) != tuple(rrc.draws.shape):
        raise _l.B200Error("input_prep_u8_rrc: host tables do not describe the device tables and buffer")
    check_rrc_tables(h_index, h_draws, nbytes, C, D)
    out = _prep_out(B * D, OH, OW, cpad, s2d, border, regions.device, out)
    mode = 2 if s2d else 0
    nbytes_read = int((h_index[:, 1].long() * h_index[:, 2].long()).sum()) * C
    with _T('input_prep', 0, nbytes_read + 8 * rrc.index.numel() + 4 * rrc.draws.numel() + 2 * out.numel()):
        _l.check(_l.load().b200_input_prep_u8_rrc(regions.data_ptr(), regions.numel(), rrc.index.data_ptr(),
                                                  rrc.draws.data_ptr(), B, D, C, OH, OW, cpad, mode,
                                                  rrc.lut.data_ptr(), out.data_ptr(), _stream()),
                 "b200_input_prep_u8_rrc")
    return out


def input_prep_u8_aug(x_nhwc_u8, cpad, aug, out=None):
    _chk(x_nhwc_u8, torch.uint8, "x"); _chk(aug.params, torch.int16, "aug params"); _chk(aug.lut, torch.float32, "lut")
    N, H, W, C = x_nhwc_u8.shape
    D = aug.duplicates
    if aug.params.dim() != 2 or aug.params.shape[0] != N * D or (aug.params.shape[1] - 3) % 4 != 0 \
            or tuple(aug.lut.shape) != (C, 256):
        raise _l.B200Error("input_prep_u8_aug: params must be int16 [N*D, 3+4*holes] and lut fp32 [C, 256]; got %s, %s"
                           % (tuple(aug.params.shape), tuple(aug.lut.shape)))
    if aug.out_hw is not None:
        OH, OW = aug.out_hw
        out = _prep_out(N * D, OH, OW, cpad, False, False, x_nhwc_u8.device, out)
        with _T('input_prep', 0, D * x_nhwc_u8.numel() + 2 * aug.params.numel() + 2 * out.numel()):
            _l.check(_l.load().b200_input_prep_u8_aug_resize(x_nhwc_u8.data_ptr(), N, D, C, H, W, OH, OW, cpad, aug.pad,
                                                             aug.lut.data_ptr(), aug.params.data_ptr(), aug.holes,
                                                             out.data_ptr(), _stream()),
                     "b200_input_prep_u8_aug_resize")
        return out
    out = _prep_out(N * D, H, W, cpad, False, False, x_nhwc_u8.device, out)
    with _T('input_prep', 0, x_nhwc_u8.numel() + 2 * aug.params.numel() + 2 * out.numel()):
        _l.check(_l.load().b200_input_prep_u8_aug(x_nhwc_u8.data_ptr(), N, D, C, H, W, cpad, aug.pad,
                                                  aug.lut.data_ptr(), aug.params.data_ptr(), aug.holes,
                                                  out.data_ptr(), _stream()), "b200_input_prep_u8_aug")
    return out


def weight_transpose(w, out=None):
    K, T, C = w.shape
    if out is None:
        out = torch.empty((C, T, K), device=w.device, dtype=bf16)
    with _T('weight_transpose', 0, 4 * w.numel()):
        _l.check(_l.load().b200_weight_transpose(w.data_ptr(), out.data_ptr(), K, T, C, _stream()),
                 "b200_weight_transpose")
    return out


def transpose_jobs(shapes_and_offsets, device):
    rows, tiles = [], 0
    for src_off, dst_off, K, T, C in shapes_and_offsets:
        rows.append([src_off, dst_off, K, T, C, tiles])
        tiles += T * ((K + 31) // 32) * ((C + 31) // 32)
    return torch.tensor(rows, dtype=torch.int32, device=device), tiles


def weight_transpose_batched(src_base, dst_base, jobs, total_tiles):
    _chk(src_base, bf16, "src_base"); _chk(dst_base, bf16, "dst_base"); _chk(jobs, torch.int32, "jobs")
    with _T('weight_transpose', 0, 4 * src_base.numel()):
        _l.check(_l.load().b200_weight_transpose_batched(src_base.data_ptr(), dst_base.data_ptr(), jobs.data_ptr(),
                                                         int(jobs.shape[0]), int(total_tiles), _stream()),
                 "b200_weight_transpose_batched")
    return dst_base


def stem_weight_to_s2d(w_f32, K, C, cpad, out):
    _l.check(_l.load().b200_stem_weight_to_s2d(w_f32.data_ptr(), K, C, cpad, out.data_ptr(), _stream()),
             "b200_stem_weight_to_s2d")
    return out


def stem_wgrad_from_s2d(dw_s2d, K, C, cpad, dw):
    _l.check(_l.load().b200_stem_wgrad_from_s2d(dw_s2d.data_ptr(), K, C, cpad, dw.data_ptr(), _stream()),
             "b200_stem_wgrad_from_s2d")
    return dw


def group_weight_pack(w32_grouped, K, T, C, groups, window, transpose=False, out=None):
    if out is None:
        out = torch.empty((C if transpose else K, T, window), device=w32_grouped.device, dtype=bf16)
    with _T('weight_transpose', 0, 2 * out.numel()):
        _l.check(_l.load().b200_group_weight_pack(w32_grouped.data_ptr(), K, T, C, groups, int(window), int(bool(transpose)),
                                                  out.data_ptr(), _stream()), "b200_group_weight_pack")
    return out


def group_wgrad_unpack(dw_win, K, T, C, groups, window, dw_grouped):
    with _T('weight_transpose', 0, 4 * dw_grouped.numel()):
        _l.check(_l.load().b200_group_wgrad_unpack(dw_win.data_ptr(), K, T, C, groups, int(window), dw_grouped.data_ptr(),
                                                   _stream()), "b200_group_wgrad_unpack")
    return dw_grouped


def cast_bf16(src, dst):
    with _T('cast', 0, 6 * src.numel()):
        _l.check(_l.load().b200_cast_f32_to_bf16(src.data_ptr(), dst.data_ptr(), src.numel(), _stream()),
                 "b200_cast_f32_to_bf16")
    return dst


def softmax_ce(logits, target, classes, smooth_eps, loss=None, row_loss=None, dlogits=None, grad_scale=1.0,
               grad_scale_dev=None):
    if loss is not None and (loss.numel() < 3 or row_loss is None or row_loss.numel() < 2 * logits.shape[0]):
        raise _l.B200Error("softmax_ce: loss needs 3 floats and row_loss 2*B floats")
    B, ld = logits.shape
    _chk(logits, torch.float32, "logits"); _chk(target, torch.int64, "target"); _chk(dlogits, bf16, "dlogits")
    _chk(loss, torch.float32, "loss"); _chk(row_loss, torch.float32, "row_loss")
    _chk(grad_scale_dev, torch.float32, "grad_scale_dev")
    with _T('softmax_ce', 0, 4 * logits.numel()):
        _l.check(_l.load().b200_softmax_ce(logits.data_ptr(), target.data_ptr(), B, int(classes), int(ld),
                                           float(smooth_eps or 0.0), float(grad_scale), _l.ptr(grad_scale_dev),
                                           _l.ptr(loss), _l.ptr(row_loss), _l.ptr(dlogits), _stream()),
                 "b200_softmax_ce")


def softmax_ce_mix(logits, target, mix, classes, loss=None, row_loss=None, dlogits=None, grad_scale=1.0,
                   grad_scale_dev=None):
    if loss is not None and (loss.numel() < 3 or row_loss is None or row_loss.numel() < 2 * logits.shape[0]):
        raise _l.B200Error("softmax_ce_mix: loss needs 3 floats and row_loss 2*B floats")
    B, ld = logits.shape
    _chk(logits, torch.float32, "logits"); _chk(target, torch.int64, "target"); _chk(dlogits, bf16, "dlogits")
    _chk(loss, torch.float32, "loss"); _chk(row_loss, torch.float32, "row_loss")
    _chk(grad_scale_dev, torch.float32, "grad_scale_dev")
    _check_mix(mix, B)
    with _T('softmax_ce', 0, 4 * logits.numel()):
        _l.check(_l.load().b200_softmax_ce_mix(logits.data_ptr(), target.data_ptr(), mix.perm.data_ptr(),
                                               mix.lam.data_ptr(), B, int(classes), int(ld), float(grad_scale),
                                               _l.ptr(grad_scale_dev), _l.ptr(loss), _l.ptr(row_loss), _l.ptr(dlogits),
                                               _stream()), "b200_softmax_ce_mix")


def colsum_bf16(m, out):
    B, K = m.shape
    _l.check(_l.load().b200_colsum_bf16(m.data_ptr(), B, K, out.data_ptr(), _stream()), "b200_colsum_bf16")


def fused_sgd(p32, g32, m32, p16, n, wd_count, lr, momentum, dampening, weight_decay, inv_scale, clip_coef,
              first_step, zero_grad=False):
    with _T('fused_sgd', 0, (26 if zero_grad else 22) * int(n)):
        _l.check(_l.load().b200_fused_sgd(p32.data_ptr(), g32.data_ptr(), _l.ptr(m32), _l.ptr(p16), int(n),
                                          int(wd_count), float(lr), float(momentum), float(dampening),
                                          float(weight_decay), float(inv_scale), _l.ptr(clip_coef), int(bool(first_step)),
                                          int(bool(zero_grad)), _stream()), "b200_fused_sgd")


def sumsq(g, n, out, workspace):
    _l.check(_l.load().b200_sumsq(g.data_ptr(), int(n), out.data_ptr(), workspace.data_ptr(), _stream()),
             "b200_sumsq")


def grad_coef(sumsq_t, inv_scale, mode, max_norm, momentum, state, coef_out, norm_out):
    _l.check(_l.load().b200_grad_coef(sumsq_t.data_ptr(), float(inv_scale), int(mode), float(max_norm),
                                      float(momentum), _l.ptr(state), coef_out.data_ptr(), _l.ptr(norm_out),
                                      _stream()), "b200_grad_coef")
```

### include/b200conv.h

```cpp
#ifndef B200CONV_H_
#define B200CONV_H_

#include <stddef.h>
#include <stdint.h>

#ifdef __cplusplus
extern "C" {
#endif

typedef void* b200_stream_t;

#define B200_OK 0
#define B200_ERR_INVALID (-1)
#define B200_ERR_UNSUPPORTED (-2)
#define B200_ERR_CUDA (-3)

#define B200_ACT_NONE 0
#define B200_ACT_RELU 1
#define B200_ACT_RELU6 2

typedef struct {
  int N, H, W, C;
  int K, R, S;
  int stride;
  int pad_h, pad_w;
  int P, Q;
  int x_pixel_stride, x_row_stride, x_image_stride;
  int window;
} b200_conv_desc;

typedef struct {
  const float* bias;
  const void* residual;
  int act;
  int out_fp32;
  float* bn_stats_workspace;
} b200_epilogue;

const char* b200_last_error(void);
int b200_version(void);
long long b200_launch_count(void);

int b200_conv_fprop(const b200_conv_desc* d, const void* x, const void* w, void* y,
                    const b200_epilogue* ep, b200_stream_t stream);
int b200_conv_dgrad(const b200_conv_desc* d, const void* dy, const void* wt, void* dx,
                    const void* residual, b200_stream_t stream);
size_t b200_conv_wgrad_workspace_bytes(void);
int b200_conv_wgrad(const b200_conv_desc* d, const void* x, const void* dy, float* dw,
                    void* workspace, size_t workspace_bytes, b200_stream_t stream);

int b200_dwconv_fprop(const b200_conv_desc* d, const void* x, const void* w, void* y, b200_stream_t stream);
int b200_dwconv_dgrad(const b200_conv_desc* d, const void* dy, const void* w, void* dx, b200_stream_t stream);
int b200_dwconv_wgrad(const b200_conv_desc* d, const void* x, const void* dy, float* dw,
                      float* workspace, size_t workspace_bytes, b200_stream_t stream);

size_t b200_bn_workspace_floats(int C);
int b200_bn_stats(const void* z, long long M, int C, const float* gamma, const float* beta,
                  float eps, float momentum, float* running_mean, float* running_var,
                  long long* num_batches_tracked, float* mean, float* invstd, float* scale, float* shift,
                  float* workspace, b200_stream_t stream);
int b200_bn_finalize(long long M, int C, const float* gamma, const float* beta, float eps, float momentum,
                     float* running_mean, float* running_var, long long* num_batches_tracked, float* mean,
                     float* invstd, float* scale, float* shift, float* workspace, b200_stream_t stream);
int b200_bn_eval_coeffs(int C, const float* gamma, const float* beta, const float* running_mean,
                        const float* running_var, float eps, float* scale, float* shift, b200_stream_t stream);
size_t b200_bn_act_mask_bytes(long long M, int C);
int b200_bn_apply(const void* z, long long M, int C, const float* scale, const float* shift,
                  const void* residual, const void* z2, const float* scale2, const float* shift2,
                  int act, void* y, uint8_t* act_mask, b200_stream_t stream);
int b200_bn_bwd_reduce(const void* dy, const void* y, const uint8_t* act_mask, const void* z, long long M, int C, int act,
                       const float* mean, const float* invstd, const float* gamma, const float* beta,
                       float* sums, float* dgamma_acc, float* dbeta_acc, float* workspace, b200_stream_t stream);
int b200_bn_bwd_dx(const void* dy, const void* y, const uint8_t* act_mask, const void* z, long long M, int C, int act,
                   const float* mean, const float* invstd, const float* gamma, const float* beta,
                   const float* sums, void* dz, void* g_out, b200_stream_t stream);

int b200_bn_l1_stats(const void* z, long long M, int C, const float* gamma, const float* beta, float eps,
                     float momentum, float* running_mean, float* running_var, float* mean, float* invstd,
                     float* sign_sum, float* scale, float* shift, float* workspace, b200_stream_t stream);
int b200_bn_l1_eval_coeffs(int C, const float* gamma, const float* beta, const float* running_mean,
                           const float* running_var, float* scale, float* shift, b200_stream_t stream);
int b200_bn_l1_bwd_dx(const void* dy, const void* y, const uint8_t* act_mask, const void* z, long long M, int C,
                      int act, const float* mean, const float* invstd, const float* sign_sum, const float* gamma,
                      const float* beta, const float* sums, void* dz, void* g_out, b200_stream_t stream);

int b200_bn_apply_dropout(const void* z, long long M, int C, const float* scale, const float* shift, const uint64_t* key,
                          int layer, unsigned T, float c, void* y, uint8_t* act_mask, b200_stream_t stream);
int b200_bn_bwd_reduce_dropout(const void* dy, const uint8_t* act_mask, const void* z, long long M, int C, float c,
                               const float* mean, const float* invstd, float* sums, float* dgamma_acc, float* dbeta_acc,
                               float* workspace, b200_stream_t stream);
int b200_bn_bwd_dx_dropout(const void* dy, const uint8_t* act_mask, const void* z, long long M, int C, float c,
                           const float* mean, const float* invstd, const float* gamma, const float* sums, void* dz,
                           b200_stream_t stream);

int b200_maxpool3x3s2_fwd(const void* x, int N, int H, int W, int C, void* y, uint8_t* argmax, b200_stream_t stream);
int b200_maxpool3x3s2_bwd(const void* dy, const uint8_t* argmax, int N, int H, int W, int C, void* dx, b200_stream_t stream);
int b200_bn_apply_maxpool3x3s2(const void* z, int N, int H, int W, int C, const float* scale, const float* shift,
                               int act, void* y, uint8_t* argmax, b200_stream_t stream);
int b200_avgpool_fwd(const void* x, int N, int HW, int C, void* y, b200_stream_t stream);
int b200_avgpool_bwd(const void* dy, int N, int HW, int C, void* dx, b200_stream_t stream);

int b200_input_prep(const float* x_nchw, int N, int C, int H, int W, int Cpad, int mode, void* out, b200_stream_t stream);
int b200_input_prep_u8(const uint8_t* x_nhwc, int N, int C, int H, int W, int Cpad, int mode, const float* scale_host,
                       const float* bias_host, void* out, b200_stream_t stream);
#define B200_MIX_NONE 0
#define B200_MIX_MIXUP 1
#define B200_MIX_CUTMIX 2
typedef struct {
  float lam;
  int r0, r1, c0, c1;
} b200_mix_params;
int b200_input_prep_mix(const float* x_nchw, int N, int C, int H, int W, int Cpad, int mode, const long long* perm,
                        const b200_mix_params* params, int kind, void* out, b200_stream_t stream);
int b200_input_prep_u8_mix(const uint8_t* x_nhwc, int N, int C, int H, int W, int Cpad, int mode, const float* scale_host,
                           const float* bias_host, const long long* perm, const b200_mix_params* params, int kind,
                           void* out, b200_stream_t stream);
int b200_input_prep_u8_aug(const uint8_t* x_nhwc, int N, int D, int C, int H, int W, int Cpad, int pad, const float* lut,
                           const int16_t* params, int holes, void* out, b200_stream_t stream);
int b200_input_prep_u8_aug_resize(const uint8_t* x_nhwc, int N, int D, int C, int H, int W, int OH, int OW, int Cpad,
                                  int pad, const float* lut, const int16_t* params, int holes, void* out,
                                  b200_stream_t stream);
int b200_input_prep_u8_rrc(const uint8_t* regions, long long region_bytes, const long long* index, const int* draws,
                           int B, int D, int C, int OH, int OW, int Cpad, int mode, const float* lut, void* out,
                           b200_stream_t stream);
int b200_weight_transpose(const void* src, void* dst, int K, int T, int C, b200_stream_t stream);
int b200_weight_transpose_batched(const void* src_base, void* dst_base, const int* jobs, int njobs, int total_tiles,
                                  b200_stream_t stream);
int b200_stem_weight_to_s2d(const float* w, int K, int C, int Cpad, void* w_s2d, b200_stream_t stream);
int b200_stem_wgrad_from_s2d(const float* dw_s2d, int K, int C, int Cpad, float* dw, b200_stream_t stream);
int b200_cast_f32_to_bf16(const float* src, void* dst, long long n, b200_stream_t stream);
int b200_group_weight_pack(const float* w_grouped, int K, int T, int C, int groups, int window, int transpose,
                           void* out_bf16, b200_stream_t stream);
int b200_group_wgrad_unpack(const float* dw_win, int K, int T, int C, int groups, int window, float* dw_grouped,
                            b200_stream_t stream);

int b200_se_pool(const void* r, int N, int HW, int C, void* mean_bf16, b200_stream_t stream);
int b200_se_scale_fwd(const void* r, const float* logit, int N, int HW, int C, void* out, b200_stream_t stream);
int b200_se_bwd_reduce(const void* g, const void* r, const float* logit, int N, int HW, int C, void* dlogit_bf16,
                       b200_stream_t stream);
int b200_se_bwd_dx(const void* g, const float* logit, const void* dmean_bf16, int N, int HW, int C, void* dr,
                   b200_stream_t stream);
int b200_act_bwd(const void* dy, const void* y, long long n, int act, void* dx, b200_stream_t stream);

int b200_softmax_ce(const float* logits, const long long* target, int B, int classes, int ld, float smooth_eps,
                    float grad_scale, const float* grad_scale_dev, float* loss, float* row_loss, void* dlogits_bf16,
                    b200_stream_t stream);
int b200_softmax_ce_mix(const float* logits, const long long* target, const long long* perm, const float* lam_dev, int B,
                        int classes, int ld, float grad_scale, const float* grad_scale_dev, float* loss, float* row_loss,
                        void* dlogits_bf16, b200_stream_t stream);
int b200_colsum_bf16(const void* m, int B, int K, float* out, b200_stream_t stream);

int b200_fused_sgd(float* p32, float* g32, float* m32, void* p16, long long n, long long wd_count,
                   float lr, float momentum, float dampening, float weight_decay, float inv_scale,
                   const float* clip_coef_dev, int first_step, int zero_grad, b200_stream_t stream);
int b200_sumsq(const float* g, long long n, float* out, float* workspace, b200_stream_t stream);
int b200_grad_coef(const float* sumsq, float inv_scale, int mode, float max_norm, float momentum,
                   float* state, float* coef_out, float* norm_out, b200_stream_t stream);

#ifdef __cplusplus
}
#endif
#endif
```

Before: 6701.

## Fuse BN backward reduction into conv dgrad epilogue

```diff
diff --git a/convnet/pytorch_b200/csrc/bn_common.cuh b/convnet/pytorch_b200/csrc/bn_common.cuh
--- a/convnet/pytorch_b200/csrc/bn_common.cuh
+++ b/convnet/pytorch_b200/csrc/bn_common.cuh
@@ -129,7 +129,7 @@
   return m;
 }
 
-static int check_c(int C, const char* who) {
+static inline int check_c(int C, const char* who) {
   B200_REQUIRE(C > 0 && C % 8 == 0 && C <= kBnMaxC, B200_ERR_UNSUPPORTED,
                "%s: C=%d must be a multiple of 8 and <= %d", who, C, kBnMaxC);
   return B200_OK;
diff --git a/convnet/pytorch_b200/csrc/conv.cu b/convnet/pytorch_b200/csrc/conv.cu
--- a/convnet/pytorch_b200/csrc/conv.cu
+++ b/convnet/pytorch_b200/csrc/conv.cu
@@ -1,3 +1,4 @@
+#include "bn_common.cuh"
 #include "common.cuh"
 #include "host.h"
 #include <stdlib.h>
@@ -37,6 +38,10 @@
   int window;
   uint32_t epi_bytes;
   double* stats;
+  float* bn_partial;
+  const float *bn_mean, *bn_invstd, *bn_gamma, *bn_beta;
+  int bn_act, bn_bits;
+  uint32_t bn_mask_bytes;
   void* out;
   const void* res;
   const float* bias;
@@ -83,6 +88,15 @@
   }
 }
 
+__device__ __forceinline__ void flush_bn_bwd(const IgemmParams& p, float* dst, int n, const float (&s1)[2],
+                                             const float (&s2)[2]) {
+#pragma unroll
+  for (int e = 0; e < 2; ++e) {
+    dst[e] += s1[e] * __ldg(p.bn_invstd + n + e);
+    dst[p.N_total + e] += s2[e];
+  }
+}
+
 template <int KS, int SZ>
 __device__ __forceinline__ void igemm_stage_mma(float (&acc)[2][SZ], uint64_t da, uint64_t db, uint32_t a_half,
                                                 uint32_t scale0) {
@@ -99,6 +113,7 @@
 __global__ void __launch_bounds__(kThreads, 1)
 conv_igemm_kernel(const __grid_constant__ CUtensorMap tmA, const __grid_constant__ CUtensorMap tmB,
                   const __grid_constant__ CUtensorMap tmC, const __grid_constant__ CUtensorMap tmR,
+                  const __grid_constant__ CUtensorMap tmZ, const __grid_constant__ CUtensorMap tmM,
                   const __grid_constant__ IgemmParams p) {
   extern __shared__ uint8_t smem_raw[];
   __shared__ __align__(8) uint64_t full_bar[kMaxStages];
@@ -129,6 +144,10 @@
     if (p.tma_store) {
       prefetch_tmap(&tmC);
       if (p.res != nullptr) prefetch_tmap(&tmR);
+      if (p.bn_partial != nullptr) {
+        prefetch_tmap(&tmZ);
+        if (p.bn_bits) prefetch_tmap(&tmM);
+      }
     }
   }
   __syncthreads();
@@ -197,11 +216,29 @@
   const uint32_t bstat_addr = smem_u32(sBstat);
   constexpr int nbox = BN / 64;
   uint8_t* epi_w = epi + wg * p.epi_bytes;
+  uint8_t* z_w = epi + (2 + wg) * p.epi_bytes;
+  const uint32_t* mask_w = reinterpret_cast<const uint32_t*>(epi + 4 * p.epi_bytes + wg * p.bn_mask_bytes);
   const int st_col = wt % BN;
   constexpr int st_rows = BN;
   const int st_row0 = (wt / BN) * st_rows;
   int st_ntile = -1;
   float st_s1 = 0.f, st_s2 = 0.f;
+  const int bb_col = 2 * (wt % (BN / 2));
+  const int bb_row0 = (wt / (BN / 2)) * (BN / 2);
+  float bb_s1[2] = {0.f, 0.f}, bb_s2[2] = {0.f, 0.f};
+  float bn_mu[2] = {0.f, 0.f}, bn_sc[2] = {0.f, 0.f}, bn_sh[2] = {0.f, 0.f};
+  float* bn_dst = nullptr;
+  if constexpr (BN == 64 || BN == 128) {
+    if (p.bn_partial != nullptr) {
+      bn_dst = p.bn_partial +
+               static_cast<size_t>((blockIdx.x * 2 + wg) * (2 * kTileM / BN) + wt / (BN / 2)) * 2 * p.N_total + bb_col;
+      for (int nt = 0; nt < p.n_tiles; ++nt)
+        for (int e = 0; e < 2; ++e) {
+          bn_dst[nt * BN + e] = 0.f;
+          bn_dst[p.N_total + nt * BN + e] = 0.f;
+        }
+    }
+  }
   const int IJ = p.I * p.J;
   if (p.b_stationary && walk_first < walk_end) mbar_wait(&bstat_bar, 0);
 
@@ -216,11 +253,19 @@
     if (p.tma_store) {
       if (leader && mine > 0) bulk_wait_group_read0();
       named_bar_sync(1 + wg, 128);
-      if (leader && p.res != nullptr) {
+      if (leader && (p.res != nullptr || p.bn_partial != nullptr)) {
         fence_proxy_async();
-        mbar_arrive_expect_tx(&res_bar[wg], static_cast<uint32_t>(nbox) * kTileM * 128u);
-        for (int b = 0; b < nbox; ++b)
-          tma_load_2d(&tmR, &res_bar[wg], epi_w + b * (kTileM * 128), nbase + b * 64, m_tile * kTileM);
+        const uint32_t tile_bytes = static_cast<uint32_t>(nbox) * kTileM * 128u;
+        mbar_arrive_expect_tx(&res_bar[wg], (p.res != nullptr ? tile_bytes : 0u) +
+                                                (p.bn_partial != nullptr ? tile_bytes + p.bn_mask_bytes : 0u));
+        if (p.res != nullptr)
+          for (int b = 0; b < nbox; ++b)
+            tma_load_2d(&tmR, &res_bar[wg], epi_w + b * (kTileM * 128), nbase + b * 64, m_tile * kTileM);
+        if (p.bn_partial != nullptr) {
+          for (int b = 0; b < nbox; ++b)
+            tma_load_2d(&tmZ, &res_bar[wg], z_w + b * (kTileM * 128), nbase + b * 64, m_tile * kTileM);
+          if (p.bn_bits) tma_load_2d(&tmM, &res_bar[wg], const_cast<uint32_t*>(mask_w), nbase / 4, m_tile * (kTileM / 4));
+        }
       }
     }
 
@@ -254,7 +299,7 @@
 
     if (p.tma_store) {
       if constexpr (BN % 64 == 0) {
-        if (p.res != nullptr) mbar_wait(&res_bar[wg], static_cast<uint32_t>(mine & 1));
+        if (p.res != nullptr || p.bn_partial != nullptr) mbar_wait(&res_bar[wg], static_cast<uint32_t>(mine & 1));
 #pragma unroll
         for (int j = 0; j < BN / 2; j += 4) {
           const int c = 2 * j + c_lo;
@@ -301,6 +346,50 @@
             st_s1 += s1;
             st_s2 += s2;
           }
+          if (p.bn_partial != nullptr) {
+            if (st_ntile != n_tile) {
+              if (st_ntile >= 0) {
+                flush_bn_bwd(p, bn_dst + st_ntile * BN, st_ntile * BN + bb_col, bb_s1, bb_s2);
+                bb_s1[0] = bb_s1[1] = bb_s2[0] = bb_s2[1] = 0.f;
+              }
+              st_ntile = n_tile;
+#pragma unroll
+              for (int e = 0; e < 2; ++e) {
+                const int n = nbase + bb_col + e;
+                bn_mu[e] = __ldg(p.bn_mean + n);
+                bn_sc[e] = (p.bn_gamma != nullptr ? __ldg(p.bn_gamma + n) : 1.f) * __ldg(p.bn_invstd + n);
+                bn_sh[e] = (p.bn_beta != nullptr ? __ldg(p.bn_beta + n) : 0.f) - bn_mu[e] * bn_sc[e];
+              }
+            }
+            float s1[2] = {0.f, 0.f}, s2[2] = {0.f, 0.f};
+#pragma unroll 2
+            for (int q = bb_row0 / 4; q < (bb_row0 + BN / 2) / 4; ++q) {
+              const uint32_t bits = p.bn_bits ? mask_w[q * (BN / 8) + (bb_col >> 3)] >> (bb_col & 7) : 0u;
+#pragma unroll
+              for (int u = 0; u < 4; ++u) {
+                const uint32_t off = staged_offset(4 * q + u, bb_col, kTileM * 128);
+                const float2 dd = unpack_bf16x2(*reinterpret_cast<const uint32_t*>(epi_w + off));
+                const float2 zp = unpack_bf16x2(*reinterpret_cast<const uint32_t*>(z_w + off));
+                const float gv[2] = {dd.x, dd.y}, zv[2] = {zp.x, zp.y};
+#pragma unroll
+                for (int e = 0; e < 2; ++e) {
+                  float g = gv[e];
+                  if (p.bn_bits) {
+                    if (((bits >> (8 * u + e)) & 1u) == 0u) g = 0.f;
+                  } else if (p.bn_act != B200_ACT_NONE && act_mask(fmaf(zv[e], bn_sc[e], bn_sh[e]), p.bn_act) == 0.f) {
+                    g = 0.f;
+                  }
+                  s1[e] = fmaf(g, zv[e] - bn_mu[e], s1[e]);
+                  s2[e] += g;
+                }
+              }
+            }
+#pragma unroll
+            for (int e = 0; e < 2; ++e) {
+              bb_s1[e] += s1[e];
+              bb_s2[e] += s2[e];
+            }
+          }
         }
       }
       continue;
@@ -321,8 +410,11 @@
         for (int j = 0; j < BN / 2; j += 4) store_pair(p, acc[mh][j + 2 * h], acc[mh][j + 2 * h + 1], off, nbase + 2 * j + c_lo);
       }
   }
-  if constexpr (BN == 64 || BN == 128)
+  if constexpr (BN == 64 || BN == 128) {
     if (p.stats != nullptr && st_ntile >= 0) flush_bn_stats(p.stats, p.N_total, st_ntile * BN, st_col, st_s1, st_s2);
+    if (p.bn_partial != nullptr && st_ntile >= 0)
+      flush_bn_bwd(p, bn_dst + st_ntile * BN, st_ntile * BN + bb_col, bb_s1, bb_s2);
+  }
   if (p.tma_store && leader) bulk_wait_group0();
 }
 
@@ -608,6 +700,14 @@
   const void* res; const float* bias; int act, out_fp32;
   double* stats;
   int window;
+  struct IgemmBn* bn;
+};
+
+struct IgemmBn {
+  const void* z; const uint8_t* mask; int act;
+  const float *mean, *invstd, *gamma, *beta;
+  float* partial; int max_rows;
+  int rows;
 };
 
 template <int... Is>
@@ -660,10 +760,15 @@
   p.tma_store = (L.os == 1 && !L.out_fp32 && (p.block_n % 64) == 0 && (L.Nout % p.block_n) == 0 && L.ldo == L.Nout &&
                  L.OH == L.I && L.OW == L.J && L.oh0 == 0 && L.ow0 == 0) ? 1 : 0;
   const int epi_bytes = p.tma_store ? kTileM * p.block_n * 2 : 0;
-  const int epi_total = 2 * epi_bytes;
+  const bool bn_fused = L.bn != nullptr && p.tma_store && (p.block_n == 64 || p.block_n == 128) &&
+                        sm_count() * 2 * (2 * kTileM / p.block_n) <= L.bn->max_rows;
+  if (L.bn != nullptr) L.bn->rows = 0;
+  const int mask_bytes = (bn_fused && L.bn->mask != nullptr) ? (kTileM / 4) * (p.block_n / 8) * 4 : 0;
+  const int epi_total = bn_fused ? 2 * (2 * epi_bytes + mask_bytes) : 2 * epi_bytes;
   const int b_all = L.ntaps * p.c_chunks * (int)p.b_bytes;
   int bstat_bytes = 0;
-  if (p.n_tiles == 1 && !L.window && (p.a_bytes % 1024) == 0 && (p.b_bytes % 1024) == 0 && b_all <= 64 * 1024) {
+  if (p.n_tiles == 1 && !L.window && (p.a_bytes % 1024) == 0 && (p.b_bytes % 1024) == 0 && b_all <= 64 * 1024 &&
+      kSmemBudgetMax - epi_total - b_all >= 2 * (int)p.a_bytes) {
     p.b_stationary = 1;
     bstat_bytes = b_all;
     stage = p.a_bytes;
@@ -689,9 +794,21 @@
   p.num_stages = (kSmemBudgetMax - epi_total - bstat_bytes) / (int)stage;
   if (p.num_stages > kMaxStages) p.num_stages = kMaxStages;
   if (p.num_stages < 2) p.num_stages = 2;
+  if (bn_fused && p.num_stages < 3) {
+    IgemmLaunch L0 = L;
+    L0.bn = nullptr;
+    return launch_igemm(L0, stream);
+  }
   p.OH = L.OH; p.OW = L.OW; p.os = L.os; p.oh0 = L.oh0; p.ow0 = L.ow0; p.ldo = L.ldo;
   p.act = L.act; p.out_fp32 = L.out_fp32; p.out = L.out; p.res = L.res; p.bias = L.bias;
   p.stats = L.stats;
+  if (bn_fused) {
+    p.bn_partial = L.bn->partial;
+    p.bn_mean = L.bn->mean; p.bn_invstd = L.bn->invstd; p.bn_gamma = L.bn->gamma; p.bn_beta = L.bn->beta;
+    p.bn_act = L.bn->act;
+    p.bn_bits = L.bn->mask != nullptr ? 1 : 0;
+    p.bn_mask_bytes = (uint32_t)mask_bytes;
+  }
   if (L.stats != nullptr)
     B200_REQUIRE(p.tma_store && (128 % p.block_n) == 0 && L.res == nullptr && L.bias == nullptr && L.act == 0,
                  B200_ERR_UNSUPPORTED, "conv_fprop: fused BN statistics need a dense bf16 output with K %% 64 == 0 "
@@ -713,14 +830,25 @@
   rc = encode_tiled(&tmB, L.wmat, 3, {L.window ? L.window : L.SC, L.wtaps, L.Nout}, {p.ck, 1, p.block_n}, "igemm B");
   if (rc) return rc;
 
-  CUtensorMap tmC, tmR;
+  CUtensorMap tmC, tmR, tmZ, tmM;
   memset(&tmC, 0, sizeof(tmC));
   memset(&tmR, 0, sizeof(tmR));
+  memset(&tmZ, 0, sizeof(tmZ));
+  memset(&tmM, 0, sizeof(tmM));
   if (p.tma_store) {
     rc = encode_tiled(&tmC, L.out, 2, {L.ldo, p.M_total}, {64, kTileM}, "igemm output");
     if (rc) return rc;
     if (L.res != nullptr) {
       rc = encode_tiled(&tmR, L.res, 2, {L.ldo, p.M_total}, {64, kTileM}, "igemm residual");
+      if (rc) return rc;
+    }
+  }
+  if (bn_fused) {
+    rc = encode_tiled(&tmZ, L.bn->z, 2, {L.ldo, p.M_total}, {64, kTileM}, "igemm BN z");
+    if (rc) return rc;
+    if (p.bn_bits) {
+      rc = encode_tiled(&tmM, L.bn->mask, 2, {L.ldo / 4, (p.M_total + 7) / 8 * 2}, {p.block_n / 4, kTileM / 4},
+                        "igemm BN mask", false);
       if (rc) return rc;
     }
   }
@@ -735,13 +863,14 @@
                                       : (total_tiles + grid - 1) / grid;
     fprintf(stderr, "[igemm] M=%d C=%d N=%d taps=%d os=%d block_n=%d n_tiles=%d m_tiles=%d ck=%d k_iters=%d stages=%d "
             "tma_store=%d plain_a=%d bstat=%d own=%d out_fp32=%d bias=%d res=%d act=%d stats=%d grid=%d max_tiles=%d "
-            "smem=%d\n",
+            "smem=%d bn_bwd=%d\n",
             p.M_total, L.SC, L.Nout, L.ntaps, L.os, p.block_n, p.n_tiles, p.m_tiles, p.ck, L.ntaps * p.c_chunks,
             p.num_stages, p.tma_store, p.plain_a, p.b_stationary, p.own_ntile, p.out_fp32, L.bias != nullptr,
-            L.res != nullptr, p.act, L.stats != nullptr, grid, max_tiles, smem_bytes);
-  }
-  b200::launch(kfn, grid, kThreads, smem_bytes, stream, tmA, tmB, tmC, tmR, p);
+            L.res != nullptr, p.act, L.stats != nullptr, grid, max_tiles, smem_bytes, bn_fused ? 1 + p.bn_bits : 0);
+  }
+  b200::launch(kfn, grid, kThreads, smem_bytes, stream, tmA, tmB, tmC, tmR, tmZ, tmM, p);
   B200_CHECK_LAUNCH("conv_igemm_kernel");
+  if (bn_fused) L.bn->rows = grid * 2 * (2 * kTileM / p.block_n);
   return B200_OK;
 }
 
@@ -803,11 +932,10 @@
   return launch_igemm(L, (cudaStream_t)stream);
 }
 
-extern "C" int b200_conv_dgrad(const b200_conv_desc* d, const void* dy, const void* wt, void* dx,
-                               const void* residual, b200_stream_t stream_) {
+static int conv_dgrad(const b200_conv_desc* d, const void* dy, const void* wt, void* dx, const void* residual,
+                      IgemmBn* bn, cudaStream_t stream) {
   int rc = check_desc(d);
   if (rc) return rc;
-  cudaStream_t stream = (cudaStream_t)stream_;
   B200_REQUIRE(dy && wt && dx, B200_ERR_INVALID, "conv_dgrad: null pointer");
   B200_REQUIRE(d->K % 8 == 0, B200_ERR_UNSUPPORTED, "conv_dgrad: K=%d must be a multiple of 8", d->K);
   const int st = d->stride;
@@ -868,9 +996,44 @@
       L.out = dx; L.OH = d->H; L.OW = d->W; L.os = st; L.oh0 = ph; L.ow0 = pw; L.ldo = d->C;
       L.res = residual; L.bias = nullptr; L.act = 0; L.out_fp32 = 0;
       L.window = d->window;
+      L.bn = st == 1 ? bn : nullptr;
       rc = launch_igemm(L, stream);
       if (rc) return rc;
     }
+  return B200_OK;
+}
+
+extern "C" int b200_conv_dgrad(const b200_conv_desc* d, const void* dy, const void* wt, void* dx,
+                               const void* residual, b200_stream_t stream) {
+  return conv_dgrad(d, dy, wt, dx, residual, nullptr, (cudaStream_t)stream);
+}
+
+extern "C" int b200_conv_dgrad_bn_reduce(const b200_conv_desc* d, const void* dy, const void* wt, void* dx,
+                                         const void* residual, const void* y, const uint8_t* act_mask, const void* z,
+                                         long long M, int C, int act, const float* mean, const float* invstd,
+                                         const float* gamma, const float* beta, float* sums, float* dgamma_acc,
+                                         float* dbeta_acc, float* workspace, b200_stream_t stream_) {
+  cudaStream_t stream = (cudaStream_t)stream_;
+  const int src = (act == B200_ACT_NONE) ? 0 : (act_mask != nullptr ? 2 : (y != nullptr ? 1 : 0));
+  const bool fusable = d != nullptr && residual != nullptr && src != 1 && z && mean && invstd && sums && workspace &&
+                       C > 0 && C % 8 == 0 &&
+                       C <= kBnMaxC && (src != 2 || C % 32 == 0) && C == d->C &&
+                       M == static_cast<long long>(d->N) * d->H * d->W;
+  IgemmBn bn;
+  memset(&bn, 0, sizeof(bn));
+  if (fusable) {
+    bn.z = z; bn.mask = src == 2 ? act_mask : nullptr; bn.act = act;
+    bn.mean = mean; bn.invstd = invstd; bn.gamma = gamma; bn.beta = beta;
+    bn.partial = workspace + kAccumFloats;
+    bn.max_rows = kMaxPartialBlocks * kBnMaxC / C;
+  }
+  int rc = conv_dgrad(d, dy, wt, dx, residual, fusable ? &bn : nullptr, stream);
+  if (rc) return rc;
+  if (bn.rows == 0)
+    return b200_bn_bwd_reduce(dx, y, act_mask, z, M, C, act, mean, invstd, gamma, beta, sums, dgamma_acc, dbeta_acc,
+                              workspace, stream_);
+  launch_bwd_reduce_final(bn.partial, bn.rows, C, sums, dgamma_acc, dbeta_acc, stream);
+  B200_CHECK_LAUNCH("bn_bwd_reduce_final_kernel");
   return B200_OK;
 }
 
diff --git a/convnet/pytorch_b200/csrc/host.cu b/convnet/pytorch_b200/csrc/host.cu
--- a/convnet/pytorch_b200/csrc/host.cu
+++ b/convnet/pytorch_b200/csrc/host.cu
@@ -48,7 +48,7 @@
                                   CUtensorMapSwizzle, CUtensorMapL2promotion, CUtensorMapFloatOOBfill);
 
 int encode_tiled(CUtensorMap* tm, const void* base, int rank, const long long (&dims)[4], const int (&box)[4],
-                 const char* what) {
+                 const char* what, bool swizzle) {
   static EncodeTiledFn fn = (EncodeTiledFn)driver_entry("cuTensorMapEncodeTiled");
   B200_REQUIRE(fn != nullptr, B200_ERR_CUDA, "cuTensorMapEncodeTiled entry point unavailable");
   cuuint64_t gdims[4], strides[3];
@@ -59,7 +59,8 @@
     if (i + 1 < rank) strides[i] = (i == 0 ? 2 : strides[i - 1]) * gdims[i];
   }
   CUresult r = fn(tm, CU_TENSOR_MAP_DATA_TYPE_BFLOAT16, rank, const_cast<void*>(base), gdims, strides, gbox, estr,
-                  CU_TENSOR_MAP_INTERLEAVE_NONE, swizzle_for_row_bytes(box[0] * 2), CU_TENSOR_MAP_L2_PROMOTION_L2_128B,
+                  CU_TENSOR_MAP_INTERLEAVE_NONE,
+                  swizzle ? swizzle_for_row_bytes(box[0] * 2) : CU_TENSOR_MAP_SWIZZLE_NONE, CU_TENSOR_MAP_L2_PROMOTION_L2_128B,
                   CU_TENSOR_MAP_FLOAT_OOB_FILL_NONE);
   if (r != CUDA_SUCCESS) {
     char d[96] = "", b[64] = "";
diff --git a/convnet/pytorch_b200/csrc/host.h b/convnet/pytorch_b200/csrc/host.h
--- a/convnet/pytorch_b200/csrc/host.h
+++ b/convnet/pytorch_b200/csrc/host.h
@@ -18,7 +18,7 @@
 EncodeIm2colFn encode_im2col_fn();
 
 int encode_tiled(CUtensorMap* tm, const void* base, int rank, const long long (&dims)[4], const int (&box)[4],
-                 const char* what);
+                 const char* what, bool swizzle = true);
 int set_smem_attr(const void* fn, int bytes);
 
 int launch_wgrad_reduce(const float* partial, float* dw, int K_out, int taps, int C, int ck, int tap_stride,
diff --git a/convnet/pytorch_b200/engine.py b/convnet/pytorch_b200/engine.py
--- a/convnet/pytorch_b200/engine.py
+++ b/convnet/pytorch_b200/engine.py
@@ -432,7 +432,7 @@
         dist.all_reduce(sums, group=self.sync_bn_group)
         sums.mul_(1.0 / self.sync_bn_world)
 
-    def _bn_bwd(self, u, dy, y_mask, act, want_g=False):
+    def _bn_bwd(self, u, dy, y_mask, act, want_g=False, reduced=False):
         bn = u.bn
         drop = getattr(u, 'drop', None)
         if drop is not None:
@@ -441,8 +441,9 @@
                 self._sync_bn_sums(u.sums)
             return ops.bn_bwd_dx_dropout(dy, u.z, u.mask, drop[1], u.mean, u.invstd, bn.gamma, u.sums), None
         mask = getattr(u, 'mask', None) if y_mask is not None else None
-        ops.bn_bwd_reduce(dy, y_mask, u.z, act, u.mean, u.invstd, bn.gamma, bn.beta, u.sums, bn.dgamma, bn.dbeta,
-                          self._ws, act_mask=mask)
+        if not reduced:
+            ops.bn_bwd_reduce(dy, y_mask, u.z, act, u.mean, u.invstd, bn.gamma, bn.beta, u.sums, bn.dgamma, bn.dbeta,
+                              self._ws, act_mask=mask)
         if self.sync_bn_world > 1:
             self._sync_bn_sums(u.sums)
         g = torch.empty_like(dy) if want_g else None
@@ -494,7 +495,13 @@
     def _spec_lo(convs):
         return min(c.slot.offset for c in convs)
 
-    def _conv_bwd(self, u, dz, need_dx=True, residual=None):
+    @staticmethod
+    def _dgrad_bn(v, y_mask, act):
+        if v is None or getattr(v, 'drop', None) is not None:
+            return None
+        return v, y_mask, act
+
+    def _conv_bwd(self, u, dz, need_dx=True, residual=None, bn=None):
         conv = u.conv
         if conv.groups == 1:
             self._wgrad_async(lambda: ops.conv_wgrad(u.x, dz, u.desc, conv.g32), u.x, dz)
@@ -513,7 +520,12 @@
             wt = conv.dgrad_weights()
         else:
             wt = conv.wt
-        return ops.conv_dgrad(dz, wt, u.desc, residual=residual)
+        if bn is None:
+            return ops.conv_dgrad(dz, wt, u.desc, residual=residual)
+        v, y_mask, act = bn
+        mask = getattr(v, 'mask', None) if y_mask is not None else None
+        return ops.conv_dgrad_bn_reduce(dz, wt, u.desc, y_mask, v.z, act, v.mean, v.invstd, v.bn.gamma, v.bn.beta,
+                                        v.sums, v.bn.dgamma, v.bn.dbeta, self._ws, residual=residual, act_mask=mask)
 
     def _head_build(self, fc, dropout_p=0.0):
         a = self.arena
@@ -795,10 +807,10 @@
         units.append(last)
         return last.y, {'units': units, 'down': down, 'se': se_tape}
 
-    def _block_bwd(self, spec, saved, dy):
+    def _block_bwd(self, spec, saved, dy, reduced=False, prev_bn=None):
         units, down = saved['units'], saved['down']
         last = units[-1]
-        dz, g = self._bn_bwd(last, dy, last.y, ACT_RELU, want_g=True)
+        dz, g = self._bn_bwd(last, dy, last.y, ACT_RELU, want_g=True, reduced=reduced)
         if saved.get('se') is not None:
             g = spec['se'].bwd(self, saved['se'], g)
         if down is not None:
@@ -806,13 +818,15 @@
             skip = self._conv_bwd(down, dzd)
         else:
             skip = g
-        d = self._conv_bwd(last, dz)
-        for u in reversed(units[1:-1]):
-            dz, _ = self._bn_bwd(u, d, None, ACT_RELU)
-            d = self._conv_bwd(u, dz)
+        bn = self._dgrad_bn(units[-2], None, ACT_RELU)
+        d = self._conv_bwd(last, dz, bn=bn)
+        for i in range(len(units) - 2, 0, -1):
+            dz, _ = self._bn_bwd(units[i], d, None, ACT_RELU, reduced=bn is not None)
+            bn = self._dgrad_bn(units[i - 1], None, ACT_RELU)
+            d = self._conv_bwd(units[i], dz, bn=bn)
         u = units[0]
-        dz, _ = self._bn_bwd(u, d, None, ACT_RELU)
-        return self._conv_bwd(u, dz, residual=skip)
+        dz, _ = self._bn_bwd(u, d, None, ACT_RELU, reduced=bn is not None)
+        return self._conv_bwd(u, dz, residual=skip, bn=prev_bn)
 
     def run_forward(self, x, training, want_tape, mix=None, aug=None):
         self._want_tape = want_tape
@@ -833,8 +847,14 @@
         self._transpose_weights()
         self._buckets_begin()
         d = self._head_bwd(tape['head'], dlogits, dl_bf16)
-        for spec, saved in zip(reversed(self.blocks), reversed(tape['blocks'])):
-            d = self._block_bwd(spec, saved, d)
+        reduced = False
+        blocks = tape['blocks']
+        for i in range(len(blocks) - 1, -1, -1):
+            spec, saved = self.blocks[i], blocks[i]
+            prev = blocks[i - 1]['units'][-1] if i > 0 else None
+            prev_bn = self._dgrad_bn(prev, prev.y, ACT_RELU) if prev is not None else None
+            d = self._block_bwd(spec, saved, d, reduced=reduced, prev_bn=prev_bn)
+            reduced = prev_bn is not None
             convs = spec['convs'] + ([spec['down'][0]] if spec['down'] is not None else [])
             self._bucket_point(self._spec_lo(convs))
         self._stem_bwd(tape['stem'], d)
diff --git a/convnet/pytorch_b200/lib.py b/convnet/pytorch_b200/lib.py
--- a/convnet/pytorch_b200/lib.py
+++ b/convnet/pytorch_b200/lib.py
@@ -44,6 +44,8 @@
     "b200_bn_apply": [_vp, _ll, _i, _vp, _vp, _vp, _vp, _vp, _vp, _i, _vp, _vp, _vp],
     "b200_bn_bwd_reduce": [_vp, _vp, _vp, _vp, _ll, _i, _i, _vp, _vp, _vp, _vp, _vp, _vp, _vp, _vp, _vp],
     "b200_bn_bwd_dx": [_vp, _vp, _vp, _vp, _ll, _i, _i, _vp, _vp, _vp, _vp, _vp, _vp, _vp, _vp],
+    "b200_conv_dgrad_bn_reduce": [_dp, _vp, _vp, _vp, _vp, _vp, _vp, _vp, _ll, _i, _i, _vp, _vp, _vp, _vp, _vp, _vp, _vp,
+                                  _vp, _vp],
     "b200_bn_l1_stats": [_vp, _ll, _i, _vp, _vp, _f, _f, _vp, _vp, _vp, _vp, _vp, _vp, _vp, _vp, _vp],
     "b200_bn_l1_eval_coeffs": [_i, _vp, _vp, _vp, _vp, _vp, _vp, _vp],
     "b200_bn_l1_bwd_dx": [_vp, _vp, _vp, _vp, _ll, _i, _i, _vp, _vp, _vp, _vp, _vp, _vp, _vp, _vp, _vp],
diff --git a/convnet/pytorch_b200/ops.py b/convnet/pytorch_b200/ops.py
--- a/convnet/pytorch_b200/ops.py
+++ b/convnet/pytorch_b200/ops.py
@@ -119,6 +119,23 @@
     with _T('conv_dgrad', _conv_flops(desc), _conv_bytes(dy, wt, out, residual)):
         _l.check(_l.load().b200_conv_dgrad(ctypes.byref(desc), dy.data_ptr(), wt.data_ptr(), out.data_ptr(),
                                            _l.ptr(residual), _stream()), "b200_conv_dgrad")
+    return out
+
+
+def conv_dgrad_bn_reduce(dy, wt, desc, y, z, act, mean, invstd, gamma, beta, sums, dgamma_acc, dbeta_acc, workspace,
+                         out=None, residual=None, act_mask=None):
+    _chk(dy, bf16, "dy"); _chk(wt, bf16, "wt"); _chk(residual, bf16, "residual")
+    _chk(y, bf16, "y"); _chk(z, bf16, "z"); _chk(act_mask, torch.uint8, "act_mask")
+    C = z.shape[-1]
+    M = z.numel() // C
+    if out is None:
+        out = torch.empty((desc.N, desc.H, desc.W, desc.C), device=dy.device, dtype=bf16)
+    with _T('conv_dgrad', _conv_flops(desc), _conv_bytes(dy, wt, out, residual) + z.numel() * z.element_size()):
+        _l.check(_l.load().b200_conv_dgrad_bn_reduce(
+            ctypes.byref(desc), dy.data_ptr(), wt.data_ptr(), out.data_ptr(), _l.ptr(residual), _l.ptr(y),
+            _l.ptr(act_mask), z.data_ptr(), M, C, int(act), mean.data_ptr(), invstd.data_ptr(), _l.ptr(gamma),
+            _l.ptr(beta), sums.data_ptr(), _l.ptr(dgamma_acc), _l.ptr(dbeta_acc), workspace.data_ptr(), _stream()),
+            "b200_conv_dgrad_bn_reduce")
     return out
 
 
diff --git a/include/b200conv.h b/include/b200conv.h
--- a/include/b200conv.h
+++ b/include/b200conv.h
@@ -74,6 +74,11 @@
 int b200_bn_bwd_dx(const void* dy, const void* y, const uint8_t* act_mask, const void* z, long long M, int C, int act,
                    const float* mean, const float* invstd, const float* gamma, const float* beta,
                    const float* sums, void* dz, void* g_out, b200_stream_t stream);
+int b200_conv_dgrad_bn_reduce(const b200_conv_desc* d, const void* dy, const void* wt, void* dx, const void* residual,
+                              const void* y, const uint8_t* act_mask, const void* z, long long M, int C, int act,
+                              const float* mean, const float* invstd, const float* gamma, const float* beta,
+                              float* sums, float* dgamma_acc, float* dbeta_acc, float* workspace,
+                              b200_stream_t stream);
 
 int b200_bn_l1_stats(const void* z, long long M, int C, const float* gamma, const float* beta, float eps,
                      float momentum, float* running_mean, float* running_var, float* mean, float* invstd,
```

After: 6699, median of 6. Within noise of the previous version (-0.0%).
